# galacticglum/composer

Hardware: AMD Instinct MI355X
Metric: MIDI-event tokens/sec (train, seq=1024) (higher is better)
Workload: dtype bf16; 1 GPU; 6L/8H/d512 Transformer train step, seq=1024, B=128/GPU, dropout 0.10, Adam lr 1e-3, synthetic int32 event ids (vocab 390), random-init weights; global_batch=128, seq_len=1024, parallelism=dp1

## Files before the change

composer_amd/_lib.py:

```python
import ctypes as C
import os

_HERE = os.path.dirname(os.path.abspath(__file__))
LIB_PATH = os.environ.get("COMPOSER_HIP_LIB") or os.path.join(_HERE, "lib", "libcomposer_hip.so")

CMP_FP32, CMP_BF16 = 0, 1
DECODE_LITERAL, DECODE_KV = 0, 1
KIND_VALUE, KIND_ADAM_M, KIND_ADAM_V, KIND_GRAD = 0, 1, 2, 3


class HipLibraryError(RuntimeError):
    pass


class ModelCfg(C.Structure):
    _fields_ = [
        ("vocab_size", C.c_int32), ("embedding_size", C.c_int32), ("window_size", C.c_int32),
        ("layers", C.c_int32), ("heads", C.c_int32), ("ln_eps", C.c_float),
        ("scale_attention", C.c_int32), ("use_layer_norm", C.c_int32),
        ("attn_dropout", C.c_float), ("resid_dropout", C.c_float),
        ("dtype", C.c_int32), ("max_batch", C.c_int32), ("max_seq", C.c_int32), ("seed", C.c_uint64),
    ]


_P = C.c_void_p
_i, _f, _i64, _u64, _u32 = C.c_int, C.c_float, C.c_int64, C.c_uint64, C.c_uint32

SIGNATURES = {
    "cmp_last_error": (C.c_char_p, []),
    "cmp_version": (_i, []),
    "cmp_build_key": (C.c_char_p, []),
    "cmp_device_count": (_i, []),
    "cmp_ctx_create": (_i, [_i, C.POINTER(_P)]),
    "cmp_ctx_destroy": (_i, [_P]),
    "cmp_sync": (_i, [_P]),
    "cmp_ctx_stream": (_P, [_P]),
    "cmp_dp_unique_id": (_i, [_P]),
    "cmp_dp_init": (_i, [_P, _i, _i, _P]),
    "cmp_dp_allreduce_test": (_i, [_P, _P, _i]),
    "cmp_dp_init_exchange": (_i, [_P, _i, _i, _P, _P]),
    "cmp_dp_test_hog": (_i, [_P, _i, _i]),
    "cmp_dp_set_gemm_cus": (_i, [_P, _i]),
    "cmp_dp_set_mask_rank": (_i, [_P, _i]),
    "cmp_dp_stats": (_i, [_P, _i, C.POINTER(_i64), C.POINTER(C.c_double), C.POINTER(_i64), C.POINTER(_i)]),
    "cmp_dp_rccl_version": (_i, [C.POINTER(_i)]),
    "cmp_dp_allreduce_pattern": (_i, [_P, _i, C.POINTER(C.c_double), C.POINTER(_i64), C.POINTER(_i)]),
    "cmp_model_create": (_i, [_P, C.POINTER(ModelCfg), C.POINTER(_P)]),
    "cmp_model_destroy": (_i, [_P]),
    "cmp_param_count": (_i, [_P, C.POINTER(_i)]),
    "cmp_param_info": (_i, [_P, _i, C.POINTER(C.c_char_p), C.POINTER(_i), C.POINTER(_i64 * 4), C.POINTER(_i64)]),
    "cmp_param_get": (_i, [_P, C.c_char_p, _i, _P, _i64]),
    "cmp_param_set": (_i, [_P, C.c_char_p, _i, _P, _i64]),
    "cmp_adam_iter_get": (_i, [_P, C.POINTER(_i64)]),
    "cmp_adam_iter_set": (_i, [_P, _i64]),
    "cmp_train_step": (_i, [_P, _P, _P, _i, _i, _f, C.POINTER(_f), C.POINTER(_f)]),
    "cmp_train_step_dev": (_i, [_P, _P, _P, _i, _i, _f]),
    "cmp_train_metrics": (_i, [_P, C.POINTER(_f), C.POINTER(_f)]),
    "cmp_train_step_launches": (_i, [_P, _P, _P, _i, _i, C.POINTER(_i), C.POINTER(_i)]),
    "cmp_train_step_graph_probe": (_i, [_P, _P, _P, _i, _i, C.POINTER(_i), C.POINTER(_i), _i, C.POINTER(_f)]),
    "cmp_train_step_async": (_i, [_P, _P, _P, _i, _i, _f, C.POINTER(_i64)]),
    "cmp_train_metrics_wait": (_i, [_P, _i64, C.POINTER(_f), C.POINTER(_f)]),
    "cmp_train_options": (_i, [_P, _f, _i]),
    "cmp_train_options_get": (_i, [_P, C.POINTER(_f), C.POINTER(_i), C.POINTER(_i)]),
    "cmp_train_grad_stats": (_i, [_P, C.POINTER(_f), C.POINTER(_f)]),
    "cmp_train_metrics_wait_ex": (_i, [_P, _i64, C.POINTER(_f), C.POINTER(_f), C.POINTER(_f), C.POINTER(_f)]),
    "cmp_loss_and_grads": (_i, [_P, _P, _P, _i, _i, C.POINTER(_f), C.POINTER(_f)]),
    "cmp_eval_step": (_i, [_P, _P, _P, _i, _i, C.POINTER(C.c_double), C.POINTER(_i64), C.POINTER(_i64)]),
    "cmp_present_get": (_i, [_P, _i, _i, _i, _P]),
    "cmp_forward_generation": (_i, [_P, C.POINTER(_i64)]),
    "cmp_present_get_at": (_i, [_P, _i, _i, _i, _i64, _P]),
    "cmp_hidden_get_at": (_i, [_P, _i, _i, _i, _i64, _P]),
    "cmp_forward_logits": (_i, [_P, _P, _i, _i, _P]),
    "cmp_forward": (_i, [_P, _P, _i, _i, _i, _P, _i, _P]),
    "cmp_forward_ex": (_i, [_P, _P, _i, _i, _i, _P, _i, _P, _P, _P, _P, _P]),
    "cmp_decode_begin": (_i, [_P, _P, _i, _i, _f, _u64]),
    "cmp_decode_steps": (_i, [_P, _i, _P]),
    "cmp_decode_logits_get": (_i, [_P, _P]),
    "cmp_decode_begin_slide": (_i, [_P, _P, _i, _i, _f, _u64]),
    "cmp_decode_batch_begin_slide": (_i, [_P, _P, _P, _i, _i, _i, _f, _u64]),
    "cmp_decode_slide_stats": (_i, [_P, _i, _P, _P]),
    "cmp_k_sample": (_i, [_P, _P, _i, _f, _u64, _u32, _i, _P]),
    "cmp_decode_batch_begin": (_i, [_P, _P, _P, _i, _i, _i, _f, _u64]),
    "cmp_decode_batch_steps": (_i, [_P, _i, _P]),
    "cmp_decode_batch_logits_get": (_i, [_P, _P]),
    "cmp_k_sample_rows": (_i, [_P, _P, _i, _i, _i, _f, _u64, _u32, _P]),
    "cmp_k_sample_ex": (_i, [_P, _P, _i, _f, _i, _f, _u64, _u32, _i, _P]),
    "cmp_decode_begin_ex": (_i, [_P, _P, _i, _i, _i, _f, _i, _f, _u64]),
    "cmp_decode_batch_begin_ex": (_i, [_P, _P, _P, _i, _i, _i, _i, _P, _P, _P, _u64]),
    "cmp_k_sample_rows_ex": (_i, [_P, _P, _i, _i, _i, _P, _P, _P, _u64, _u32, _P]),
    "cmp_prof_begin": (_i, [_i]),
    "cmp_prof_end": (_i, [C.POINTER(C.c_double), C.POINTER(_i64), C.POINTER(C.c_double)]),
    "cmp_prof_pause": (_i, []),
    "cmp_prof_resume": (_i, []),
    "cmp_prof_end2": (_i, [C.POINTER(C.c_double), C.POINTER(_i64), C.POINTER(C.c_double), C.POINTER(C.c_double)]),
    "cmp_k_embed_fwd": (_i, [_P, _P, _P, _P, _P, _i, _i, _i, _i, _i, _f, _u64, _u32]),
    "cmp_k_embed_bwd": (_i, [_P, _P, _P, _P, _P, _i, _i, _i, _i, _i, _f, _u64, _u32]),
    "cmp_k_embed_bwd_v": (_i, [_P, _P, _P, _P, _P, _i, _i, _i, _i, _i, _f, _u64, _u32, _i]),
    "cmp_k_layernorm_fwd": (_i, [_P, _P, _P, _P, _P, _P, _P, _i, _i, _f, _i]),
    "cmp_k_layernorm_bwd": (_i, [_P, _P, _P, _P, _P, _P, _P, _P, _P, _P, _P, _i, _i, _i]),
    "cmp_k_layernorm_bwd_ws": (_i64, [_i, _i]),
    "cmp_k_layernorm_bwd_fused": (_i, [_P, _P, _P, _P, _P, _P, _P, _P, _P, _P, _P, _i, _i, _i, _P, _P, _f, _u64, _u32]),
    "cmp_k_gemm": (_i, [_P, _i, _i, _i, _i, _i, _i, _P, _i, _P, _i, _P, _i, _P, _i, _P, _i, _P, _i, _i, _i, _f, _u64, _u32, _i]),
    "cmp_k_embed_fwd_stats": (_i, [_P, _P, _P, _P, _P, _P, _i, _i, _i, _i, _f, _u64, _u32]),
    "cmp_k_ln_fold_prep": (_i, [_P, _P, _P, _P, _P, _P, _P, _P, _i, _i]),
    "cmp_gemm_ln_next": (_i, [_P, _i, _f, _P, _P, _P, _P]),
    "cmp_gemm_ln_scale_next": (_i, [_P, _i, _f]),
    "cmp_attn_bwd_ln_next": (_i, [_P]),
    "cmp_k_ln_stats_merge": (_i, [_P, _P, _i, _f, _P, _P, _i]),
    "cmp_k_layernorm_bwd_prescaled": (_i, [_P, _P, _P, _P, _P, _P, _P, _P, _P, _P, _P, _i, _i, _P, _P, _f, _u64, _u32]),
    "cmp_k_wgrad_ln_fix": (_i, [_P, _P, _i, _i, _P, _P, _P]),
    "cmp_k_layernorm_bwd_parts": (_i, [_P, _P, _P, _P, _P, _P, _f, _P, _P, _P, _P, _P, _P, _i, _i, _P, _P, _f, _u64, _u32]),
    "cmp_model_path_info": (_i, [_P, C.POINTER(_i), C.POINTER(_i64)]),
    "cmp_k_wgrad_group": (_i, [_P, _i, _P, _P, _P, _P, _P, _P, _P, _P, _i]),
    "cmp_gemm_set_workspace": (_i, [_P, _i64]),
    "cmp_gemm_colsum_next": (_i, [_P]),
    "cmp_gemm_set_stamps": (_i, [_P]),
    "cmp_k_colsum": (_i, [_P, _P, _i, _P, _i, _i, _i]),
    "cmp_k_attn_fwd": (_i, [_P, _P, _P, _P, _i, _i, _i, _i, _i, _i, _f, _u64, _u32]),
    "cmp_attn_bwd_bias_next": (_i, [_P]),
    "cmp_k_attn_bwd": (_i, [_P, _P, _P, _P, _P, _P, _P, _i, _i, _i, _i, _i, _i, _f, _u64, _u32]),
    "cmp_k_softmax_xent": (_i, [_P, _P, _i, _P, _P, _P, _P, _i, _i, _f, _i]),
    "cmp_k_adam": (_i, [_P, _P, _P, _P, _P, _P, _i64, _f, _f, _f, _f, _i64, _f]),
    "cmp_k_adam_dev": (_i, [_P, _P, _P, _P, _P, _P, _i64, _f, _f, _f, _f, _i64, _P]),
    "cmp_k_grad_clip_ws": (_i64, [_i64]),
    "cmp_k_grad_clip": (_i, [_P, _P, _i64, _f, _f, _P, _P]),
}

_ADDED_LATER = {"cmp_gemm_ln_scale_next", "cmp_attn_bwd_ln_next", "cmp_k_layernorm_bwd_prescaled", "cmp_k_wgrad_ln_fix", "cmp_k_ln_stats_merge", "cmp_dp_rccl_version", "cmp_dp_allreduce_pattern", "cmp_dp_init_exchange", "cmp_train_step_graph_probe", "cmp_train_step_launches", "cmp_k_embed_fwd_stats", "cmp_k_ln_fold_prep", "cmp_gemm_ln_next", "cmp_k_layernorm_bwd_parts", "cmp_model_path_info", "cmp_forward_ex", "cmp_hidden_get_at", "cmp_dp_stats", "cmp_prof_end2", "cmp_prof_pause", "cmp_prof_resume", "cmp_k_wgrad_group", "cmp_k_embed_bwd_v", "cmp_decode_batch_begin", "cmp_decode_batch_steps", "cmp_k_sample_rows", "cmp_decode_logits_get", "cmp_decode_batch_logits_get", "cmp_k_sample_ex", "cmp_k_sample_rows_ex", "cmp_decode_begin_ex", "cmp_decode_batch_begin_ex", "cmp_train_options",
                "cmp_train_options_get", "cmp_train_grad_stats", "cmp_train_metrics_wait_ex", "cmp_k_adam_dev", "cmp_k_grad_clip_ws", "cmp_k_grad_clip"}

_lib = None


def load():
    global _lib
    if _lib is not None:
        return _lib
    if not os.path.exists(LIB_PATH):
        raise HipLibraryError(
            "libcomposer_hip.so not found at %s -- build it with `python -m composer_amd.build` "
            "(hipcc, gfx950).  composer_amd has no CPU fallback." % LIB_PATH)
    lib = C.CDLL(LIB_PATH)
    check_single_runtime()
    for name, (res, args) in SIGNATURES.items():
        if name in _ADDED_LATER and os.environ.get("COMPOSER_HIP_LIB") and not hasattr(lib, name):
            continue
        fn = getattr(lib, name)
        fn.restype = res
        fn.argtypes = args
    _lib = lib
    return lib


_RUNTIME_STEMS = ("libamdhip64", "librccl", "libhsa-runtime64")


def mapped_runtime_libraries():
    found = {k: set() for k in _RUNTIME_STEMS}
    try:
        with open("/proc/self/maps") as f:
            for line in f:
                path = line.rstrip("\n").split(None, 5)[-1] if line.count("/") else ""
                base = os.path.basename(path)
                for stem in _RUNTIME_STEMS:
                    if base.startswith(stem + ".so"):
                        found[stem].add(os.path.realpath(path))
    except OSError:
        pass
    return {k: sorted(v) for k, v in found.items()}


def check_single_runtime():
    dup = {k: v for k, v in mapped_runtime_libraries().items() if len(v) > 1 and k != "libhsa-runtime64"}
    if dup:
        raise HipLibraryError(
            "two copies of the GPU runtime are mapped into this process: %s.  libcomposer_hip.so was loaded before torch was "
            "imported, so it is bound to /opt/rocm's runtime while torch brought its own.  Fix: `import torch` BEFORE the first "
            "composer_amd call that loads the library (composer_amd._lib.load(), Transformer(...)), or do not import torch in "
            "this process, or put torch's lib directory first in LD_LIBRARY_PATH so both resolve to the same files."
            % "; ".join("%s -> %s" % (k, " AND ".join(v)) for k, v in sorted(dup.items())))


def runtime_info():
    v = C.c_int(0)
    rc = load().cmp_dp_rccl_version(C.byref(v))
    libs = mapped_runtime_libraries()
    return {"rccl_version": v.value if rc == 0 else None, "rccl_path": (libs.get("librccl") or [None])[0],
            "hip_runtime_path": (libs.get("libamdhip64") or [None])[0]}


def last_error():
    return load().cmp_last_error().decode("utf-8", "replace")


def check(rc, what=""):
    if rc != 0:
        raise HipLibraryError("%s failed (status %d): %s" % (what or "libcomposer_hip call", rc, last_error()))


def require_gpu():
    check_single_runtime()
    n = load().cmp_device_count()
    if n <= 0:
        raise HipLibraryError("no HIP device visible: composer_amd needs an MI355X (gfx950); there is no CPU fallback")
    return n
```

composer_amd/build.py:

```python
import hashlib
import json
import os
import subprocess
import sys
from concurrent.futures import ThreadPoolExecutor

HERE = os.path.dirname(os.path.abspath(__file__))
CSRC = os.path.join(HERE, "csrc")
OBJ = os.path.join(CSRC, "_obj")
LIBDIR = os.path.join(HERE, "lib")
LIB = os.path.join(LIBDIR, "libcomposer_hip.so")
ROOT = os.path.dirname(HERE)
SOURCES = ["elementwise.hip", "gemm.hip", "attention.hip", "model.hip", "decode.hip", "decode_batch.hip"]
ARCH = "gfx950"
FLAGS = ["--offload-arch=" + ARCH, "-O3", "-fPIC", "-std=c++17", "-Wno-unused-value", "-Wno-inline-asm", "-I" + os.path.join(ROOT, "include")]
SOURCE_FLAGS = {"attention.hip": ["-fno-slp-vectorize"]}


def flags_for(src, flags=None):
    return list(FLAGS if flags is None else flags) + SOURCE_FLAGS.get(src, [])


def _hipcc():
    for c in (os.environ.get("HIPCC"), "/opt/rocm/bin/hipcc", "hipcc"):
        if c and (os.path.isabs(c) and os.path.exists(c) or not os.path.isabs(c)):
            return c
    return "hipcc"


def _hipcc_version():
    try:
        return subprocess.run([_hipcc(), "--version"], capture_output=True, text=True).stdout.strip().split("\n")[0]
    except Exception:
        return "unknown"


def _headers():
    out = []
    for d in (CSRC, os.path.join(ROOT, "include")):
        for f in sorted(os.listdir(d)):
            if f.endswith(".h"):
                out.append(os.path.join(d, f))
    return out


def source_key(src, flags):
    h = hashlib.sha256()
    h.update(("\0".join(flags) + "\0" + _hipcc_version()).encode())
    for path in [os.path.join(CSRC, src)] + _headers():
        h.update(os.path.basename(path).encode() + b"\0")
        h.update(open(path, "rb").read())
    return h.hexdigest()


def _compile(src, force, flags, tag=""):
    obj = os.path.join(OBJ, tag + src.replace(".hip", ".o"))
    keyfile = obj + ".key"
    key = source_key(src, flags)
    if not force and os.path.exists(obj) and os.path.exists(keyfile) and open(keyfile).read().strip() == key:
        return obj, False, key
    sp = os.path.join(CSRC, src)
    cmd = [_hipcc()] + flags + ["-c", sp, "-o", obj]
    r = subprocess.run(cmd, capture_output=True, text=True)
    if r.returncode != 0:
        raise RuntimeError("hipcc failed for %s:\n%s\n%s" % (src, " ".join(cmd), r.stderr[-4000:]))
    open(keyfile, "w").write(key)
    return obj, True, key


def _lib_key(keys):
    return hashlib.sha256("".join(keys).encode()).hexdigest()


def _file_sha256(path):
    h = hashlib.sha256()
    with open(path, "rb") as f:
        for blk in iter(lambda: f.read(1 << 20), b""):
            h.update(blk)
    return h.hexdigest()


def _key_object(lib_key, tag):
    src = os.path.join(OBJ, tag + "buildkey.cpp")
    obj = os.path.join(OBJ, tag + "buildkey.o")
    open(src, "w").write('extern "C" const char* cmp_build_key(void) { return "%s"; }\n' % lib_key)
    r = subprocess.run(["g++", "-O1", "-fPIC", "-c", src, "-o", obj], capture_output=True, text=True)
    if r.returncode != 0:
        raise RuntimeError("g++ failed for buildkey.cpp:\n" + r.stderr[-2000:])
    return obj


def build(force=False, verbose=True, asan=False):
    os.makedirs(OBJ, exist_ok=True)
    os.makedirs(LIBDIR, exist_ok=True)
    flags = FLAGS + (["-fsanitize=address", "-fno-gpu-sanitize", "-shared-libsan", "-g", "-fno-omit-frame-pointer"] if asan else [])
    tag = "asan_" if asan else ""
    lib = os.path.join(LIBDIR, "libcomposer_hip_asan.so") if asan else LIB
    info_path = os.path.join(LIBDIR, "BUILD_INFO_asan.json" if asan else "BUILD_INFO.json")
    with ThreadPoolExecutor(max_workers=min(5, os.cpu_count() or 1)) as ex:
        res = list(ex.map(lambda s: _compile(s, force, flags_for(s, flags), tag), SOURCES))
    objs = [o for o, _, _ in res]
    lib_key = _lib_key([k for _, _, k in res])
    old = {}
    try:
        old = json.load(open(info_path))
    except Exception:
        pass
    relink = any(c for _, c, _ in res) or not os.path.exists(lib) or old.get("library_key") != lib_key \
        or old.get("library_sha256") != _file_sha256(lib)
    if relink:
        objs = objs + [_key_object(lib_key, tag)]
        cmd = [_hipcc(), "--offload-arch=" + ARCH, "-shared", "-fPIC", "-o", lib] + objs + \
              ["-L/opt/rocm/lib", "-lrccl", "-Wl,-rpath,/opt/rocm/lib"] + (["-fsanitize=address", "-shared-libsan"] if asan else [])
        r = subprocess.run(cmd, capture_output=True, text=True)
        if r.returncode != 0:
            raise RuntimeError("link failed:\n%s\n%s" % (" ".join(cmd), r.stderr[-4000:]))
    info = {"library": os.path.basename(lib), "library_key": lib_key, "library_sha256": _file_sha256(lib), "hipcc": _hipcc_version(), "arch": ARCH,
            "sources": {s: {"key": k, "compiled_by_this_call": bool(c)} for s, (_, c, k) in zip(SOURCES, res)},
            "relinked_by_this_call": bool(relink)}
    json.dump(info, open(info_path, "w"), indent=1)
    if verbose:
        for s, (_, c, _) in zip(SOURCES, res):
            print("  %-18s %s" % (s, "compiled" if c else "cached object (source key unchanged)"))
        print(("built " if relink else "up to date: ") + lib)
    return lib


def verify():
    try:
        info = json.load(open(os.path.join(LIBDIR, "BUILD_INFO.json")))
    except Exception:
        return False
    if not os.path.exists(LIB):
        return False
    want = _lib_key([source_key(s, flags_for(s)) for s in SOURCES])
    if info.get("library_key") != want or info.get("library_sha256") != _file_sha256(LIB):
        return False
    import ctypes
    try:
        fn = ctypes.CDLL(LIB).cmp_build_key
    except (OSError, AttributeError):
        return False
    fn.restype = ctypes.c_char_p
    return fn().decode() == want


if __name__ == "__main__":
    build(force="--force" in sys.argv, asan="--asan" in sys.argv)
```

composer_amd/csrc/elementwise.hip:

```cpp
#include "model.h"

template <typename T>
__global__ void embed_fwd_kernel(const int32_t* __restrict__ ids, const float* __restrict__ wte,
                                 const float* __restrict__ wpe, T* __restrict__ out, int ntok, int T_,
                                 int E, int pos0, DropCfg drop, const int32_t* __restrict__ pos_ids,
                                 const int32_t* __restrict__ type_ids) {
    constexpr int VN = Vec16<T>::N;
    const int chunks = E / VN;
    int64_t gid = (int64_t)blockIdx.x * blockDim.x + threadIdx.x;
    int64_t total = (int64_t)ntok * chunks;
    for (; gid < total; gid += (int64_t)gridDim.x * blockDim.x) {
        int tok = (int)(gid / chunks);
        int e0 = (int)(gid % chunks) * VN;
        int id = ids[tok];
        int t = tok % T_;
        const float* a = wte + (int64_t)id * E + e0;
        const float* p = wpe + (int64_t)(pos_ids ? pos_ids[tok] : pos0 + t) * E + e0;
        const float* ty = type_ids ? wte + (int64_t)type_ids[tok] * E + e0 : nullptr;
        Vec16<T> r;
        const uint32_t rowh = drop_row_hash(drop, (uint32_t)tok);
#pragma unroll
        for (int i = 0; i < VN; i += 4) {
            f32x4 av = *reinterpret_cast<const f32x4*>(a + i);
            f32x4 pv = *reinterpret_cast<const f32x4*>(p + i);
// ... 632 lines not shown
        ssum = wave_sum(ssum);
        const float lse = gmx + logf(ssum);
        if (dz && active) {
            const float inv = 1.0f / ssum;
            Vec16<T> o0, o1;
            float g[8];
#pragma unroll
            for (int j = 0; j < 8; j++) g[j] = (c0 + j < V) ? (e[j] * inv - (c0 + j == yy ? 1.0f : 0.0f)) * inv_n : 0.f;
            T* dr = dz + (int64_t)row * ldz + c0;
            if constexpr (std::is_same<T, float>::value) {
#pragma unroll
                for (int j = 0; j < 4; j++) { o0.set(j, g[j]); o1.set(j, g[4 + j]); }
                st16(dr, o0);
                st16(dr + 4, o1);
            } else {
#pragma unroll
                for (int j = 0; j < 8; j++) o0.set(j, g[j]);
                st16(dr, o0);
            }
        }
        float zy = 0.f;
#pragma unroll
        for (int j = 0; j < 8; j++)
            if (j == (yy & 7)) zy = v[j];
        zy = __shfl(zy, yy >> 3);
        if (lane == 0) {
            row_loss[row] = lse - zy;
            row_correct[row] = (garg == yy) ? 1 : 0;
        }
    }
}

template <typename T>
__global__ void softmax_xent_wide_kernel(const float* __restrict__ z, int ldz, const int32_t* __restrict__ y,
                                         T* __restrict__ dz, float* __restrict__ row_loss,
                                         int32_t* __restrict__ row_correct, int rows, int V, float inv_n) {
    const int lane = threadIdx.x & 63;
    const int wpb = blockDim.x >> 6;
    for (int row = blockIdx.x * wpb + (threadIdx.x >> 6); row < rows; row += gridDim.x * wpb) {
        const float* zr = z + (int64_t)row * ldz;
        float mx = -INFINITY;
        int arg = 0x7fffffff;
        for (int c = lane; c < V; c += 64) {
            const float v = zr[c];
            if (v > mx) {
                mx = v;
                arg = c;
            }
        }
#pragma unroll
        for (int o = 32; o > 0; o >>= 1) {
            float om = __shfl_xor(mx, o);
            int oa = __shfl_xor(arg, o);
            if (om > mx || (om == mx && oa < arg)) {
                mx = om;
                arg = oa;
            }
        }
        float s = 0.f;
        for (int c = lane; c < V; c += 64) s += expf(zr[c] - mx);
        s = wave_sum(s);
        const float lse = mx + logf(s);
        const int yy = y[row];
        if (dz) {
            T* dr = dz + (int64_t)row * ldz;
            for (int c = lane; c < ldz; c += 64) {
                float g = 0.f;
                if (c < V) g = (expf(zr[c] - lse) - (c == yy ? 1.0f : 0.0f)) * inv_n;
                dr[c] = from_f32<T>(g);
            }
        }
        if (lane == 0) {
            row_loss[row] = lse - zr[yy];
            row_correct[row] = (arg == yy) ? 1 : 0;
        }
    }
}

__global__ __launch_bounds__(1024) void metrics_reduce_kernel(const float* __restrict__ row_loss, const int32_t* __restrict__ row_correct,
                                                               int rows, Metrics* __restrict__ out) {
    __shared__ double sl[1024];
    __shared__ long long sc[1024];
    double a0 = 0.0, a1 = 0.0, a2 = 0.0, a3 = 0.0;
    int c = 0;
    const int rows4 = rows >> 2;
    typedef int i32x4 __attribute__((ext_vector_type(4)));
    for (int i = threadIdx.x; i < rows4; i += 1024) {
        const f32x4 l = reinterpret_cast<const f32x4*>(row_loss)[i];
        const i32x4 k = reinterpret_cast<const i32x4*>(row_correct)[i];
        a0 += (double)l[0];
        a1 += (double)l[1];
        a2 += (double)l[2];
        a3 += (double)l[3];
        c += k[0] + k[1] + k[2] + k[3];
    }
    for (int i = (rows4 << 2) + threadIdx.x; i < rows; i += 1024) {
        a0 += (double)row_loss[i];
        c += row_correct[i];
    }
    sl[threadIdx.x] = (a0 + a1) + (a2 + a3);
    sc[threadIdx.x] = c;
    __syncthreads();
    for (int s = 512; s > 0; s >>= 1) {
        if (threadIdx.x < s) {
            sl[threadIdx.x] += sl[threadIdx.x + s];
            sc[threadIdx.x] += sc[threadIdx.x + s];
        }
        __syncthreads();
    }
    if (threadIdx.x == 0) {
        out->loss_sum = sl[0];
        out->correct = sc[0];
        out->loss_mean = (float)(sl[0] / (double)rows);
        out->acc = (float)((double)sc[0] / (double)rows);
    }
}

#define ADAM_LOOP()                                                                     \
    int64_t i = (int64_t)blockIdx.x * blockDim.x + threadIdx.x;                         \
    for (; i < n4; i += (int64_t)gridDim.x * blockDim.x) {                              \
        f32x4 pv = reinterpret_cast<f32x4*>(p)[i];                                      \
        f32x4 gv = reinterpret_cast<const f32x4*>(g)[i];                                \
        f32x4 mv = reinterpret_cast<f32x4*>(m)[i];                                      \
        f32x4 vv = reinterpret_cast<f32x4*>(v)[i];                                      \
        _Pragma("unroll")                                                               \
        for (int j = 0; j < 4; j++) {                                                   \
            float gg = gv[j] * gscale;                                                  \
            mv[j] = beta1 * mv[j] + (1.0f - beta1) * gg;                                \
            vv[j] = beta2 * vv[j] + (1.0f - beta2) * gg * gg;                           \
            pv[j] = pv[j] - alpha * mv[j] / (sqrtf(vv[j]) + eps);                       \
        }                                                                               \
        reinterpret_cast<f32x4*>(p)[i] = pv;                                            \
        reinterpret_cast<f32x4*>(m)[i] = mv;                                            \
        reinterpret_cast<f32x4*>(v)[i] = vv;                                            \
        if (shadow) {                                                                   \
            bf16x4 s;                                                                   \
            _Pragma("unroll")                                                           \
            for (int j = 0; j < 4; j++) s[j] = (bf16_t)pv[j];                           \
            reinterpret_cast<bf16x4*>(shadow)[i] = s;                                   \
        }                                                                               \
    }
__global__ void adam_kernel(float* __restrict__ p, const float* __restrict__ g, float* __restrict__ m,
                            float* __restrict__ v, bf16_t* __restrict__ shadow, int64_t n4, int64_t n,
                            float alpha, float beta1, float beta2, float eps, float gscale) {
    ADAM_LOOP()
}
__global__ void adam_dev_kernel(float* __restrict__ p, const float* __restrict__ g, float* __restrict__ m,
                                float* __restrict__ v, bf16_t* __restrict__ shadow, int64_t n4, int64_t n,
                                float alpha, float beta1, float beta2, float eps, const float* __restrict__ factor_dev) {
    const float gscale = *factor_dev;
    ADAM_LOOP()
}
#undef ADAM_LOOP

#define CLIP_CHUNK 8192
struct GradClipOut { double norm; float scale; float factor; };
__global__ __launch_bounds__(256) void grad_sumsq_kernel(const float* __restrict__ g, int64_t n4, double* __restrict__ slots) {
    __shared__ double sw[4];
    const int64_t base = (int64_t)blockIdx.x * (CLIP_CHUNK / 4);
    const int64_t lim = min(n4, base + CLIP_CHUNK / 4);
    double a0 = 0.0, a1 = 0.0, a2 = 0.0, a3 = 0.0;
#pragma unroll
    for (int r = 0; r < CLIP_CHUNK / 4 / 256; r++) {
        const int64_t i = base + r * 256 + threadIdx.x;
        if (i < lim) {
            const f32x4 x = reinterpret_cast<const f32x4*>(g)[i];
            const double d0 = (double)x[0], d1 = (double)x[1], d2 = (double)x[2], d3 = (double)x[3];
            a0 = fma(d0, d0, a0);
            a1 = fma(d1, d1, a1);
            a2 = fma(d2, d2, a2);
            a3 = fma(d3, d3, a3);
        }
    }
    double a = (a0 + a1) + (a2 + a3);
#pragma unroll
    for (int o = 32; o > 0; o >>= 1) a += __shfl_xor(a, o);
    if ((threadIdx.x & 63) == 0) sw[threadIdx.x >> 6] = a;
    __syncthreads();
    if (threadIdx.x == 0) slots[blockIdx.x] = (sw[0] + sw[1]) + (sw[2] + sw[3]);
}
__global__ __launch_bounds__(256) void grad_clip_finish_kernel(const double* __restrict__ slots, int nslots, float gscale, float clip_norm,
                                                               GradClipOut* __restrict__ out) {
    __shared__ double sl[256];
    double a = 0.0;
    for (int i = threadIdx.x; i < nslots; i += 256) a += slots[i];
    sl[threadIdx.x] = a;
    __syncthreads();
    for (int s = 128; s > 0; s >>= 1) {
        if ((int)threadIdx.x < s) sl[threadIdx.x] += sl[threadIdx.x + s];
        __syncthreads();
    }
    if (threadIdx.x == 0) {
        const double norm = (double)gscale * sqrt(sl[0]);
        const float scale = norm <= (double)clip_norm ? 1.0f : (float)((double)clip_norm / norm);
        out->norm = norm;
        out->scale = scale;
        out->factor = gscale * scale;
    }
}

__global__ void cast_f32_to_bf16_kernel(const float* __restrict__ in, bf16_t* __restrict__ out, int64_t n4) {
    int64_t i = (int64_t)blockIdx.x * blockDim.x + threadIdx.x;
    for (; i < n4; i += (int64_t)gridDim.x * blockDim.x) {
        f32x4 a = reinterpret_cast<const f32x4*>(in)[i];
        bf16x4 s;
#pragma unroll
        for (int j = 0; j < 4; j++) s[j] = (bf16_t)a[j];
        reinterpret_cast<bf16x4*>(out)[i] = s;
    }
}

template <typename T>
__global__ __launch_bounds__(256) void colsum_kernel(const T* __restrict__ X, int ldx, float* __restrict__ out, int rows, int cols,
                                                     float* __restrict__ part) {
    constexpr int VN = Vec16<T>::N;
    __shared__ float sm[4][64 * VN];
    const int lane = threadIdx.x & 63, wave = threadIdx.x >> 6;
    const int c0 = (blockIdx.x * 64 + lane) * VN;
    const int rows_per = cdiv(rows, (int)gridDim.y);
    const int r0 = blockIdx.y * rows_per;
    const int r1 = min(rows, r0 + rows_per);
    float acc[VN];
#pragma unroll
    for (int j = 0; j < VN; j++) acc[j] = 0.f;
    if (c0 < cols) {
        int r = r0 + wave;
        for (; r + 12 < r1; r += 16) {
            Vec16<T> v0 = ld16(X + (int64_t)r * ldx + c0), v1 = ld16(X + (int64_t)(r + 4) * ldx + c0);
            Vec16<T> v2 = ld16(X + (int64_t)(r + 8) * ldx + c0), v3 = ld16(X + (int64_t)(r + 12) * ldx + c0);
#pragma unroll
            for (int j = 0; j < VN; j++) acc[j] += (v0.get(j) + v1.get(j)) + (v2.get(j) + v3.get(j));
        }
        for (; r < r1; r += 4) {
            Vec16<T> v0 = ld16(X + (int64_t)r * ldx + c0);
#pragma unroll
            for (int j = 0; j < VN; j++) acc[j] += v0.get(j);
        }
    }
#pragma unroll
    for (int j = 0; j < VN; j++) sm[wave][lane * VN + j] = acc[j];
    __syncthreads();
    for (int i = threadIdx.x; i < 64 * VN; i += 256) {
        int c = blockIdx.x * 64 * VN + i;
        const float v = sm[0][i] + sm[1][i] + sm[2][i] + sm[3][i];
        if (c < cols) {
            if (part) part[(size_t)blockIdx.y * cols + c] = v;
            else atomicAdd(out + c, v);
        }
    }
}
__global__ void colsum_fold_kernel(const float* __restrict__ part, float* __restrict__ out, int splits, int cols) {
    const int c = blockIdx.x * blockDim.x + threadIdx.x;
    if (c >= cols) return;
    float a = 0.f;
    for (int sI = 0; sI < splits; sI++) a += part[(size_t)sI * cols + c];
    out[c] += a;
}

extern "C" int cmp_k_embed_fwd(void* stream, const int32_t* ids, const float* wte, const float* wpe, void* out,
                               int B, int T, int E, int pos0, int dtype, float p_drop, uint64_t seed,
                               uint32_t rng_stream) {
    return embed_fwd_run(stream, ids, wte, wpe, out, B, T, E, pos0, dtype, p_drop, seed, rng_stream, nullptr, nullptr);
}

int embed_fwd_run(void* stream, const int32_t* ids, const float* wte, const float* wpe, void* out, int B, int T, int E, int pos0,
                  int dtype, float p_drop, uint64_t seed, uint32_t rng_stream, const int32_t* pos_ids, const int32_t* type_ids) {
    CMP_REQUIRE(E % 8 == 0, "embed_fwd: E=%d must be a multiple of 8", E);
    hipStream_t s = (hipStream_t)stream;
    DropCfg d = make_drop(p_drop, seed, rng_stream);
    int ntok = B * T;
    if (ntok == 0) return CMP_OK;
    if (dtype == CMP_BF16) {
        int64_t total = (int64_t)ntok * (E / 8);
        int grid = (int)std::min<int64_t>(cdiv64(total, 256), 4096);
        embed_fwd_kernel<bf16_t><<<grid, 256, 0, s>>>(ids, wte, wpe, (bf16_t*)out, ntok, T, E, pos0, d, pos_ids, type_ids);
    } else {
        int64_t total = (int64_t)ntok * (E / 4);
        int grid = (int)std::min<int64_t>(cdiv64(total, 256), 4096);
        embed_fwd_kernel<float><<<grid, 256, 0, s>>>(ids, wte, wpe, (float*)out, ntok, T, E, pos0, d, pos_ids, type_ids);
    }
    KERNEL_CHECK();
    return CMP_OK;
}

int embed_fwd_stats_run(void* stream, const int32_t* ids, const float* wte, const float* wpe, void* out, float* part, int B, int T,
                        int E, int pos0, float p_drop, uint64_t seed, uint32_t rng_stream) {
    CMP_REQUIRE(E % 256 == 0 && E <= 2048, "embed_fwd_stats: E=%d must be a multiple of 256, at most 2048", E);
    hipStream_t s = (hipStream_t)stream;
    DropCfg d = make_drop(p_drop, seed, rng_stream);
    const int ntok = B * T;
    if (ntok == 0) return CMP_OK;
    const int grid = std::min(cdiv(ntok, 4), 8192), maxi = cdiv(E / 8, 64);
#define EMB_ST(MI) embed_fwd_stats_kernel<MI><<<grid, 256, 0, s>>>(ids, wte, wpe, (bf16_t*)out, part, ntok, T, E, pos0, d)
    if (maxi == 1) EMB_ST(1); else if (maxi == 2) EMB_ST(2); else EMB_ST(4);
#undef EMB_ST
    KERNEL_CHECK();
    return CMP_OK;
}
extern "C" int cmp_k_embed_fwd_stats(void* stream, const int32_t* ids, const float* wte, const float* wpe, void* out, float* part,
                                     int B, int T, int E, int pos0, float p_drop, uint64_t seed, uint32_t rng_stream) {
    return embed_fwd_stats_run(stream, ids, wte, wpe, out, part, B, T, E, pos0, p_drop, seed, rng_stream);
}

__global__ __launch_bounds__(256) void ln_fold_prep_kernel(const float* __restrict__ P, bf16_t* __restrict__ ST, float* __restrict__ fold,
                                                           const FoldDesc* __restrict__ desc) {
    __shared__ bf16_t tile[32][34];
// ... 277 lines not shown
__global__ __launch_bounds__(1024) void wgrad_ln_fix_kernel(LnFixDesc d0, LnFixDesc d1) {
    __shared__ float part[32][33];
    const LnFixDesc d = ((int)blockIdx.x >= d1.blk0 && d1.G) ? d1 : d0;
    const int tx = threadIdx.x & 31, ty = threadIdx.x >> 5;
    const int c = ((int)blockIdx.x - d.blk0) * 32 + tx;
    const bool ok = c < d.cols;
    float s0 = 0.f, s1 = 0.f, s2 = 0.f, s3 = 0.f;
    if (ok) {
        int k = ty;
        for (; k + 96 < d.rows; k += 128) {
            s0 += d.G[(int64_t)k * d.cols + c];
            s1 += d.G[(int64_t)(k + 32) * d.cols + c];
            s2 += d.G[(int64_t)(k + 64) * d.cols + c];
            s3 += d.G[(int64_t)(k + 96) * d.cols + c];
        }
        for (; k < d.rows; k += 32) s0 += d.G[(int64_t)k * d.cols + c];
    }
    part[ty][tx] = (s0 + s1) + (s2 + s3);
    __syncthreads();
    float tot = 0.f;
#pragma unroll
    for (int t = 0; t < 32; t++) tot += part[t][tx];
    if (!ok) return;
    const float mean = tot / (float)d.rows, bc = d.colsum[c];
    for (int k = ty; k < d.rows; k += 32) {
        const int64_t at = (int64_t)k * d.cols + c;
        d.G[at] = fmaf(d.gamma[k], d.G[at] - mean, d.beta[k] * bc);
    }
}
int wgrad_ln_fix_run(void* stream, float* G0, int rows0, int cols0, const float* gamma0, const float* beta0, const float* colsum0,
                     float* G1, int rows1, int cols1, const float* gamma1, const float* beta1, const float* colsum1) {
    CMP_REQUIRE(G0 && gamma0 && beta0 && colsum0 && rows0 > 0 && cols0 > 0, "wgrad_ln_fix: bad arguments");
    LnFixDesc d0{G0, gamma0, beta0, colsum0, rows0, cols0, 0, 0};
    LnFixDesc d1{G1, gamma1, beta1, colsum1, rows1, cols1, cdiv(cols0, 32), 0};
    const int grid = cdiv(cols0, 32) + (G1 ? cdiv(cols1, 32) : 0);
    wgrad_ln_fix_kernel<<<grid, 1024, 0, (hipStream_t)stream>>>(d0, d1);
    KERNEL_CHECK();
    return CMP_OK;
}
int layernorm_bwd_run(void* stream, const void* dy, const void* x, const float* gamma, const float* mean, const float* rstd,
                      const void* resid, void* dx, float* dgamma, float* dbeta, void* ws, int rows, int E, int dtype, void* dmask,
                      float* colsum, float p_drop, uint64_t seed, uint32_t rng_stream, bool deterministic, const LnBwdFused* fz,
                      bool keep_dmask, bool prescaled) {
    int rc = ln_check(E, dtype);
    if (rc) return rc;
    if (rows == 0) return CMP_OK;
    hipStream_t s = (hipStream_t)stream;
    int grid = ln_bwd_grid(rows);
    size_t smem = (size_t)4 * 3 * E * sizeof(float);
    const int vn = dtype == CMP_BF16 ? 8 : 4;
    const int maxi = cdiv(E / vn, 64);
    DropCfg dcfg = make_drop(p_drop, seed, rng_stream);
    if (fz) CMP_REQUIRE(dtype == CMP_BF16 && fz->part && fz->beta && E % 256 == 0 && fz->np == E / 256,
                        "layernorm_bwd: the statistics-from-partials form needs bf16 rows of a multiple of 256 columns (E=%d, np=%d)", E, fz->np);
    if (p_drop <= 0.f && !fz && !keep_dmask) dmask = nullptr;
    PROF_START(8, s);
    const int want_cs = colsum != nullptr;
    const bool direct = !deterministic && grid <= 256;
    float* dg_ = direct ? dgamma : nullptr;
#define LN_BWD(TT, MI) do { \
        if (smem > 65536) HIP_CHECK(hipFuncSetAttribute((const void*)layernorm_bwd_kernel<TT, MI>, hipFuncAttributeMaxDynamicSharedMemorySize, (int)smem)); \
        layernorm_bwd_kernel<TT, MI><<<grid, 256, smem, s>>>((const TT*)dy, (const TT*)x, gamma, mean, rstd, (const TT*)resid, (TT*)dx, (float*)ws, rows, E, (TT*)dmask, want_cs, dcfg, dg_, dbeta, colsum); \
    } while (0)
#define LN_BWDF(MI) do { \
        if (smem > 65536) HIP_CHECK(hipFuncSetAttribute((const void*)layernorm_bwd_kernel<bf16_t, MI, true>, hipFuncAttributeMaxDynamicSharedMemorySize, (int)smem)); \
        layernorm_bwd_kernel<bf16_t, MI, true><<<grid, 256, smem, s>>>((const bf16_t*)dy, (const bf16_t*)x, gamma, mean, rstd, (const bf16_t*)resid, (bf16_t*)dx, (float*)ws, rows, E, (bf16_t*)dmask, want_cs, dcfg, dg_, dbeta, colsum, *fz); \
    } while (0)
#define LN_BWDP(MI) do { \
        if (smem > 65536) HIP_CHECK(hipFuncSetAttribute((const void*)layernorm_bwd_kernel<bf16_t, MI, false, true>, hipFuncAttributeMaxDynamicSharedMemorySize, (int)smem)); \
        layernorm_bwd_kernel<bf16_t, MI, false, true><<<grid, 256, smem, s>>>((const bf16_t*)dy, (const bf16_t*)x, gamma, mean, rstd, (const bf16_t*)resid, (bf16_t*)dx, (float*)ws, rows, E, (bf16_t*)dmask, want_cs, dcfg, dg_, dbeta, colsum); \
    } while (0)
    if (prescaled && !fz) {
        CMP_REQUIRE(dtype == CMP_BF16 && maxi <= 4, "layernorm_bwd: the prescaled form exists for bf16 rows of at most 2048 columns");
        if (maxi == 1) LN_BWDP(1); else if (maxi == 2) LN_BWDP(2); else LN_BWDP(4);
    } else
    if (fz) { if (maxi == 1) LN_BWDF(1); else if (maxi == 2) LN_BWDF(2); else if (maxi <= 4) LN_BWDF(4); else LN_BWDF(8); }
    else if (dtype == CMP_BF16) { if (maxi == 1) LN_BWD(bf16_t, 1); else if (maxi == 2) LN_BWD(bf16_t, 2); else if (maxi <= 4) LN_BWD(bf16_t, 4); else LN_BWD(bf16_t, 8); }
    else { if (maxi == 1) LN_BWD(float, 1); else if (maxi == 2) LN_BWD(float, 2); else if (maxi <= 4) LN_BWD(float, 4); else LN_BWD(float, 8); }
#undef LN_BWD
#undef LN_BWDF
#undef LN_BWDP
    KERNEL_CHECK();
    if (!direct)
        ln_param_reduce_kernel<<<dim3(cdiv(3 * E, 256), deterministic ? 1 : std::min(grid, 32)), 256, 0, s>>>((const float*)ws, dgamma, dbeta, colsum, grid, E);
    {
        const double lb = (double)rows * ((3.0 + (resid ? 1.0 : 0.0) + (dmask ? 1.0 : 0.0) + (fz && fz->yout ? 1.0 : 0.0)) * E * dtype_size(dtype) + 8.0);
        PROF_STOP(8, s, lb, lb);
    }
    KERNEL_CHECK();
    return CMP_OK;
}

extern "C" int cmp_k_softmax_xent(void* stream, const float* logits, int ldz, const int32_t* y, void* dlogits,
                                  float* row_loss, int32_t* row_correct, int rows, int V, float inv_n, int dtype) {
    CMP_REQUIRE(V > 0 && V <= ldz, "softmax_xent: V=%d ldz=%d", V, ldz);
    if (rows == 0) return CMP_OK;
    hipStream_t s = (hipStream_t)stream;
    int grid = std::min(cdiv(rows, 4), 8192);
    if (ldz > 64 * XENT_MAXI) {
        if (dtype == CMP_BF16)
            softmax_xent_wide_kernel<bf16_t><<<grid, 256, 0, s>>>(logits, ldz, y, (bf16_t*)dlogits, row_loss, row_correct, rows, V, inv_n);
        else
            softmax_xent_wide_kernel<float><<<grid, 256, 0, s>>>(logits, ldz, y, (float*)dlogits, row_loss, row_correct, rows, V, inv_n);
    } else if (ldz % 8 == 0 && ((uintptr_t)logits & 15) == 0 && ((uintptr_t)dlogits & 15) == 0) {
        if (dtype == CMP_BF16)
            softmax_xent8_kernel<bf16_t><<<grid, 256, 0, s>>>(logits, ldz, y, (bf16_t*)dlogits, row_loss, row_correct, rows, V, inv_n);
        else
            softmax_xent8_kernel<float><<<grid, 256, 0, s>>>(logits, ldz, y, (float*)dlogits, row_loss, row_correct, rows, V, inv_n);
    } else if (dtype == CMP_BF16)
        softmax_xent_kernel<bf16_t><<<grid, 256, 0, s>>>(logits, ldz, y, (bf16_t*)dlogits, row_loss, row_correct, rows, V, inv_n);
    else
        softmax_xent_kernel<float><<<grid, 256, 0, s>>>(logits, ldz, y, (float*)dlogits, row_loss, row_correct, rows, V, inv_n);
    KERNEL_CHECK();
    return CMP_OK;
}

int launch_metrics_reduce(hipStream_t s, const float* row_loss, const int32_t* row_correct, int rows, void* metrics) {
    metrics_reduce_kernel<<<1, 1024, 0, s>>>(row_loss, row_correct, rows, (Metrics*)metrics);
    KERNEL_CHECK();
    return CMP_OK;
}

extern "C" int cmp_k_adam(void* stream, float* p, const float* g, float* m, float* v, void* shadow_bf16, int64_t n,
                          float lr, float beta1, float beta2, float eps, int64_t step, float grad_scale) {
    CMP_REQUIRE(n % 4 == 0, "adam: n=%lld must be a multiple of 4", (long long)n);
    if (n == 0) return CMP_OK;
    hipStream_t s = (hipStream_t)stream;
    double alpha = (double)lr * sqrt(1.0 - pow((double)beta2, (double)step)) / (1.0 - pow((double)beta1, (double)step));
    int64_t n4 = n / 4;
    int grid = (int)std::min<int64_t>(cdiv64(n4, 256), 8192);
    PROF_START(7, s);
    adam_kernel<<<grid, 256, 0, s>>>(p, g, m, v, (bf16_t*)shadow_bf16, n4, n, (float)alpha, beta1, beta2, eps, grad_scale);
    PROF_STOP(7, s, (double)n * (28.0 + (shadow_bf16 ? 2.0 : 0.0)), (double)n * (28.0 + (shadow_bf16 ? 2.0 : 0.0)));
    KERNEL_CHECK();
    return CMP_OK;
}

extern "C" int cmp_k_adam_dev(void* stream, float* p, const float* g, float* m, float* v, void* shadow_bf16, int64_t n,
                              float lr, float beta1, float beta2, float eps, int64_t step, const float* factor_dev) {
    CMP_REQUIRE(n % 4 == 0, "adam_dev: n=%lld must be a multiple of 4", (long long)n);
    CMP_REQUIRE(factor_dev, "adam_dev: null factor");
    if (n == 0) return CMP_OK;
    hipStream_t s = (hipStream_t)stream;
    double alpha = (double)lr * sqrt(1.0 - pow((double)beta2, (double)step)) / (1.0 - pow((double)beta1, (double)step));
    int64_t n4 = n / 4;
    int grid = (int)std::min<int64_t>(cdiv64(n4, 256), 8192);
    PROF_START(7, s);
    adam_dev_kernel<<<grid, 256, 0, s>>>(p, g, m, v, (bf16_t*)shadow_bf16, n4, n, (float)alpha, beta1, beta2, eps, factor_dev);
    PROF_STOP(7, s, (double)n * (28.0 + (shadow_bf16 ? 2.0 : 0.0)), (double)n * (28.0 + (shadow_bf16 ? 2.0 : 0.0)));
    KERNEL_CHECK();
    return CMP_OK;
}

int64_t grad_sumsq_slots(int64_t n) { return cdiv64(n, CLIP_CHUNK); }
int grad_sumsq_run(void* stream, const float* g, int64_t n, double* slots) {
    CMP_REQUIRE(n % 4 == 0 && ((uintptr_t)g & 15) == 0, "grad_sumsq: n=%lld must be a multiple of 4 and the range 16-byte aligned", (long long)n);
    CMP_REQUIRE(grad_sumsq_slots(n) < (1ll << 31), "grad_sumsq: n=%lld is too large", (long long)n);
    if (n == 0) return CMP_OK;
    grad_sumsq_kernel<<<(int)grad_sumsq_slots(n), 256, 0, (hipStream_t)stream>>>(g, n / 4, slots);
    KERNEL_CHECK();
    return CMP_OK;
}
int grad_clip_finish_run(void* stream, const double* slots, int nslots, float gscale, float clip_norm, void* out) {
    grad_clip_finish_kernel<<<1, 256, 0, (hipStream_t)stream>>>(slots, nslots, gscale, clip_norm, (GradClipOut*)out);
    KERNEL_CHECK();
    return CMP_OK;
}
extern "C" int64_t cmp_k_grad_clip_ws(int64_t n) { return std::max<int64_t>(1, grad_sumsq_slots(n)) * 8; }
extern "C" int cmp_k_grad_clip(void* stream, const float* g, int64_t n, float gscale, float clip_norm, void* ws, void* out) {
    CMP_REQUIRE(g && ws && out && n > 0, "grad_clip: null argument or empty range");
    CMP_REQUIRE(clip_norm > 0.f, "grad_clip: clip_norm %g must be positive (+inf: measure only)", (double)clip_norm);
    CMP_REQUIRE(((uintptr_t)ws & 7) == 0 && ((uintptr_t)out & 7) == 0, "grad_clip: ws and out must be 8-byte aligned");
    { const int rc = grad_sumsq_run(stream, g, n, (double*)ws); if (rc != CMP_OK) return rc; }
    return grad_clip_finish_run(stream, (const double*)ws, (int)grad_sumsq_slots(n), gscale, clip_norm, out);
}

int launch_cast_bf16(hipStream_t s, const float* in, void* out, int64_t n) {
    if (n == 0) return CMP_OK;
    int64_t n4 = n / 4;
    int grid = (int)std::min<int64_t>(cdiv64(n4, 256), 8192);
    cast_f32_to_bf16_kernel<<<grid, 256, 0, s>>>(in, (bf16_t*)out, n4);
    KERNEL_CHECK();
    return CMP_OK;
}

extern "C" int cmp_k_colsum(void* stream, const void* X, int ldx, float* out, int rows, int cols, int dtype) {
    return colsum_run(stream, X, ldx, out, rows, cols, dtype, nullptr, 0);
}

int colsum_run(void* stream, const void* X, int ldx, float* out, int rows, int cols, int dtype, float* det_ws, size_t det_ws_bytes) {
    if (rows == 0 || cols == 0) return CMP_OK;
    hipStream_t s = (hipStream_t)stream;
    const int vn = dtype == CMP_BF16 ? 8 : 4;
    CMP_REQUIRE(cols % vn == 0 && ldx % vn == 0, "colsum: cols=%d and ldx=%d must be multiples of %d", cols, ldx, vn);
    const int gx = cdiv(cols, 64 * vn);
    int splits = std::max(1, std::min(std::min(rows / 64, 128), std::max(1, 1024 / gx)));
    dim3 grid(gx, splits);
    if (det_ws) CMP_REQUIRE((size_t)splits * cols * 4 <= det_ws_bytes, "colsum: deterministic workspace too small");
    if (dtype == CMP_BF16)
        colsum_kernel<bf16_t><<<grid, 256, 0, s>>>((const bf16_t*)X, ldx, out, rows, cols, det_ws);
    else
        colsum_kernel<float><<<grid, 256, 0, s>>>((const float*)X, ldx, out, rows, cols, det_ws);
    if (det_ws) colsum_fold_kernel<<<cdiv(cols, 256), 256, 0, s>>>(det_ws, out, splits, cols);
    KERNEL_CHECK();
    return CMP_OK;
}
```

composer_amd/csrc/model.h:

```cpp
#pragma once
#include "common.h"
#include <rccl/rccl.h>
#include <vector>
#include <string>
#include <map>

struct DecodeState;
struct DecodeBatchState;

struct GradClipStats { double norm; float scale; float factor; };

struct Metrics {
    double loss_sum;
    long long correct;
    float loss_mean;
    float acc;
    int bad_ids;
    int pad;
};

#define NCCL_CHECK(expr)                                                                         \
    do {                                                                                         \
        ncclResult_t _r = (expr);                                                                \
        if (_r != ncclSuccess) {                                                                 \
            cmp_set_error("%s:%d: %s failed: %s", __FILE__, __LINE__, #expr, ncclGetErrorString(_r)); \
            return CMP_ERR_RCCL;                                                                 \
        }                                                                                        \
    } while (0)

#define CHECK_RC(expr)            \
    do {                          \
        int _rc = (expr);         \
        if (_rc != CMP_OK) return _rc; \
    } while (0)

struct cmp_ctx {
    int device = 0;
    hipStream_t stream = nullptr;
    hipStream_t comm_stream = nullptr;
    ncclComm_t comm = nullptr;
    int (*xfn)(void*, void*, int64_t, void*) = nullptr;
    void* xuser = nullptr;
    bool dp_on() const { return comm != nullptr || xfn != nullptr; }
    int rank = 0, nranks = 1;
    uint32_t seed_mix = 0;
    int mask_rank = 0;
    int gemm_max_wgs = 0;
    hipStream_t copy_stream = nullptr;
    SchedWs gemm_sched;
};
void sched_ws_free(SchedWs* w);

struct ParamInfo {
    std::string name;
    int rank;
    int64_t shape[4];
    int64_t numel;
    int64_t offset;
    int pad = 0;
    int64_t store = 0;
};

struct LayerOff {
    int64_t ln1_g, ln1_b, attn_w, attn_b, proj_w, proj_b, ln2_g, ln2_b, fc_w, fc_b, pr_w, pr_b;
    int64_t begin, end;
};

struct WDesc {
    int64_t off;
    int rows, cols;
};

struct FoldDesc {
    int64_t w_off, b_off, g_off, be_off;
    int64_t out_off;
    int rows, cols;
};

struct LayerAct {
    void *u, *qkv, *att, *r, *n, *fc, *g;
    float *ln1_mean, *ln1_rstd, *ln2_mean, *ln2_rstd, *lse;
    float *ln1_part = nullptr, *ln2_part = nullptr;
};

struct cmp_model {
    cmp_ctx* ctx = nullptr;
    cmp_model_cfg cfg;
    int V, E, W, L, H, D, ldz;
    int Dl = 0, Ea = 0;
    int dtype;
    size_t es;
    std::vector<ParamInfo> params;
    std::map<std::string, int> index;
    int64_t total = 0;
    int64_t off_wte = 0, off_wpe = 0, off_lnf_g = 0, off_lnf_b = 0;
    std::vector<LayerOff> lo;
    float *P = nullptr, *G = nullptr, *Am = nullptr, *Av = nullptr;
    bf16_t* S = nullptr;
    bf16_t* ST = nullptr;
    void* wdesc = nullptr;
    void* wdesc_plain = nullptr;
    void* fdesc = nullptr;
    void* ln_sites = nullptr;
    float* lnfold = nullptr;
    int64_t fold_stride = 0;
    int st_state = 0;
    int64_t st_version = -1;
    bool fused_last = false;
    void* dmask3 = nullptr;
    bf16_t* wte_lnf = nullptr;
    float* lnf_fold = nullptr;
    int lnf_npad = 0;
    float* lnf_part = nullptr;
    bool hf_valid = false;
    int64_t iterations = 0;
    int64_t param_version = 0;
    int capB = 0, capT = 0;
    std::vector<void*> allocs;
    std::vector<void*> xs;
    const int32_t* fwd_pos_ids = nullptr;
    const int32_t* fwd_type_ids = nullptr;
    const float* fwd_amask = nullptr;
    float* const* fwd_probs_out = nullptr;
    float* fwd_probs_dev = nullptr;
    void* io_buf[3] = {nullptr, nullptr, nullptr};
    size_t io_buf_bytes[3] = {0, 0, 0};
    std::vector<LayerAct> act;
    void *hf = nullptr, *dlogits = nullptr;
    float* logits_pack = nullptr;
    float *logits = nullptr, *lnf_mean = nullptr, *lnf_rstd = nullptr, *row_loss = nullptr, *delta = nullptr;
    int32_t *row_correct = nullptr, *x_dev = nullptr, *y_dev = nullptr;
    void *dx = nullptr, *dr = nullptr, *tmpE = nullptr, *dmask = nullptr, *dfc = nullptr, *dqkv = nullptr;
    int* embed_ws = nullptr;
    int64_t embed_ws_words = 0;
    void* dmask2 = nullptr;
    std::vector<WgradGroup> wgrad_groups;
    WgradWs wgrad_ws;
    void* ln_ws = nullptr;
    void* slab = nullptr;
    int64_t slab_bytes = 0;
    Metrics* metrics = nullptr;
    Metrics* metrics_host = nullptr;
    float* dp_metrics = nullptr;
    static constexpr int STAGES = 3;
    int32_t* stage_host[STAGES] = {nullptr, nullptr, nullptr};
    int32_t* stage_dev[STAGES] = {nullptr, nullptr, nullptr};
    Metrics* stage_metrics = nullptr;
    hipEvent_t stage_uploaded[STAGES] = {nullptr, nullptr, nullptr};
    hipEvent_t stage_done[STAGES] = {nullptr, nullptr, nullptr};
    int64_t stage_ticket[STAGES] = {-1, -1, -1};
    int64_t next_ticket = 0;
    int64_t stage_cap = 0;
    int lastB = 0, lastT = 0, last_past = 0;
    int64_t fwd_gen = 0;
    std::vector<hipEvent_t> bucket_ev;
    hipEvent_t comm_done = nullptr, metrics_ev = nullptr;
    static constexpr int DP_RING = 32;
    hipEvent_t dp_wait_a[DP_RING] = {}, dp_wait_b[DP_RING] = {};
    bool dp_wait_used[DP_RING] = {};
    int64_t dp_steps = 0;
    int64_t dp_folded = 0;
    double dp_exposed_ms = 0.0;
    int64_t dp_bytes_step = 0;
    int dp_msgs_step = 0;
    int dp_buckets_updated = 0;
    bool poisoned = false;
    float clip_norm = 0.f;
    int accum_steps = 1;
    int accum_pending = 0;
    int accumB = 0, accumT = 0;
    double* clip_slots = nullptr;
    int64_t clip_slots_cap = 0;
    int64_t clip_slots_used = 0;
    GradClipStats* clip_out = nullptr;
    GradClipStats* clip_host = nullptr;
    bool last_has_norm = false;
    bool stage_has_norm[3] = {false, false, false};
    std::vector<char> reload_seen;
    int ln_fused_mode = -1;
    DecodeState* dec = nullptr;
    DecodeBatchState* decb = nullptr;
    int gemm_role = -1;

    uint64_t drop_seed() const { return (uint64_t)((uint32_t)cfg.seed ^ ctx->seed_mix); }
    const void* w(int64_t off) const { return dtype == CMP_BF16 ? (const void*)(S + off) : (const void*)(P + off); }
};


template <typename Tp> static int dev_alloc(cmp_model* m, Tp** p, size_t bytes) {
    void* q = nullptr;
    HIP_CHECK(hipMalloc(&q, bytes ? bytes : 16));
    m->allocs.push_back(q);
    *p = (Tp*)q;
    return CMP_OK;
}

int embed_fwd_run(void* stream, const int32_t* ids, const float* wte, const float* wpe, void* out, int B, int T, int E, int pos0,
                  int dtype, float p_drop, uint64_t seed, uint32_t rng_stream, const int32_t* pos_ids, const int32_t* type_ids);
int embed_bwd_run(void* stream, const int32_t* ids, const void* dh, float* dwte, float* dwpe, int B, int T, int E, int pos0,
                  int dtype, float p_drop, uint64_t seed, uint32_t rng_stream, int V, float* det_ws, size_t det_ws_bytes,
                  int sort_V = 0, int* sort_ws = nullptr, int64_t sort_ws_words = 0);
int64_t embed_bwd_sort_ws_words(int64_t ntok, int V);
struct LnBwdFused {
    const float* part = nullptr;
    int np = 0;
    float eps = 0.f;
    const float* beta = nullptr;
    void* yout = nullptr;
    int prescaled = 0;
};
int wgrad_ln_fix_run(void* stream, float* G0, int rows0, int cols0, const float* gamma0, const float* beta0, const float* colsum0,
                     float* G1, int rows1, int cols1, const float* gamma1, const float* beta1, const float* colsum1);
int layernorm_bwd_run(void* stream, const void* dy, const void* x, const float* gamma, const float* mean, const float* rstd,
                      const void* resid, void* dx, float* dgamma, float* dbeta, void* ws, int rows, int E, int dtype, void* dmask,
                      float* colsum, float p_drop, uint64_t seed, uint32_t rng_stream, bool deterministic, const LnBwdFused* fz = nullptr,
                      bool keep_dmask = false, bool prescaled = false);
int ln_stats_merge_run(void* stream, const void* sites_dev, int nsites, int np, float eps, int rows);
int embed_fwd_stats_run(void* stream, const int32_t* ids, const float* wte, const float* wpe, void* out, float* part, int B, int T,
                        int E, int pos0, float p_drop, uint64_t seed, uint32_t rng_stream);
int ln_fold_prep_run(void* stream, const float* P, void* ST, float* fold, const void* desc_dev, int ndesc, int max_cols);
int lnf_fold_prep_run(void* stream, const float* wte, const float* gamma, const float* beta, void* out, float* cs, float* bias, int V, int E,
                      int npad);
int colsum_run(void* stream, const void* X, int ldx, float* out, int rows, int cols, int dtype, float* det_ws, size_t det_ws_bytes);
int launch_metrics_reduce(hipStream_t s, const float* row_loss, const int32_t* row_correct, int rows, void* metrics);
int launch_cast_bf16(hipStream_t s, const float* in, void* out, int64_t n);
int64_t grad_sumsq_slots(int64_t n);
int grad_sumsq_run(void* stream, const float* g, int64_t n, double* slots);
int grad_clip_finish_run(void* stream, const double* slots, int nslots, float gscale, float clip_norm, void* out);
int ensure_workspace(cmp_model* m, int B, int T);
int model_forward(cmp_model* m, const int32_t* x_dev, int B, int T, bool training, int64_t step, int past_len = 0);
void decode_state_free(DecodeState* d);
void decode_batch_state_free(DecodeBatchState* d);
int decode_batch_slide_stats(DecodeBatchState* d, int64_t* row_slides, int64_t* forward_calls);
```

composer_amd/csrc/model.hip:

```cpp
#include "model.h"
#include <stdarg.h>
#include <dlfcn.h>

static thread_local char g_err[1024] = "";
void cmp_set_error(const char* fmt, ...) {
    va_list ap;
    va_start(ap, fmt);
    vsnprintf(g_err, sizeof(g_err), fmt, ap);
    va_end(ap);
}
extern "C" const char* cmp_last_error(void) { return g_err; }
extern "C" int cmp_version(void) { return 1; }
extern "C" int cmp_device_count(void) {
    int n = 0;
    if (hipGetDeviceCount(&n) != hipSuccess) return 0;
    return n;
}

thread_local int g_prof_cls = -1;
static thread_local std::vector<hipEvent_t> g_prof_ev;
static thread_local size_t g_prof_used = 0;
static thread_local double g_prof_work = 0.0, g_prof_bytes = 0.0;
void prof_start(int, hipStream_t s) {
    if (g_prof_used + 2 > g_prof_ev.size()) {
// ... 151 lines not shown
        const int rc = c->xfn(c->xuser, p, (int64_t)n, (void*)c->comm_stream);
        if (rc != 0) {
            cmp_set_error("data-parallel exchange function failed with %d on %zu floats", rc, n);
            return CMP_ERR_INVALID;
        }
        return CMP_OK;
    }
    NCCL_CHECK(ncclAllReduce(p, p, n, ncclFloat, ncclSum, c->comm, c->comm_stream));
    return CMP_OK;
}
extern "C" int cmp_dp_set_mask_rank(cmp_ctx* c, int rank) {
    CMP_REQUIRE(c && rank >= 0, "dp_set_mask_rank: bad arguments");
    c->seed_mix = mix32((uint32_t)rank);
    c->mask_rank = rank;
    return CMP_OK;
}
extern "C" int cmp_dp_set_gemm_cus(cmp_ctx* c, int cus) {
    CMP_REQUIRE(c && cus >= 0 && cus <= 256, "dp_set_gemm_cus: 0 (all) .. 256");
    c->gemm_max_wgs = cus;
    return CMP_OK;
}
__global__ __launch_bounds__(1024) void cu_hog_kernel(unsigned long long ticks, int* sink) {
    __shared__ int big[16384];
    big[threadIdx.x] = (int)threadIdx.x;
    __syncthreads();
    const unsigned long long t0 = __builtin_amdgcn_s_memrealtime();
    while (__builtin_amdgcn_s_memrealtime() - t0 < ticks) __builtin_amdgcn_s_sleep(32);
    if (sink && big[(threadIdx.x * 7) & 16383] == -1) *sink = 1;
}
extern "C" int cmp_dp_test_hog(cmp_ctx* c, int wgs, int usec) {
    CMP_REQUIRE(c && wgs > 0 && wgs <= 256 && usec > 0 && usec <= 1000000, "dp_test_hog: bad arguments");
    HIP_CHECK(hipSetDevice(c->device));
    cu_hog_kernel<<<wgs, 1024, 0, c->comm_stream>>>((unsigned long long)usec * 100ull, nullptr);
    KERNEL_CHECK();
    return CMP_OK;
}
extern "C" int cmp_dp_allreduce_test(cmp_ctx* c, float* host_inout, int n) {
    CMP_REQUIRE(c && c->dp_on(), "dp_allreduce_test: communicator not initialised");
    float* d = nullptr;
    HIP_CHECK(hipMalloc(&d, (size_t)n * 4));
    HIP_CHECK(hipMemcpyAsync(d, host_inout, (size_t)n * 4, hipMemcpyHostToDevice, c->comm_stream));
    if (const int rc = dp_allreduce(c, d, (size_t)n)) {
        (void)hipStreamSynchronize(c->comm_stream);
        (void)hipFree(d);
        return rc;
    }
    HIP_CHECK(hipMemcpyAsync(host_inout, d, (size_t)n * 4, hipMemcpyDeviceToHost, c->comm_stream));
    HIP_CHECK(hipStreamSynchronize(c->comm_stream));
    HIP_CHECK(hipFree(d));
    return CMP_OK;
}

static int64_t add_param(cmp_model* m, const std::string& name, int rank, int64_t d0, int64_t d1, int pad = 0) {
    ParamInfo p;
    p.name = name;
    p.rank = rank;
    p.shape[0] = d0;
    p.shape[1] = d1;
    p.shape[2] = p.shape[3] = 1;
    p.numel = d0 * (rank > 1 ? d1 : 1);
    p.pad = (m->Dl == m->D) ? 0 : pad;
    p.store = p.numel;
    if (p.pad == 1) p.store = d0 * 3 * m->Ea;
    if (p.pad == 2) p.store = (int64_t)m->Ea * d1;
    p.offset = m->total;
    m->total += (p.store + 7) / 8 * 8;
    m->index[name] = (int)m->params.size();
    m->params.push_back(p);
    return p.offset;
}


static int model_create_fill(cmp_model* m, cmp_ctx* ctx, const cmp_model_cfg* cfg, int V, int E, int W, int L, int H, int D, int Dl);
extern "C" int cmp_model_destroy(cmp_model* m);

extern "C" int cmp_model_create(cmp_ctx* ctx, const cmp_model_cfg* cfg, cmp_model** out) {
    CMP_REQUIRE(ctx && cfg && out, "model_create: null argument");
    const int V = cfg->vocab_size, E = cfg->embedding_size, W = cfg->window_size, L = cfg->layers, H = cfg->heads;
    CMP_REQUIRE(V > 0 && E > 0 && W > 0 && L > 0 && H > 0, "model_create: sizes must be positive");
    CMP_REQUIRE(E % H == 0, "model_create: embedding_size %d not divisible by heads %d (transformer.py:255)", E, H);
    CMP_REQUIRE(E % 8 == 0, "model_create: embedding_size %d must be a multiple of 8", E);
    CMP_REQUIRE(E <= 2048, "model_create: embedding_size %d unsupported (at most 2048: LayerNorm rows, per-token decode rows of 4E)", E);
    const int Dl = E / H;
    CMP_REQUIRE(Dl <= 128, "model_create: head size %d unsupported (at most 128)", Dl);
    const int D = Dl <= 16 ? 16 : (Dl <= 32 ? 32 : (Dl <= 64 ? 64 : 128));
    CMP_REQUIRE(cfg->dtype == CMP_FP32 || cfg->dtype == CMP_BF16, "model_create: bad dtype %d", cfg->dtype);
    CMP_REQUIRE(L < 64, "model_create: at most 63 layers");
    HIP_CHECK(hipSetDevice(ctx->device));
    cmp_model* m = new cmp_model();
    m->ctx = ctx;
    {
        const char* e = getenv("COMPOSER_LN_FUSED");
        m->ln_fused_mode = e ? atoi(e) : -1;
    }
    const int rc = model_create_fill(m, ctx, cfg, V, E, W, L, H, D, Dl);
    if (rc != CMP_OK) { cmp_model_destroy(m); return rc; }
    *out = m;
    return CMP_OK;
}

static int model_create_fill(cmp_model* m, cmp_ctx* ctx, const cmp_model_cfg* cfg, int V, int E, int W, int L, int H, int D, int Dl) {
    m->cfg = *cfg;
    m->V = V; m->E = E; m->W = W; m->L = L; m->H = H; m->D = D; m->Dl = Dl; m->Ea = H * D;
    m->ldz = (V + 63) / 64 * 64;
    m->dtype = cfg->dtype;
    m->es = dtype_size(cfg->dtype);
    m->off_wte = add_param(m, "wte/weight", 2, V, E);
    m->off_wpe = add_param(m, "wpe/embeddings", 2, W, E);
    m->lo.resize(L);
    for (int i = 0; i < L; i++) {
        std::string p = "decoder_blocks/" + std::to_string(i) + "/";
        LayerOff& o = m->lo[i];
        o.begin = m->total;
        o.ln1_g = add_param(m, p + "ln_1/gamma", 1, E, 1);
        o.ln1_b = add_param(m, p + "ln_1/beta", 1, E, 1);
        o.attn_w = add_param(m, p + "attn/c_attn/weight", 2, E, 3 * E, 1);
        o.attn_b = add_param(m, p + "attn/c_attn/bias", 2, 1, 3 * E, 1);
        o.proj_w = add_param(m, p + "attn/c_proj/weight", 2, E, E, 2);
        o.proj_b = add_param(m, p + "attn/c_proj/bias", 2, 1, E);
        o.ln2_g = add_param(m, p + "ln_2/gamma", 1, E, 1);
        o.ln2_b = add_param(m, p + "ln_2/beta", 1, E, 1);
        o.fc_w = add_param(m, p + "mlp/c_fc/weight", 2, E, 4 * E);
        o.fc_b = add_param(m, p + "mlp/c_fc/bias", 2, 1, 4 * E);
        o.pr_w = add_param(m, p + "mlp/c_proj/weight", 2, 4 * E, E);
        o.pr_b = add_param(m, p + "mlp/c_proj/bias", 2, 1, E);
        o.end = m->total;
    }
    m->off_lnf_g = add_param(m, "ln_f/gamma", 1, E, 1);
    m->off_lnf_b = add_param(m, "ln_f/beta", 1, E, 1);
    size_t bytes = (size_t)m->total * 4;
    CHECK_RC(dev_alloc(m, &m->P, bytes));
    CHECK_RC(dev_alloc(m, &m->G, bytes));
    CHECK_RC(dev_alloc(m, &m->Am, bytes));
    CHECK_RC(dev_alloc(m, &m->Av, bytes));
    HIP_CHECK(hipMemsetAsync(m->P, 0, bytes, ctx->stream));
    HIP_CHECK(hipMemsetAsync(m->G, 0, bytes, ctx->stream));
    HIP_CHECK(hipMemsetAsync(m->Am, 0, bytes, ctx->stream));
    HIP_CHECK(hipMemsetAsync(m->Av, 0, bytes, ctx->stream));
    if (m->dtype == CMP_BF16) {
        CHECK_RC(dev_alloc(m, &m->S, (size_t)m->total * 2));
        HIP_CHECK(hipMemsetAsync(m->S, 0, (size_t)m->total * 2, ctx->stream));
        CHECK_RC(dev_alloc(m, &m->ST, (size_t)m->total * 2));
        HIP_CHECK(hipMemsetAsync(m->ST, 0, (size_t)m->total * 2, ctx->stream));
        std::vector<WDesc> wd;
        for (int i = 0; i < m->L; i++) {
            const LayerOff& o = m->lo[i];
            wd.push_back({o.attn_w, m->E, 3 * m->Ea});
            wd.push_back({o.proj_w, m->Ea, m->E});
            wd.push_back({o.fc_w, m->E, 4 * m->E});
            wd.push_back({o.pr_w, 4 * m->E, m->E});
        }
        CHECK_RC(dev_alloc(m, &m->wdesc, wd.size() * sizeof(WDesc)));
        HIP_CHECK(hipMemcpyAsync(m->wdesc, wd.data(), wd.size() * sizeof(WDesc), hipMemcpyHostToDevice, ctx->stream));
        std::vector<WDesc> wp;
        std::vector<FoldDesc> fd;
        m->fold_stride = 2 * (int64_t)(3 * m->Ea + 4 * m->E);
        for (int i = 0; i < m->L; i++) {
            const LayerOff& o = m->lo[i];
            wp.push_back({o.proj_w, m->Ea, m->E});
            wp.push_back({o.pr_w, 4 * m->E, m->E});
            fd.push_back({o.attn_w, o.attn_b, o.ln1_g, o.ln1_b, i * m->fold_stride, m->E, 3 * m->Ea});
            fd.push_back({o.fc_w, o.fc_b, o.ln2_g, o.ln2_b, i * m->fold_stride + 6 * m->Ea, m->E, 4 * m->E});
        }
        CHECK_RC(dev_alloc(m, &m->wdesc_plain, wp.size() * sizeof(WDesc)));
        CHECK_RC(dev_alloc(m, &m->fdesc, fd.size() * sizeof(FoldDesc)));
        CHECK_RC(dev_alloc(m, &m->lnfold, (size_t)m->L * m->fold_stride * 4));
        m->lnf_npad = cdiv(m->V, 256) * 256;
        CHECK_RC(dev_alloc(m, &m->wte_lnf, (size_t)m->V * m->E * 2));
        CHECK_RC(dev_alloc(m, &m->lnf_fold, (size_t)2 * m->lnf_npad * 4));
        HIP_CHECK(hipMemcpyAsync(m->wdesc_plain, wp.data(), wp.size() * sizeof(WDesc), hipMemcpyHostToDevice, ctx->stream));
        HIP_CHECK(hipMemcpyAsync(m->fdesc, fd.data(), fd.size() * sizeof(FoldDesc), hipMemcpyHostToDevice, ctx->stream));
        HIP_CHECK(hipStreamSynchronize(ctx->stream));
    }
    CHECK_RC(dev_alloc(m, &m->metrics, sizeof(Metrics)));
    CHECK_RC(dev_alloc(m, &m->dp_metrics, 16));
    HIP_CHECK(hipHostMalloc((void**)&m->metrics_host, sizeof(Metrics), hipHostMallocDefault));
    memset(m->metrics_host, 0, sizeof(Metrics));
    m->bucket_ev.resize(L + 2);
    for (auto& e : m->bucket_ev) HIP_CHECK(hipEventCreateWithFlags(&e, hipEventDisableTiming));
    HIP_CHECK(hipEventCreateWithFlags(&m->comm_done, hipEventDisableTiming));
    HIP_CHECK(hipEventCreateWithFlags(&m->metrics_ev, hipEventDisableTiming));
    HIP_CHECK(hipStreamSynchronize(ctx->stream));
    return CMP_OK;
}

extern "C" int cmp_model_destroy(cmp_model* m) {
    if (!m) return CMP_OK;
    hipSetDevice(m->ctx->device);
    hipStreamSynchronize(m->ctx->stream);
    hipStreamSynchronize(m->ctx->comm_stream);
    if (m->ctx->copy_stream) hipStreamSynchronize(m->ctx->copy_stream);
    if (m->dec) decode_state_free(m->dec);
    if (m->decb) decode_batch_state_free(m->decb);
    for (void* p : m->allocs) if (p) hipFree(p);
    for (auto& wg : m->wgrad_groups) wgrad_group_free(&wg);
    wgrad_ws_free(&m->wgrad_ws);
    if (m->metrics_host) hipHostFree(m->metrics_host);
    if (m->clip_host) hipHostFree(m->clip_host);
    if (m->stage_metrics) hipHostFree(m->stage_metrics);
    for (int i = 0; i < cmp_model::STAGES; i++) {
        if (m->stage_host[i]) hipHostFree(m->stage_host[i]);
        if (m->stage_uploaded[i]) hipEventDestroy(m->stage_uploaded[i]);
        if (m->stage_done[i]) hipEventDestroy(m->stage_done[i]);
    }
    for (auto& e : m->bucket_ev) hipEventDestroy(e);
    if (m->comm_done) hipEventDestroy(m->comm_done);
    if (m->metrics_ev) hipEventDestroy(m->metrics_ev);
    for (int i = 0; i < cmp_model::DP_RING; i++) {
        if (m->dp_wait_a[i]) hipEventDestroy(m->dp_wait_a[i]);
        if (m->dp_wait_b[i]) hipEventDestroy(m->dp_wait_b[i]);
    }
    delete m;
    (void)hipGetLastError();
    return CMP_OK;
}

extern "C" int cmp_param_count(cmp_model* m, int* n) {
    CMP_REQUIRE(m && n, "param_count: null");
    *n = (int)m->params.size();
    return CMP_OK;
}
extern "C" int cmp_param_info(cmp_model* m, int i, const char** name, int* rank, int64_t shape[4], int64_t* numel) {
    CMP_REQUIRE(m && i >= 0 && i < (int)m->params.size(), "param_info: index %d out of range", i);
    const ParamInfo& p = m->params[i];
    if (name) *name = p.name.c_str();
    if (rank) *rank = p.rank;
    if (shape) for (int k = 0; k < 4; k++) shape[k] = p.shape[k];
    if (numel) *numel = p.numel;
    return CMP_OK;
}
static void pad_copy(const cmp_model* m, const ParamInfo& p, float* st, float* logical, bool to_store) {
    const int H = m->H, D = m->D, Dl = m->Dl, E = m->E, Ea = m->Ea;
    if (p.pad == 1) {
        const int64_t rows = p.numel / (3 * E);
        for (int64_t r = 0; r < rows; r++)
            for (int part = 0; part < 3; part++)
                for (int h = 0; h < H; h++)
                    for (int d = 0; d < Dl; d++) {
                        float& a = st[r * 3 * Ea + (int64_t)part * Ea + h * D + d];
                        float& b = logical[r * 3 * E + (int64_t)part * E + h * Dl + d];
                        if (to_store) a = b; else b = a;
                    }
    } else {
        const int64_t cols = p.shape[1];
        for (int h = 0; h < H; h++)
            for (int d = 0; d < Dl; d++)
                for (int64_t c = 0; c < cols; c++) {
                    float& a = st[((int64_t)h * D + d) * cols + c];
                    float& b = logical[((int64_t)h * Dl + d) * cols + c];
                    if (to_store) a = b; else b = a;
                }
    }
}
static float* kind_buf(cmp_model* m, int kind) {
    switch (kind) {
        case 0: return m->P;
        case 1: return m->Am;
        case 2: return m->Av;
        case 3: return m->G;
    }
    return nullptr;
}
extern "C" int cmp_param_get(cmp_model* m, const char* name, int kind, float* host, int64_t numel) {
    CMP_REQUIRE(m && name && host, "param_get: null");
    auto it = m->index.find(name);
    CMP_REQUIRE(it != m->index.end(), "param_get: unknown parameter '%s'", name);
    const ParamInfo& p = m->params[it->second];
    CMP_REQUIRE(numel == p.numel, "param_get: '%s' has %lld elements, caller passed %lld", name, (long long)p.numel, (long long)numel);
    float* b = kind_buf(m, kind);
    CMP_REQUIRE(b, "param_get: bad kind %d", kind);
    HIP_CHECK(hipStreamSynchronize(m->ctx->stream));
    HIP_CHECK(hipStreamSynchronize(m->ctx->comm_stream));
    if (p.pad) {
        std::vector<float> st((size_t)p.store);
        HIP_CHECK(hipMemcpyAsync(st.data(), b + p.offset, (size_t)p.store * 4, hipMemcpyDeviceToHost, m->ctx->stream));
        HIP_CHECK(hipStreamSynchronize(m->ctx->stream));
        pad_copy(m, p, st.data(), host, false);
        return CMP_OK;
    }
    HIP_CHECK(hipMemcpyAsync(host, b + p.offset, (size_t)numel * 4, hipMemcpyDeviceToHost, m->ctx->stream));
    HIP_CHECK(hipStreamSynchronize(m->ctx->stream));
    return CMP_OK;
}
extern "C" int cmp_param_set(cmp_model* m, const char* name, int kind, const float* host, int64_t numel) {
    CMP_REQUIRE(m && name && host, "param_set: null");
    auto it = m->index.find(name);
    CMP_REQUIRE(it != m->index.end(), "param_set: unknown parameter '%s'", name);
    const ParamInfo& p = m->params[it->second];
    CMP_REQUIRE(numel == p.numel, "param_set: '%s' has %lld elements, caller passed %lld", name, (long long)p.numel, (long long)numel);
    float* b = kind_buf(m, kind);
    CMP_REQUIRE(b, "param_set: bad kind %d", kind);
    HIP_CHECK(hipStreamSynchronize(m->ctx->stream));
    if (p.pad) {
        std::vector<float> st((size_t)p.store, 0.f);
        pad_copy(m, p, st.data(), const_cast<float*>(host), true);
        HIP_CHECK(hipMemcpyAsync(b + p.offset, st.data(), (size_t)p.store * 4, hipMemcpyHostToDevice, m->ctx->stream));
        HIP_CHECK(hipStreamSynchronize(m->ctx->stream));
    } else {
        HIP_CHECK(hipMemcpyAsync(b + p.offset, host, (size_t)numel * 4, hipMemcpyHostToDevice, m->ctx->stream));
        HIP_CHECK(hipStreamSynchronize(m->ctx->stream));
    }
    if (kind == 0) {
        m->param_version += 1;
        if (m->poisoned) {
            if (m->reload_seen.size() != m->params.size()) m->reload_seen.assign(m->params.size(), 0);
            m->reload_seen[it->second] = 1;
            bool all = true;
            for (char c : m->reload_seen) all = all && c;
            if (all) { m->poisoned = false; m->reload_seen.clear(); }
        }
    }
    if (kind == 0 && m->S) {
        int64_t n8 = (p.store + 7) / 8 * 8;
        CHECK_RC(launch_cast_bf16(m->ctx->stream, m->P + p.offset, m->S + p.offset, n8));
        HIP_CHECK(hipStreamSynchronize(m->ctx->stream));
    }
    return CMP_OK;
}
extern "C" int cmp_adam_iter_get(cmp_model* m, int64_t* it) {
    CMP_REQUIRE(m && it, "adam_iter_get: null");
    *it = m->iterations;
    return CMP_OK;
}
extern "C" int cmp_adam_iter_set(cmp_model* m, int64_t it) {
    CMP_REQUIRE(m && it >= 0, "adam_iter_set: bad value");
    m->iterations = it;
    return CMP_OK;
}

static int ensure_workspace_fill(cmp_model* m, int B, int T);
int ensure_workspace(cmp_model* m, int B, int T) {
    const size_t mark = m->allocs.size();
    const int rc = ensure_workspace_fill(m, B, T);
    if (rc != CMP_OK && m->allocs.size() > mark) {
        for (size_t i = mark; i < m->allocs.size(); i++) (void)hipFree(m->allocs[i]);
        m->allocs.resize(mark);
        m->xs.clear(); m->act.clear();
        m->capB = 0; m->capT = 0;
        (void)hipGetLastError();
    }
    return rc;
}
static int ensure_workspace_fill(cmp_model* m, int B, int T) {
    CMP_REQUIRE(B > 0 && T > 0, "batch and sequence must be positive (B=%d T=%d)", B, T);
    CMP_REQUIRE(T <= m->W, "sequence length %d exceeds window_size %d (wpe rows, transformer.py:675-679)", T, m->W);
    if (m->capB * m->capT >= B * T && m->capB > 0) return CMP_OK;
    CMP_REQUIRE(m->capB == 0, "workspace was sized for %d tokens; create the model with max_batch/max_seq covering B=%d T=%d",
                m->capB * m->capT, B, T);
    int64_t M = (int64_t)B * T;
    int64_t Mcfg = (int64_t)std::max(1, m->cfg.max_batch) * std::max(1, std::min(m->cfg.max_seq, m->W));
    if (Mcfg > M) { M = Mcfg; }
    m->capB = (int)M; m->capT = 1;
    const int E = m->E, L = m->L;
    const size_t es = m->es;
    m->xs.resize(L + 1);
    for (int i = 0; i <= L; i++) CHECK_RC(dev_alloc(m, &m->xs[i], (size_t)M * E * es));
    m->act.resize(L);
    const bool ln = m->cfg.use_layer_norm != 0;
    for (int i = 0; i < L; i++) {
        LayerAct& a = m->act[i];
        if (ln) CHECK_RC(dev_alloc(m, &a.u, (size_t)M * E * es)); else a.u = m->xs[i];
        CHECK_RC(dev_alloc(m, &a.qkv, (size_t)M * 3 * m->Ea * es));
        CHECK_RC(dev_alloc(m, &a.att, (size_t)M * m->Ea * es));
        CHECK_RC(dev_alloc(m, &a.r, (size_t)M * E * es));
        if (ln) CHECK_RC(dev_alloc(m, &a.n, (size_t)M * E * es)); else a.n = a.r;
        CHECK_RC(dev_alloc(m, &a.fc, (size_t)M * 4 * E * es));
        CHECK_RC(dev_alloc(m, &a.g, (size_t)M * 4 * E * es));
        CHECK_RC(dev_alloc(m, &a.ln1_mean, (size_t)M * 4));
        CHECK_RC(dev_alloc(m, &a.ln1_rstd, (size_t)M * 4));
        CHECK_RC(dev_alloc(m, &a.ln2_mean, (size_t)M * 4));
        CHECK_RC(dev_alloc(m, &a.ln2_rstd, (size_t)M * 4));
        CHECK_RC(dev_alloc(m, &a.lse, (size_t)M * m->H * 4));
        if (ln && m->ST && E % 256 == 0) {
            CHECK_RC(dev_alloc(m, &a.ln1_part, (size_t)M * (E / 256) * 8));
            CHECK_RC(dev_alloc(m, &a.ln2_part, (size_t)M * (E / 256) * 8));
        }
    }
    if (ln && m->ST && E % 256 == 0) CHECK_RC(dev_alloc(m, &m->lnf_part, (size_t)M * (E / 256) * 8));
    if (ln && m->ST && E % 256 == 0) {
        std::vector<const void*> st;
        for (int i = 0; i < L; i++) {
            const LayerAct& a = m->act[i];
            st.insert(st.end(), {a.ln1_part, a.ln1_mean, a.ln1_rstd, a.ln2_part, a.ln2_mean, a.ln2_rstd});
        }
        CHECK_RC(dev_alloc(m, &m->ln_sites, st.size() * sizeof(void*)));
        HIP_CHECK(hipMemcpyAsync(m->ln_sites, st.data(), st.size() * sizeof(void*), hipMemcpyHostToDevice, m->ctx->stream));
        HIP_CHECK(hipStreamSynchronize(m->ctx->stream));
    }
    CHECK_RC(dev_alloc(m, &m->hf, (size_t)M * E * es));
    CHECK_RC(dev_alloc(m, &m->logits, (size_t)M * m->ldz * 4));
    CHECK_RC(dev_alloc(m, &m->dlogits, (size_t)M * m->ldz * es));
    CHECK_RC(dev_alloc(m, &m->lnf_mean, (size_t)M * 4));
    CHECK_RC(dev_alloc(m, &m->lnf_rstd, (size_t)M * 4));
    CHECK_RC(dev_alloc(m, &m->row_loss, (size_t)M * 4));
    CHECK_RC(dev_alloc(m, &m->row_correct, (size_t)M * 4));
    CHECK_RC(dev_alloc(m, &m->delta, (size_t)M * m->H * 4));
    CHECK_RC(dev_alloc(m, &m->x_dev, (size_t)M * 4));
    CHECK_RC(dev_alloc(m, &m->y_dev, (size_t)M * 4));
    CHECK_RC(dev_alloc(m, &m->dx, (size_t)M * E * es));
    CHECK_RC(dev_alloc(m, &m->dr, (size_t)M * E * es));
    CHECK_RC(dev_alloc(m, &m->tmpE, (size_t)M * m->Ea * es));
    CHECK_RC(dev_alloc(m, &m->dmask, (size_t)M * E * es));
    CHECK_RC(dev_alloc(m, &m->dmask2, (size_t)M * E * es));
    CHECK_RC(dev_alloc(m, &m->dmask3, (size_t)M * E * es));
    CHECK_RC(dev_alloc(m, &m->dfc, (size_t)M * 4 * E * es));
    CHECK_RC(dev_alloc(m, &m->dqkv, (size_t)M * 3 * m->Ea * es));
    {
        const char* det = getenv("COMPOSER_DETERMINISTIC");
        if (det && det[0] == '1') {
            m->slab_bytes = (int64_t)16 * E * std::max(4 * E, 3 * m->Ea) * 4 + (int64_t)64 * m->V * E * 4;
            CHECK_RC(dev_alloc(m, &m->slab, (size_t)m->slab_bytes));
        }
    }
    CHECK_RC(dev_alloc(m, &m->ln_ws, (size_t)cmp_k_layernorm_bwd_ws((int)std::min<int64_t>(M, 1 << 30), E)));
    m->embed_ws_words = embed_bwd_sort_ws_words(M, m->V);
    if (m->embed_ws_words > 0) CHECK_RC(dev_alloc(m, &m->embed_ws, (size_t)m->embed_ws_words * 4));
    return CMP_OK;
}

template <typename T>
__global__ void drop_apply_kernel(const T* __restrict__ in, T* __restrict__ out, int64_t n, int E, DropCfg d) {
    int64_t i = (int64_t)blockIdx.x * blockDim.x + threadIdx.x;
    for (; i < n; i += (int64_t)gridDim.x * blockDim.x)
        out[i] = from_f32<T>(apply_drop(d, (uint32_t)(i / E), (uint32_t)(i % E), to_f32<T>(in[i])));
}
static int drop_apply(cmp_model* m, const void* in, void* out, int64_t n, float p, uint32_t stream_id) {
    DropCfg d = make_drop(p, m->drop_seed(), stream_id);
    int grid = (int)std::min<int64_t>(cdiv64(n, 256), 8192);
    if (m->dtype == CMP_BF16)
        drop_apply_kernel<bf16_t><<<grid, 256, 0, m->ctx->stream>>>((const bf16_t*)in, (bf16_t*)out, n, m->cfg.embedding_size, d);
    else
        drop_apply_kernel<float><<<grid, 256, 0, m->ctx->stream>>>((const float*)in, (float*)out, n, m->cfg.embedding_size, d);
    KERNEL_CHECK();
    return CMP_OK;
}

__global__ __launch_bounds__(256) void transpose_weights_kernel(const bf16_t* __restrict__ S, bf16_t* __restrict__ ST,
                                                                const WDesc* __restrict__ desc) {
    __shared__ bf16_t tile[32][34];
    const WDesc d = desc[blockIdx.y];
    const int tiles_c = (d.cols + 31) >> 5, ntiles = ((d.rows + 31) >> 5) * tiles_c;
    if ((int)blockIdx.x >= ntiles) return;
    const int tr = (blockIdx.x / tiles_c) << 5, tc = (blockIdx.x % tiles_c) << 5;
    const int tx = threadIdx.x & 31, ty = threadIdx.x >> 5;
    const bf16_t* src = S + d.off;
    bf16_t* dst = ST + d.off;
#pragma unroll
    for (int j = 0; j < 4; j++) {
        const int r = tr + ty + 8 * j, c = tc + tx;
        tile[ty + 8 * j][tx] = (r < d.rows && c < d.cols) ? src[(int64_t)r * d.cols + c] : (bf16_t)0.f;
    }
    __syncthreads();
#pragma unroll
    for (int j = 0; j < 4; j++) {
        const int c = tc + ty + 8 * j, r = tr + tx;
        if (c < d.cols && r < d.rows) dst[(int64_t)c * d.rows + r] = tile[tx][ty + 8 * j];
    }
}
static int refresh_transposed_weights(cmp_model* m, bool fold) {
    if (!m->ST) return CMP_OK;
    const int want = fold ? 2 : 1;
    if (m->st_state == want && m->st_version == m->param_version) return CMP_OK;
    m->st_state = 0;
    const int maxtiles = std::max(cdiv(4 * m->E, 32) * cdiv(m->E, 32), cdiv(3 * m->Ea, 32) * cdiv(m->E, 32));
    if (fold) {
        transpose_weights_kernel<<<dim3(maxtiles, 2 * m->L), 256, 0, m->ctx->stream>>>(m->S, m->ST, (const WDesc*)m->wdesc_plain);
        KERNEL_CHECK();
        CHECK_RC(ln_fold_prep_run(m->ctx->stream, m->P, m->ST, m->lnfold, m->fdesc, 2 * m->L, 4 * m->E));
        CHECK_RC(lnf_fold_prep_run(m->ctx->stream, m->P + m->off_wte, m->P + m->off_lnf_g, m->P + m->off_lnf_b, m->wte_lnf, m->lnf_fold,
                                   m->lnf_fold + m->lnf_npad, m->V, m->E, m->lnf_npad));
    } else {
        transpose_weights_kernel<<<dim3(maxtiles, 4 * m->L), 256, 0, m->ctx->stream>>>(m->S, m->ST, (const WDesc*)m->wdesc);
        KERNEL_CHECK();
    }
    m->st_state = want;
    m->st_version = m->param_version;
    return CMP_OK;
}

static bool ln_fused_ok(const cmp_model* m, int M, int past_len, bool training) {
    if (m->ln_fused_mode == 0) return false;
    if (training && m->ln_fused_mode != 2 && m->ln_fused_mode != 3) return false;
    if (!m->cfg.use_layer_norm || m->dtype != CMP_BF16 || m->slab || past_len) return false;
    if (m->Ea != m->E || m->E % 256 || m->E < 512 || m->E > 768 || !m->act[0].ln1_part) return false;
    if (M % 256 || (int64_t)(M / 256) * (m->E / 256) < 192) return false;
    if (m->fwd_pos_ids || m->fwd_type_ids || m->fwd_amask || m->fwd_probs_out) return false;
    return true;
}

static int colsum_det(cmp_model* m, const void* X, int ldx, float* out, int rows, int cols) {
    return colsum_run(m->ctx->stream, X, ldx, out, rows, cols, m->dtype, (float*)m->slab, (size_t)m->slab_bytes);
}
static int colsum_any(cmp_model* m, const void* X, int ldx, float* out, int rows, int cols) {
    if (m->slab) return colsum_det(m, X, ldx, out, rows, cols);
    return cmp_k_colsum(m->ctx->stream, X, ldx, out, rows, cols, m->dtype);
}
static int ln_bwd(cmp_model* m, const void* dy, const void* x, const float* gamma, const float* mean, const float* rstd,
                  const void* resid, void* dx, float* dgamma, float* dbeta, int rows, void* dmask, float* colsum, float p_drop,
                  uint32_t rng_stream, const LnBwdFused* fz = nullptr, bool prescaled = false) {
    return layernorm_bwd_run(m->ctx->stream, dy, x, gamma, mean, rstd, resid, dx, dgamma, dbeta, m->ln_ws, rows, m->E, m->dtype,
                             dmask, colsum, p_drop, m->drop_seed(), rng_stream, m->slab != nullptr, fz, m->fused_last, prescaled);
}

#define GEMM_REV (1 << 20)
static int gemm(cmp_model* m, int ta, int tb, int M, int N, int K, const void* A, int lda, const void* B, int ldb, void* C,
                int ldc, const float* bias, int act, void* aux, int ldaux, const void* resid, int ldr, int out_fp32,
                int splitk, float p_drop, uint32_t rng_stream, int flags = 0, float* colsum = nullptr, const LnEpi* ln = nullptr) {
    const bool det = m->slab != nullptr;
    GemmExtra ex;
    if (ln) ex.ln = *ln;
    ex.rev = (flags & GEMM_REV) != 0;
    flags &= ~GEMM_REV;
    ex.colsum = det ? nullptr : colsum;
    if (splitk > 1 && det) { ex.slab_ws = (float*)m->slab; ex.slab_bytes = (size_t)m->slab_bytes; }
    ex.role = m->gemm_role >= 0 ? m->gemm_role : (ta ? 2 : 1);
    ex.max_wgs = m->ctx->dp_on() ? m->ctx->gemm_max_wgs : 0;
    ex.dp = m->ctx->dp_on();
    ex.sched = &m->ctx->gemm_sched;
    CHECK_RC(gemm_run(m->ctx->stream, m->dtype, ta, tb, M, N, K, A, lda, B, ldb, C, ldc, bias, act, aux, ldaux, resid, ldr,
                      out_fp32, splitk, p_drop, m->drop_seed(), rng_stream, flags, ex));
    if (det && colsum) CHECK_RC(colsum_det(m, C, ldc, colsum, M, N));
    return CMP_OK;
}

__global__ void rows_copy_kernel(const uint4* __restrict__ src, uint4* __restrict__ dst, int B, int Tn, int w, int sT, int s0,
                                 int src_ld, int dT, int d0, int dst_ld) {
    const int64_t n = (int64_t)B * Tn * w;
    for (int64_t i = (int64_t)blockIdx.x * blockDim.x + threadIdx.x; i < n; i += (int64_t)gridDim.x * blockDim.x) {
        const int c = (int)(i % w);
        const int t = (int)((i / w) % Tn);
        const int b = (int)(i / ((int64_t)w * Tn));
        dst[((int64_t)b * dT + d0 + t) * dst_ld + c] = src[((int64_t)b * sT + s0 + t) * src_ld + c];
    }
}
static int rows_copy(cmp_model* m, const void* src, void* dst, int B, int Tn, int width, int sT, int s0, int src_w, int dT, int d0,
                     int dst_w) {
    const int es = (int)m->es, w = width * es / 16;
    const int64_t n = (int64_t)B * Tn * w;
    rows_copy_kernel<<<(int)std::min<int64_t>(cdiv64(n, 256), 4096), 256, 0, m->ctx->stream>>>(
        (const uint4*)src, (uint4*)dst, B, Tn, w, sT, s0, src_w * es / 16, dT, d0, dst_w * es / 16);
    KERNEL_CHECK();
    return CMP_OK;
}

static float attn_scale(const cmp_model* m) { return m->cfg.scale_attention ? 1.0f / sqrtf((float)m->Dl) : 1.0f; }

int model_forward(cmp_model* m, const int32_t* x_dev, int B, int T, bool training, int64_t step, int past_len) {
    Range range_("composer.forward");
    hipStream_t s = m->ctx->stream;
    struct RoleGuard {
        cmp_model* m;
        RoleGuard(cmp_model* mm) : m(mm) { m->gemm_role = 0; }
        ~RoleGuard() { m->gemm_role = -1; }
    } role_guard(m);
    const int E = m->E, Ea = m->Ea, M = B * T, dt = m->dtype;
    const float pr = training ? m->cfg.resid_dropout : 0.f;
    const float pa = training ? m->cfg.attn_dropout : 0.f;
    const bool ln = m->cfg.use_layer_norm != 0;
    const int Tp = past_len, Tt = past_len + T;
    m->lastB = B; m->lastT = Tt; m->last_past = Tp;
    m->fwd_gen += 1;
    const bool fused = ln_fused_ok(m, M, Tp, training);
    m->fused_last = fused;
    if (fused)
        CHECK_RC(embed_fwd_stats_run(s, x_dev, m->P + m->off_wte, m->P + m->off_wpe, m->xs[0], m->act[0].ln1_part, B, T, E, 0, pr,
                                     m->drop_seed(), drop_stream(step, 0, 0)));
    else
        CHECK_RC(embed_fwd_run(s, x_dev, m->P + m->off_wte, m->P + m->off_wpe, m->xs[0], B, T, E, Tp, dt, pr, m->drop_seed(),
                               drop_stream(step, 0, 0), m->fwd_pos_ids, m->fwd_type_ids));
    CHECK_RC(refresh_transposed_weights(m, fused));
    const bool wt = m->ST != nullptr;
    auto W = [&](int64_t off) { return wt ? (const void*)(m->ST + off) : m->w(off); };
    static const int alt_mode = [] { const char* e = getenv("COMPOSER_GEMM_ALT"); return e ? atoi(e) : 1; }();
    const int RV[4] = {alt_mode == 2 ? GEMM_REV : 0, alt_mode == 1 ? GEMM_REV : 0, alt_mode == 2 ? GEMM_REV : 0, alt_mode == 1 ? GEMM_REV : 0};
    PROF_START(9, s);
    for (int i = 0; fused && i < m->L; i++) {
        const LayerOff& o = m->lo[i];
        LayerAct& a = m->act[i];
        const float* fold = m->lnfold + i * m->fold_stride;
        LnEpi l;
        l.in_part = a.ln1_part; l.np = E / 256; l.eps = m->cfg.ln_eps; l.cs = fold;
        CHECK_RC(gemm(m, 0, 1, M, 3 * E, E, m->xs[i], E, W(o.attn_w), E, a.qkv, 3 * E, fold + 3 * E, 0, nullptr, 0, nullptr, 0, 0, 1, 0.f,
                      0, RV[0], nullptr, &l));
        CHECK_RC(attn_fwd_run(s, a.qkv, a.att, a.lse, B, Tt, m->H, m->D, attn_scale(m), dt, pa, m->drop_seed(), drop_stream(step, i, 1),
                              nullptr));
        l = LnEpi();
        l.in_part = a.ln1_part; l.np = E / 256; l.eps = m->cfg.ln_eps; l.gamma = m->P + o.ln1_g; l.beta = m->P + o.ln1_b;
        l.out_part = a.ln2_part;
        CHECK_RC(gemm(m, 0, 1, M, E, E, a.att, E, W(o.proj_w), E, a.r, E, m->P + o.proj_b, 0, nullptr, 0, m->xs[i], E, 0, 1, pr,
                      drop_stream(step, i, 2), RV[1], nullptr, &l));
        l = LnEpi();
        l.in_part = a.ln2_part; l.np = E / 256; l.eps = m->cfg.ln_eps; l.cs = fold + 6 * E;
        CHECK_RC(gemm(m, 0, 1, M, 4 * E, E, a.r, E, W(o.fc_w), E, a.g, 4 * E, fold + 10 * E, 1, training ? a.fc : nullptr, 4 * E, nullptr,
                      0, 0, 1, 0.f, 0, RV[2], nullptr, &l));
        l = LnEpi();
        l.out_part = i + 1 < m->L ? m->act[i + 1].ln1_part : (training ? nullptr : m->lnf_part);
        CHECK_RC(gemm(m, 0, 1, M, E, 4 * E, a.g, 4 * E, W(o.pr_w), 4 * E, m->xs[i + 1], E, m->P + o.pr_b, 0, nullptr, 0, a.r, E, 0, 1, pr,
                      drop_stream(step, i, 3), RV[3], nullptr, l.out_part ? &l : nullptr));
    }
    for (int i = 0; !fused && i < m->L; i++) {
        const LayerOff& o = m->lo[i];
        LayerAct& a = m->act[i];
        if (ln)
            CHECK_RC(cmp_k_layernorm_fwd(s, m->xs[i], m->P + o.ln1_g, m->P + o.ln1_b, a.u, a.ln1_mean, a.ln1_rstd, M, E,
                                         m->cfg.ln_eps, dt));
        CHECK_RC(gemm(m, 0, wt, M, 3 * Ea, E, a.u, E, W(o.attn_w), wt ? E : 3 * Ea, Tp ? m->dqkv : a.qkv, 3 * Ea, m->P + o.attn_b, 0,
                      nullptr, 0, nullptr, 0, 0, 1, 0.f, 0));
        if (Tp) CHECK_RC(rows_copy(m, m->dqkv, a.qkv, B, T, 3 * Ea, T, 0, 3 * Ea, Tt, Tp, 3 * Ea));
        CHECK_RC(attn_fwd_run(s, a.qkv, a.att, a.lse, B, Tt, m->H, m->D, attn_scale(m), dt, pa, m->drop_seed(),
                              drop_stream(step, i, 1), m->fwd_amask));
        if (m->fwd_probs_out) {
            CHECK_RC(attn_probs_run(s, a.qkv, a.lse, m->fwd_amask, m->fwd_probs_dev, B, Tp, Tt, m->H, m->D, attn_scale(m), dt, pa,
                                    m->drop_seed(), drop_stream(step, i, 1)));
            HIP_CHECK(hipMemcpyAsync(m->fwd_probs_out[i], m->fwd_probs_dev, (size_t)B * m->H * T * Tt * 4, hipMemcpyDeviceToHost, s));
            HIP_CHECK(hipStreamSynchronize(s));
        }
        const void* att = a.att;
        if (Tp) { CHECK_RC(rows_copy(m, a.att, m->tmpE, B, T, Ea, Tt, Tp, Ea, T, 0, Ea)); att = m->tmpE; }
        CHECK_RC(gemm(m, 0, wt, M, E, Ea, att, Ea, W(o.proj_w), wt ? Ea : E, a.r, E, m->P + o.proj_b, 0, nullptr, 0, a.u, E, 0, 1, pr,
                      drop_stream(step, i, 2)));
        if (ln)
            CHECK_RC(cmp_k_layernorm_fwd(s, a.r, m->P + o.ln2_g, m->P + o.ln2_b, a.n, a.ln2_mean, a.ln2_rstd, M, E,
                                         m->cfg.ln_eps, dt));
        CHECK_RC(gemm(m, 0, wt, M, 4 * E, E, a.n, E, W(o.fc_w), wt ? E : 4 * E, a.g, 4 * E, m->P + o.fc_b, 1, training ? a.fc : nullptr,
                      4 * E, nullptr, 0, 0, 1, 0.f, 0));
        CHECK_RC(gemm(m, 0, wt, M, E, 4 * E, a.g, 4 * E, W(o.pr_w), wt ? 4 * E : E, m->xs[i + 1], E, m->P + o.pr_b, 0, nullptr, 0, a.r, E,
                      0, 1, pr, drop_stream(step, i, 3)));
    }
    PROF_STOP(9, s, (double)M * m->L * (24.0 * E * E + 2.0 * E * Tt), 0.0);
    static const bool lnf_fold_on = [] { const char* e = getenv("COMPOSER_LNF_FOLD"); return !(e && e[0] == '0'); }();
    if (fused && !training && lnf_fold_on) {
        LnEpi l;
        l.in_part = m->lnf_part; l.np = E / 256; l.eps = m->cfg.ln_eps; l.cs = m->lnf_fold;
        m->hf_valid = false;
        CHECK_RC(gemm(m, 0, 1, M, m->V, E, m->xs[m->L], E, m->wte_lnf, E, m->logits, m->ldz, m->lnf_fold + m->lnf_npad, 0, nullptr, 0, nullptr,
                      0, 1, 1, 0.f, 0, CMP_GEMM_TILE256, nullptr, &l));
        return CMP_OK;
    }
    CHECK_RC(cmp_k_layernorm_fwd(s, m->xs[m->L], m->P + m->off_lnf_g, m->P + m->off_lnf_b, m->hf, m->lnf_mean, m->lnf_rstd, M,
                                 E, m->cfg.ln_eps, dt));
    m->hf_valid = true;
    CHECK_RC(gemm(m, 0, 1, M, m->V, E, m->hf, E, m->w(m->off_wte), E, m->logits, m->ldz, nullptr, 0, nullptr, 0, nullptr, 0, 1,
                  1, 0.f, 0));
    return CMP_OK;
}

static int loss(cmp_model* m, const int32_t* y_dev, int M, bool want_grad) {
    Range range_("composer.loss");
    hipStream_t s = m->ctx->stream;
    CHECK_RC(cmp_k_softmax_xent(s, m->logits, m->ldz, y_dev, want_grad ? m->dlogits : nullptr, m->row_loss, m->row_correct, M,
                                m->V, 1.0f / (float)M, m->dtype));
    CHECK_RC(launch_metrics_reduce(s, m->row_loss, m->row_correct, M, m->metrics));
    return CMP_OK;
}

static int wgrad_splits(int K, int M, int N) {
    const int tiles256 = cdiv(M, 256) * cdiv(N, 256);
    int s;
    if (tiles256 >= 8) s = std::max(1, 256 / tiles256);
    else s = std::max(1, 768 / std::max(1, cdiv(M, 128) * cdiv(N, 128)));
    return std::min(s, std::max(1, K / 256));
}

static int adam_range(cmp_model* m, hipStream_t s, int64_t begin, int64_t end, float lr, int64_t step, float gscale) {
    return cmp_k_adam(s, m->P + begin, m->G + begin, m->Am + begin, m->Av + begin, m->S ? (void*)(m->S + begin) : nullptr, end - begin, lr,
                      0.9f, 0.999f, 1e-7f, step, gscale);
}

static int bucket_ready(cmp_model* m, int ev, int64_t begin, int64_t end, float lr, bool update) {
    cmp_ctx* c = m->ctx;
    if (!c->dp_on()) return CMP_OK;
    HIP_CHECK(hipEventRecord(m->bucket_ev[ev], c->stream));
    HIP_CHECK(hipStreamWaitEvent(c->comm_stream, m->bucket_ev[ev], 0));
    CHECK_RC(dp_allreduce(c, m->G + begin, (size_t)(end - begin)));
    m->dp_bytes_step += (end - begin) * 4;
    m->dp_msgs_step += 1;
    if (update && m->clip_norm > 0.f) {
        const int64_t ns = grad_sumsq_slots(end - begin);
        CMP_REQUIRE(m->clip_slots && m->clip_slots_used + ns <= m->clip_slots_cap, "train step: gradient-norm workspace too small");
        CHECK_RC(grad_sumsq_run(c->comm_stream, m->G + begin, end - begin, m->clip_slots + m->clip_slots_used));
        m->clip_slots_used += ns;
    } else if (update) {
        CHECK_RC(adam_range(m, c->comm_stream, begin, end, lr, m->iterations + 1, 1.0f / (float)(c->nranks * m->accum_steps)));
        m->dp_buckets_updated += 1;
    }
    return CMP_OK;
}

static int backward(cmp_model* m, const int32_t* x_dev, int B, int T, int64_t step, bool allreduce, float lr = 0.f, bool update = false,
                    bool zero = true) {
    Range range_("composer.backward");
    hipStream_t s = m->ctx->stream;
    const int E = m->E, Ea = m->Ea, M = B * T, dt = m->dtype, V = m->V;
    const float pr = m->cfg.resid_dropout, pa = m->cfg.attn_dropout;
    const bool ln = m->cfg.use_layer_norm != 0;
    if (zero) HIP_CHECK(hipMemsetAsync(m->G, 0, (size_t)m->total * 4, s));
    {
        const int t256 = cdiv(V, 256) * cdiv(E, 256);
        const bool p4 = dt == CMP_BF16 && t256 <= 64 && M >= 65536 && M % 32 == 0;
        const int tsplit = p4 ? std::max(2, std::min(256 / t256, M / 1024)) : std::max(2, wgrad_splits(M, V, E));
        const int tflags = p4 ? CMP_GEMM_P4 : 0;
        CHECK_RC(gemm(m, 1, 0, V, E, M, m->dlogits, m->ldz, m->hf, E, m->G + m->off_wte, E, nullptr, 0, nullptr, 0, nullptr, 0, 1,
                      tsplit, 0.f, 0, tflags));
    }
    CHECK_RC(gemm(m, 0, 0, M, E, V, m->dlogits, m->ldz, m->w(m->off_wte), E, m->tmpE, E, nullptr, 0, nullptr, 0, nullptr, 0, 0,
                  1, 0.f, 0, CMP_GEMM_KPAD_ZERO));
    CHECK_RC(ln_bwd(m, m->tmpE, m->xs[m->L], m->P + m->off_lnf_g, m->lnf_mean, m->lnf_rstd, nullptr, m->dx,
                    m->G + m->off_lnf_g, m->G + m->off_lnf_b, M, m->dmask, m->G + m->lo[m->L - 1].pr_b, pr,
                    drop_stream(step, m->L - 1, 3)));
    bool dmo_ready = true;
    const bool fused = m->fused_last;
    const bool raw = fused && m->ln_fused_mode == 3;
    if (raw) CHECK_RC(ln_stats_merge_run(s, m->ln_sites, 2 * m->L, E / 256, m->cfg.ln_eps, M));
    void* const dmk[2] = {m->dmask, m->dmask3};
    int cur = 0;
    if (allreduce) CHECK_RC(bucket_ready(m, m->L, m->off_lnf_g, m->total, lr, update));
    const bool grouped = ln && dt == CMP_BF16;
    CMP_REQUIRE(!fused || grouped, "backward: the fused block path needs the grouped weight-gradient order");
    if (grouped && (int)m->wgrad_groups.size() != m->L) m->wgrad_groups.resize(m->L);
    for (int i = m->L - 1; i >= 0; i--) {
        const LayerOff& o = m->lo[i];
        LayerAct& a = m->act[i];
        bool group_now = grouped;
        const void* dmo = m->dx;
        if (fused) {
            dmo = dmk[cur];
        } else if (pr > 0.f) {
            if (!dmo_ready) CHECK_RC(drop_apply(m, m->dx, m->dmask, (int64_t)M * E, pr, drop_stream(step, i, 3)));
            dmo = m->dmask;
        }
        LnBwdFused fz;
        fz.np = E / 256; fz.eps = m->cfg.ln_eps;
        auto wgrad = [&](int Mw, int Nw, const void* A, int lda, const void* Bm, int ldb, float* Cw) {
            return gemm(m, 1, 0, Mw, Nw, M, A, lda, Bm, ldb, Cw, Nw, nullptr, 0, nullptr, 0, nullptr, 0, 1, std::max(2, wgrad_splits(M, Mw, Nw)), 0.f, 0);
        };
        if (!group_now) CHECK_RC(wgrad(4 * E, E, a.g, 4 * E, dmo, E, m->G + o.pr_w));
        if (!dmo_ready) CHECK_RC(colsum_any(m, dmo, E, m->G + o.pr_b, M, E));
        LnEpi ls;
        ls.np = E / 256; ls.eps = m->cfg.ln_eps; ls.scale = 1;
        ls.in_part = a.ln2_part;
        CHECK_RC(gemm(m, 0, 1, M, 4 * E, E, dmo, E, m->w(o.pr_w), E, m->dfc, 4 * E, nullptr, 2, a.fc, 4 * E, nullptr, 0, 0, 1,
                      0.f, 0, 0, m->G + o.fc_b, raw ? &ls : nullptr));
        if (!group_now) CHECK_RC(wgrad(E, 4 * E, a.n, E, m->dfc, 4 * E, m->G + o.fc_w));
        void* const dao_mask = group_now ? m->dmask2 : m->dmask;
        if (ln) {
            CHECK_RC(gemm(m, 0, 1, M, E, 4 * E, m->dfc, 4 * E, m->w(o.fc_w), 4 * E, m->tmpE, E, nullptr, 0, nullptr, 0, nullptr,
                          0, 0, 1, 0.f, 0));
            fz.part = a.ln2_part; fz.beta = m->P + o.ln2_b; fz.yout = a.n;
            CHECK_RC(ln_bwd(m, m->tmpE, a.r, m->P + o.ln2_g, a.ln2_mean, a.ln2_rstd, m->dx, m->dr, m->G + o.ln2_g, m->G + o.ln2_b, M,
                            dao_mask, m->G + o.proj_b, pr, drop_stream(step, i, 2), (fused && !raw) ? &fz : nullptr, raw));
        } else {
            CHECK_RC(gemm(m, 0, 1, M, E, 4 * E, m->dfc, 4 * E, m->w(o.fc_w), 4 * E, m->dr, E, nullptr, 0, nullptr, 0, m->dx, E,
                          0, 1, 0.f, 0));
        }
        const void* dao = m->dr;
        if (fused) {
            dao = dao_mask;
        } else if (pr > 0.f) {
            if (!ln) CHECK_RC(drop_apply(m, m->dr, m->dmask, (int64_t)M * E, pr, drop_stream(step, i, 2)));
            dao = dao_mask;
        }
        if (!group_now) CHECK_RC(wgrad(Ea, E, a.att, Ea, dao, E, m->G + o.proj_w));
        if (!ln) CHECK_RC(colsum_any(m, dao, E, m->G + o.proj_b, M, E));
        CHECK_RC(gemm(m, 0, 1, M, Ea, E, dao, E, m->w(o.proj_w), E, m->tmpE, Ea, nullptr, 0, nullptr, 0, nullptr, 0, 0, 1, 0.f,
                      0));
        const bool det = m->slab != nullptr;
        AttnLnRows alr;
        if (raw) alr.rstd = a.ln1_rstd;
        CHECK_RC(attn_bwd_run(s, a.qkv, a.att, m->tmpE, a.lse, m->delta, m->dqkv, B, T, m->H, m->D, attn_scale(m),
                              dt, pa, m->drop_seed(), drop_stream(step, i, 1), det ? nullptr : m->G + o.attn_b, alr));
        if (det) CHECK_RC(colsum_det(m, m->dqkv, 3 * Ea, m->G + o.attn_b, M, 3 * Ea));
        auto group_launch = [&]() -> int {
            const WgradProblem wp[4] = {
                {a.g, 4 * E, dmo, E, m->G + o.pr_w, E, 4 * E, E},
                {raw ? a.r : a.n, E, m->dfc, 4 * E, m->G + o.fc_w, 4 * E, E, 4 * E},
                {a.att, Ea, dao, E, m->G + o.proj_w, E, Ea, E},
                {raw ? m->xs[i] : a.u, E, m->dqkv, 3 * Ea, m->G + o.attn_w, 3 * Ea, E, 3 * Ea}};
            GemmExtra ex;
            ex.role = 2;
            ex.max_wgs = m->ctx->dp_on() ? m->ctx->gemm_max_wgs : 0;
            ex.dp = m->ctx->dp_on();
            ex.sched = &m->ctx->gemm_sched;
            if (m->slab) ex.wws = &m->wgrad_ws;
            bool handled = false;
            CHECK_RC(wgrad_group_run(s, &m->wgrad_groups[i], wp, 4, M, ex, &handled));
            if (!handled) {
                CHECK_RC(wgrad(4 * E, E, a.g, 4 * E, dmo, E, m->G + o.pr_w));
                CHECK_RC(wgrad(E, 4 * E, wp[1].A, E, m->dfc, 4 * E, m->G + o.fc_w));
                CHECK_RC(wgrad(Ea, E, a.att, Ea, dao, E, m->G + o.proj_w));
                CHECK_RC(wgrad(E, 3 * Ea, wp[3].A, E, m->dqkv, 3 * Ea, m->G + o.attn_w));
            }
            if (raw) {
                CHECK_RC(wgrad_ln_fix_run(s, m->G + o.fc_w, E, 4 * E, m->P + o.ln2_g, m->P + o.ln2_b, m->G + o.fc_b,
                                          m->G + o.attn_w, E, 3 * E, m->P + o.ln1_g, m->P + o.ln1_b, m->G + o.attn_b));
            }
            return CMP_OK;
        };
        if (group_now && (!fused || raw)) {
            CHECK_RC(group_launch());
        } else if (!group_now) {
            CHECK_RC(wgrad(E, 3 * Ea, a.u, E, m->dqkv, 3 * Ea, m->G + o.attn_w));
        }
        if (ln) {
            ls.in_part = a.ln1_part;
            CHECK_RC(gemm(m, 0, 1, M, E, 3 * Ea, m->dqkv, 3 * Ea, m->w(o.attn_w), 3 * Ea, m->tmpE, E, nullptr, 0, nullptr, 0, m->dr,
                          E, 0, 1, 0.f, 0, 0, nullptr, raw ? &ls : nullptr));
            fz.part = a.ln1_part; fz.beta = m->P + o.ln1_b; fz.yout = a.u;
            void* const next_mask = fused ? dmk[cur ^ 1] : m->dmask;
            CHECK_RC(ln_bwd(m, m->tmpE, m->xs[i], m->P + o.ln1_g, a.ln1_mean, a.ln1_rstd, nullptr, m->dx, m->G + o.ln1_g,
                            m->G + o.ln1_b, M, i > 0 ? next_mask : nullptr, i > 0 ? m->G + m->lo[i - 1].pr_b : nullptr, pr,
                            drop_stream(step, i > 0 ? i - 1 : 0, 3), (fused && !raw) ? &fz : nullptr, raw));
            if (fused) {
                if (!raw) CHECK_RC(group_launch());
                cur ^= 1;
            }
            dmo_ready = true;
        } else {
            dmo_ready = false;
            CHECK_RC(gemm(m, 0, 1, M, E, 3 * Ea, m->dqkv, 3 * Ea, m->w(o.attn_w), 3 * Ea, m->dx, E, nullptr, 0, nullptr, 0, m->dr, E,
                          0, 1, 0.f, 0));
        }
        if (allreduce) CHECK_RC(bucket_ready(m, i, o.begin, o.end, lr, update));
    }
    CHECK_RC(embed_bwd_run(s, x_dev, m->dx, m->G + m->off_wte, m->G + m->off_wpe, B, T, E, 0, dt, pr, m->drop_seed(),
                           drop_stream(step, 0, 0), m->slab ? V : 0, (float*)m->slab, (size_t)m->slab_bytes, V, m->embed_ws,
                           m->embed_ws_words));
    if (allreduce) CHECK_RC(bucket_ready(m, m->L + 1, 0, m->lo[0].begin, lr, update));
    return CMP_OK;
}

__global__ void dp_metrics_pack_kernel(const Metrics* __restrict__ mt, float* __restrict__ dp) {
    if (threadIdx.x == 0) { dp[0] = mt->loss_mean; dp[1] = mt->acc; dp[2] = 1.0f; dp[3] = 0.f; }
}
__global__ void dp_metrics_unpack_kernel(Metrics* __restrict__ mt, const float* __restrict__ dp) {
    if (threadIdx.x == 0 && dp[2] > 0.f) { mt->loss_mean = dp[0] / dp[2]; mt->acc = dp[1] / dp[2]; }
}
static int dp_metrics_begin(cmp_model* m) {
    cmp_ctx* c = m->ctx;
    if (!c->dp_on()) return CMP_OK;
    dp_metrics_pack_kernel<<<1, 64, 0, c->stream>>>(m->metrics, m->dp_metrics);
    KERNEL_CHECK();
    HIP_CHECK(hipEventRecord(m->metrics_ev, c->stream));
    HIP_CHECK(hipStreamWaitEvent(c->comm_stream, m->metrics_ev, 0));
    CHECK_RC(dp_allreduce(c, m->dp_metrics, 3));
    m->dp_bytes_step = 12;
    m->dp_msgs_step = 1;
    return CMP_OK;
}

static int dp_fold(cmp_model* m, int slot, bool all) {
    for (int i = 0; i < cmp_model::DP_RING; i++) {
        if (!(all || i == slot) || !m->dp_wait_used[i]) continue;
        HIP_CHECK(hipEventSynchronize(m->dp_wait_b[i]));
        float ms = 0.f;
        HIP_CHECK(hipEventElapsedTime(&ms, m->dp_wait_a[i], m->dp_wait_b[i]));
        m->dp_exposed_ms += ms;
        m->dp_folded += 1;
        m->dp_wait_used[i] = false;
    }
    return CMP_OK;
}

static int dp_metrics_end(cmp_model* m) {
    cmp_ctx* c = m->ctx;
    if (!c->dp_on()) return CMP_OK;
    HIP_CHECK(hipEventRecord(m->comm_done, c->comm_stream));
    HIP_CHECK(hipStreamWaitEvent(c->stream, m->comm_done, 0));
    dp_metrics_unpack_kernel<<<1, 64, 0, c->stream>>>(m->metrics, m->dp_metrics);
    KERNEL_CHECK();
    return CMP_OK;
}

static int adam_clipped(cmp_model* m, hipStream_t s, int nslots, float lr, int64_t step, float gscale) {
    CHECK_RC(grad_clip_finish_run(s, m->clip_slots, nslots, gscale, m->clip_norm, m->clip_out));
    return cmp_k_adam_dev(s, m->P, m->G, m->Am, m->Av, m->S ? (void*)m->S : nullptr, m->total, lr, 0.9f, 0.999f, 1e-7f, step,
                          &m->clip_out->factor);
}

static int adam(cmp_model* m, float lr) {
    Range range_("composer.adam");
    cmp_ctx* c = m->ctx;
    const bool clip = m->clip_norm > 0.f;
    const float gscale = 1.0f / (float)(c->nranks * m->accum_steps);
    if (clip && c->dp_on()) {
        CHECK_RC(adam_clipped(m, c->comm_stream, (int)m->clip_slots_used, lr, m->iterations + 1, gscale));
        m->dp_buckets_updated = m->L + 2;
    }
    m->iterations += 1;
    m->param_version += 1;
    if (c->dp_on()) {
        const int slot = (int)(m->dp_steps % cmp_model::DP_RING);
        CHECK_RC(dp_fold(m, slot, false));
        if (!m->dp_wait_a[slot]) {
            HIP_CHECK(hipEventCreate(&m->dp_wait_a[slot]));
            HIP_CHECK(hipEventCreate(&m->dp_wait_b[slot]));
        }
        HIP_CHECK(hipEventRecord(m->comm_done, c->comm_stream));
        HIP_CHECK(hipEventRecord(m->dp_wait_a[slot], c->stream));
        HIP_CHECK(hipStreamWaitEvent(c->stream, m->comm_done, 0));
        HIP_CHECK(hipEventRecord(m->dp_wait_b[slot], c->stream));
        m->dp_wait_used[slot] = true;
        m->dp_steps += 1;
        dp_metrics_unpack_kernel<<<1, 64, 0, c->stream>>>(m->metrics, m->dp_metrics);
        KERNEL_CHECK();
        return CMP_OK;
    }
    if (clip) {
        CHECK_RC(grad_sumsq_run(c->stream, m->G, m->total, m->clip_slots));
        return adam_clipped(m, c->stream, (int)grad_sumsq_slots(m->total), lr, m->iterations, gscale);
    }
    return adam_range(m, c->stream, 0, m->total, lr, m->iterations, gscale);
}

extern "C" int cmp_dp_stats(cmp_model* m, int reset, int64_t* steps, double* exposed_ms, int64_t* bytes_per_step, int* msgs_per_step) {
    CMP_REQUIRE(m, "dp_stats: null model");
    HIP_CHECK(hipSetDevice(m->ctx->device));
    CHECK_RC(dp_fold(m, -1, true));
    if (steps) *steps = m->dp_folded;
    if (exposed_ms) *exposed_ms = m->dp_exposed_ms;
    if (bytes_per_step) *bytes_per_step = m->ctx->dp_on() ? m->dp_bytes_step : 0;
    if (msgs_per_step) *msgs_per_step = m->ctx->dp_on() ? m->dp_msgs_step : 0;
    if (reset) { m->dp_steps = 0; m->dp_folded = 0; m->dp_exposed_ms = 0.0; }
    return CMP_OK;
}

extern "C" int cmp_dp_rccl_version(int* version) {
    CMP_REQUIRE(version, "dp_rccl_version: null");
    NCCL_CHECK(ncclGetVersion(version));
    return CMP_OK;
}

extern "C" int cmp_dp_allreduce_pattern(cmp_model* m, int reps, double* ms, int64_t* bytes_per_rep, int* msgs_per_rep) {
    CMP_REQUIRE(m && reps > 0 && ms, "dp_allreduce_pattern: bad arguments");
    cmp_ctx* c = m->ctx;
    CMP_REQUIRE(c->dp_on(), "dp_allreduce_pattern: communicator not initialised");
    HIP_CHECK(hipSetDevice(c->device));
    HIP_CHECK(hipStreamSynchronize(c->stream));
    HIP_CHECK(hipMemsetAsync(m->G, 0, (size_t)m->total * 4, c->comm_stream));
    HIP_CHECK(hipMemsetAsync(m->dp_metrics, 0, 16, c->comm_stream));
    hipEvent_t a = nullptr, b = nullptr;
    HIP_CHECK(hipEventCreate(&a));
    HIP_CHECK(hipEventCreate(&b));
    int64_t bytes = 0;
    int msgs = 0, rc = CMP_OK;
    auto one = [&](float* p, int64_t n) { if (rc == CMP_OK) { rc = dp_allreduce(c, p, (size_t)n); bytes += n * 4; msgs += 1; } };
    for (int r = -1; r < reps && rc == CMP_OK; r++) {
        if (r == 0) { HIP_CHECK(hipEventRecord(a, c->comm_stream)); bytes = 0; msgs = 0; }
        one(m->dp_metrics, 3);
        one(m->G + m->off_lnf_g, m->total - m->off_lnf_g);
        for (int i = m->L - 1; i >= 0; i--) one(m->G + m->lo[i].begin, m->lo[i].end - m->lo[i].begin);
        one(m->G, m->lo[0].begin);
    }
    if (rc == CMP_OK) {
        HIP_CHECK(hipEventRecord(b, c->comm_stream));
        HIP_CHECK(hipEventSynchronize(b));
        float t = 0.f;
        HIP_CHECK(hipEventElapsedTime(&t, a, b));
        *ms = t;
    } else {
        (void)hipStreamSynchronize(c->comm_stream);
    }
    (void)hipEventDestroy(a);
    (void)hipEventDestroy(b);
    if (bytes_per_rep) *bytes_per_rep = bytes / reps;
    if (msgs_per_rep) *msgs_per_rep = msgs / reps;
    return rc;
}

extern "C" int cmp_model_path_info(cmp_model* m, int* fused, int64_t* wgrad_table_builds) {
    CMP_REQUIRE(m, "model_path_info: null model");
    if (fused) *fused = m->fused_last ? 1 : 0;
    if (wgrad_table_builds) {
        int64_t n = 0;
        for (const WgradGroup& g : m->wgrad_groups) n += g.rebuilds;
        *wgrad_table_builds = n;
    }
    return CMP_OK;
}

static int fetch_metrics(cmp_model* m) {
    HIP_CHECK(hipMemcpyAsync(m->metrics_host, m->metrics, sizeof(Metrics), hipMemcpyDeviceToHost, m->ctx->stream));
    return CMP_OK;
}

__global__ void sanitize_ids_kernel(const int32_t* __restrict__ x, const int32_t* __restrict__ y, int32_t* __restrict__ xo,
                                    int32_t* __restrict__ yo, int n, int V, int* __restrict__ bad) {
    int nbad = 0;
    for (int i = blockIdx.x * blockDim.x + threadIdx.x; i < n; i += gridDim.x * blockDim.x) {
        const int a = x[i], b = y[i];
        nbad += (a < 0 || a >= V) + (b < 0 || b >= V);
        xo[i] = min(max(a, 0), V - 1);
        yo[i] = min(max(b, 0), V - 1);
    }
    if (nbad) atomicAdd(bad, nbad);
}

static int accum_shape_check(cmp_model* m, int B, int T) {
    CMP_REQUIRE(m->accum_pending == 0 || (B == m->accumB && T == m->accumT),
                "train step: micro-step %d of %d has shape [%d,%d], the group's first had [%d,%d]", m->accum_pending + 1, m->accum_steps, B,
                T, m->accumB, m->accumT);
    return CMP_OK;
}

static int fetch_clip(cmp_model* m, int slot) {
    if (!m->last_has_norm) return CMP_OK;
    HIP_CHECK(hipMemcpyAsync(&m->clip_host[slot], m->clip_out, sizeof(GradClipStats), hipMemcpyDeviceToHost, m->ctx->stream));
    return CMP_OK;
}

extern "C" int cmp_train_options(cmp_model* m, float clip_norm, int accum_steps) {
    CMP_REQUIRE(m, "train_options: null model");
    CMP_REQUIRE(clip_norm >= 0.f, "train_options: clip_norm %g is not 0 (off), positive or +inf (measure only)", (double)clip_norm);
    CMP_REQUIRE(accum_steps >= 1, "train_options: accum_steps %d must be at least 1", accum_steps);
    CMP_REQUIRE(accum_steps == 1 || m->ln_fused_mode != 3, "train_options: COMPOSER_LN_FUSED=3 transforms the weight gradients in place and "
                "cannot accumulate (accum_steps %d)", accum_steps);
    HIP_CHECK(hipSetDevice(m->ctx->device));
    if (clip_norm > 0.f && !m->clip_slots) {
        const int64_t cap = grad_sumsq_slots(m->total) + m->L + 2;
        CHECK_RC(dev_alloc(m, &m->clip_out, sizeof(GradClipStats)));
        HIP_CHECK(hipHostMalloc((void**)&m->clip_host, sizeof(GradClipStats) * (1 + cmp_model::STAGES), hipHostMallocDefault));
        memset(m->clip_host, 0, sizeof(GradClipStats) * (1 + cmp_model::STAGES));
        CHECK_RC(dev_alloc(m, &m->clip_slots, (size_t)cap * 8));
        m->clip_slots_cap = cap;
    }
    m->clip_norm = clip_norm;
    m->accum_steps = accum_steps;
    m->accum_pending = 0;
    return CMP_OK;
}
extern "C" int cmp_train_options_get(cmp_model* m, float* clip_norm, int* accum_steps, int* pending_micro_steps) {
    CMP_REQUIRE(m, "train_options_get: null model");
    if (clip_norm) *clip_norm = m->clip_norm;
    if (accum_steps) *accum_steps = m->accum_steps;
    if (pending_micro_steps) *pending_micro_steps = m->accum_pending;
    return CMP_OK;
}
extern "C" int cmp_train_grad_stats(cmp_model* m, float* norm, float* scale) {
    CMP_REQUIRE(m, "train_grad_stats: null model");
    HIP_CHECK(hipSetDevice(m->ctx->device));
    HIP_CHECK(hipStreamSynchronize(m->ctx->stream));
    if (norm) *norm = m->last_has_norm ? (float)m->clip_host[0].norm : NAN;
    if (scale) *scale = m->last_has_norm ? m->clip_host[0].scale : 1.0f;
    return CMP_OK;
}

static int train_step_enqueue(cmp_model* m, const int32_t* x_dev, const int32_t* y_dev, int B, int T, float lr) {
    CMP_REQUIRE(lr >= 0.f && lr == lr, "train step: learning rate %g is not a non-negative number", (double)lr);
    CMP_REQUIRE(!m->poisoned, "train step: an earlier data-parallel step failed after some gradient buckets had been all-reduced and "
                "applied (parameters are partially stepped and may differ between replicas): reload a checkpoint on every rank");
    CHECK_RC(accum_shape_check(m, B, T));
    const int64_t step = m->iterations;
    const int k = m->accum_steps, j = m->accum_pending;
    const bool final_ = j == k - 1;
    const uint32_t seed_mix = m->ctx->seed_mix;
    if (k > 1) m->ctx->seed_mix = mix32((uint32_t)(m->ctx->mask_rank * k + j));
    m->last_has_norm = false;
    m->dp_buckets_updated = 0;
    m->clip_slots_used = 0;
    int rc = model_forward(m, x_dev, B, T, true, step);
    if (rc == CMP_OK) rc = loss(m, y_dev, B * T, true);
    if (rc == CMP_OK) rc = dp_metrics_begin(m);
    if (rc == CMP_OK) rc = backward(m, x_dev, B, T, step, final_, lr, final_, j == 0);
    m->ctx->seed_mix = seed_mix;
    if (rc == CMP_OK) rc = final_ ? adam(m, lr) : dp_metrics_end(m);
    if (rc == CMP_OK) {
        m->accum_pending = final_ ? 0 : j + 1;
        m->accumB = B; m->accumT = T;
        m->last_has_norm = final_ && m->clip_norm > 0.f;
    } else {
        m->accum_pending = 0;
    }
    if (rc != CMP_OK && m->ctx->dp_on()) {
        cmp_ctx* c = m->ctx;
        if (hipEventRecord(m->comm_done, c->comm_stream) == hipSuccess) (void)hipStreamWaitEvent(c->stream, m->comm_done, 0);
        else (void)hipStreamSynchronize(c->comm_stream);
        (void)hipGetLastError();
        if (m->dp_buckets_updated > 0) {
            m->poisoned = true;
            m->param_version += 1;
            m->st_state = 0;
            m->reload_seen.assign(m->params.size(), 0);
        }
    }
    return rc;
}

extern "C" int cmp_train_step_dev(cmp_model* m, const void* x_dev, const void* y_dev, int B, int T, float lr) {
    CMP_REQUIRE(m && x_dev && y_dev, "train_step_dev: null argument");
    CHECK_RC(accum_shape_check(m, B, T));
    HIP_CHECK(hipSetDevice(m->ctx->device));
    CHECK_RC(ensure_workspace(m, B, T));
    hipStream_t s = m->ctx->stream;
    HIP_CHECK(hipMemsetAsync(&m->metrics->bad_ids, 0, sizeof(int), s));
    sanitize_ids_kernel<<<std::min(cdiv(B * T, 256), 1024), 256, 0, s>>>((const int32_t*)x_dev, (const int32_t*)y_dev, m->x_dev,
                                                                         m->y_dev, B * T, m->V, &m->metrics->bad_ids);
    KERNEL_CHECK();
    CHECK_RC(train_step_enqueue(m, m->x_dev, m->y_dev, B, T, lr));
    CHECK_RC(fetch_metrics(m));
    CHECK_RC(fetch_clip(m, 0));
    return CMP_OK;
}

extern "C" int cmp_train_step_graph_probe(cmp_model* m, const void* x_dev, const void* y_dev, int B, int T, int* kernels, int* others,
                                         int replay_reps, float* replay_ms);
extern "C" int cmp_train_step_launches(cmp_model* m, const void* x_dev, const void* y_dev, int B, int T, int* kernels, int* others) {
    return cmp_train_step_graph_probe(m, x_dev, y_dev, B, T, kernels, others, 0, nullptr);
}
extern "C" int cmp_train_step_graph_probe(cmp_model* m, const void* x_dev, const void* y_dev, int B, int T, int* kernels, int* others,
                                         int replay_reps, float* replay_ms) {
    CMP_REQUIRE(m && x_dev && y_dev && kernels, "train_step_launches: null argument");
    CMP_REQUIRE(!m->ctx->dp_on(), "train_step_launches: not available with a communicator");
    HIP_CHECK(hipSetDevice(m->ctx->device));
    CHECK_RC(ensure_workspace(m, B, T));
    hipStream_t s = m->ctx->stream;
    HIP_CHECK(hipStreamSynchronize(s));
    const int64_t it = m->iterations, pv = m->param_version, gen = m->fwd_gen, stv = m->st_version;
    const int sts = m->st_state, lB = m->lastB, lT = m->lastT, lP = m->last_past;
    const bool fl = m->fused_last, hv = m->hf_valid, hn = m->last_has_norm;
    const int ap = m->accum_pending, aB = m->accumB, aT = m->accumT;
    m->accum_pending = m->accum_steps - 1;
    m->accumB = B; m->accumT = T;
    HIP_CHECK(hipStreamBeginCapture(s, hipStreamCaptureModeThreadLocal));
    const int rc = train_step_enqueue(m, (const int32_t*)x_dev, (const int32_t*)y_dev, B, T, 0.f);
    hipGraph_t g = nullptr;
    const hipError_t e = hipStreamEndCapture(s, &g);
    m->iterations = it; m->param_version = pv; m->fwd_gen = gen; m->st_version = stv; m->st_state = sts;
    m->lastB = lB; m->lastT = lT; m->last_past = lP; m->fused_last = fl; m->hf_valid = hv;
    m->accum_pending = ap; m->accumB = aB; m->accumT = aT; m->last_has_norm = hn;
    if (rc != CMP_OK) { if (g) (void)hipGraphDestroy(g); return rc; }
    HIP_CHECK(e);
    size_t n = 0;
    HIP_CHECK(hipGraphGetNodes(g, nullptr, &n));
    std::vector<hipGraphNode_t> nodes(n);
    if (n) HIP_CHECK(hipGraphGetNodes(g, nodes.data(), &n));
    int nk = 0, no = 0;
    for (size_t i = 0; i < n; i++) {
        hipGraphNodeType ty;
        if (hipGraphNodeGetType(nodes[i], &ty) == hipSuccess && ty == hipGraphNodeTypeKernel) nk++; else no++;
    }
    if (replay_reps > 0 && replay_ms) {
        hipGraphExec_t ge = nullptr;
        hipError_t e2 = hipGraphInstantiate(&ge, g, nullptr, nullptr, 0);
        if (e2 == hipSuccess) {
            hipEvent_t a, b;
            (void)hipEventCreate(&a); (void)hipEventCreate(&b);
            for (int i = 0; i < 3 && e2 == hipSuccess; i++) e2 = hipGraphLaunch(ge, s);
            (void)hipEventRecord(a, s);
            for (int i = 0; i < replay_reps && e2 == hipSuccess; i++) e2 = hipGraphLaunch(ge, s);
            (void)hipEventRecord(b, s);
            if (e2 == hipSuccess) e2 = hipEventSynchronize(b);
            float ms = 0.f;
            if (e2 == hipSuccess) (void)hipEventElapsedTime(&ms, a, b);
            *replay_ms = ms / (float)replay_reps;
            (void)hipEventDestroy(a); (void)hipEventDestroy(b);
            (void)hipGraphExecDestroy(ge);
        }
        if (e2 != hipSuccess) { (void)hipGraphDestroy(g); HIP_CHECK(e2); }
    }
    (void)hipGraphDestroy(g);
    *kernels = nk;
    if (others) *others = no;
    return CMP_OK;
}

extern "C" int cmp_train_metrics(cmp_model* m, float* loss_out, float* acc_out) {
    CMP_REQUIRE(m, "train_metrics: null model");
    HIP_CHECK(hipStreamSynchronize(m->ctx->stream));
    if (loss_out) *loss_out = m->metrics_host->loss_mean;
    if (acc_out) *acc_out = m->metrics_host->acc;
    CMP_REQUIRE(m->metrics_host->bad_ids == 0, "train step: %d token ids outside [0, %d) were passed by device pointer (clamped)",
                m->metrics_host->bad_ids, m->V);
    return CMP_OK;
}

static int check_host_ids(cmp_model* m, const int32_t* ids, int64_t n, const char* what) {
    uint32_t mx = 0;
    for (int64_t i = 0; i < n; i++) mx = std::max(mx, (uint32_t)ids[i]);
    if (mx < (uint32_t)m->V) return CMP_OK;
    for (int64_t i = 0; i < n; i++)
        CMP_REQUIRE(ids[i] >= 0 && ids[i] < m->V, "%s: token id %d at flat index %lld is outside [0, %d)", what, ids[i], (long long)i, m->V);
    return CMP_OK;
}

static int upload_xy(cmp_model* m, const int32_t* x, const int32_t* y, int B, int T, int past_len = 0) {
    CHECK_RC(ensure_workspace(m, B, T + past_len));
    CHECK_RC(check_host_ids(m, x, (int64_t)B * T, "input ids"));
    if (y) CHECK_RC(check_host_ids(m, y, (int64_t)B * T, "target ids"));
    HIP_CHECK(hipMemsetAsync(&m->metrics->bad_ids, 0, sizeof(int), m->ctx->stream));
    HIP_CHECK(hipMemcpyAsync(m->x_dev, x, (size_t)B * T * 4, hipMemcpyHostToDevice, m->ctx->stream));
    if (y) HIP_CHECK(hipMemcpyAsync(m->y_dev, y, (size_t)B * T * 4, hipMemcpyHostToDevice, m->ctx->stream));
    return CMP_OK;
}

static int ensure_stages(cmp_model* m, int64_t tokens) {
    if (m->stage_cap >= tokens) return CMP_OK;
    CMP_REQUIRE(m->stage_cap == 0, "train_step_async: staging was sized for %lld tokens", (long long)m->stage_cap);
    const int64_t cap = std::max<int64_t>(tokens, (int64_t)m->capB * m->capT);
    if (!m->stage_metrics) {
        HIP_CHECK(hipHostMalloc((void**)&m->stage_metrics, sizeof(Metrics) * cmp_model::STAGES, hipHostMallocDefault));
        memset(m->stage_metrics, 0, sizeof(Metrics) * cmp_model::STAGES);
    }
    for (int i = 0; i < cmp_model::STAGES; i++) {
        if (!m->stage_host[i]) HIP_CHECK(hipHostMalloc((void**)&m->stage_host[i], (size_t)cap * 8, hipHostMallocDefault));
        if (!m->stage_dev[i]) CHECK_RC(dev_alloc(m, &m->stage_dev[i], (size_t)cap * 8));
        if (!m->stage_uploaded[i]) HIP_CHECK(hipEventCreateWithFlags(&m->stage_uploaded[i], hipEventDisableTiming));
        if (!m->stage_done[i]) HIP_CHECK(hipEventCreateWithFlags(&m->stage_done[i], hipEventDisableTiming));
    }
    m->stage_cap = cap;
    return CMP_OK;
}

extern "C" int cmp_train_step_async(cmp_model* m, const int32_t* x, const int32_t* y, int B, int T, float lr, int64_t* ticket) {
    CMP_REQUIRE(m && x && y && ticket, "train_step_async: null argument");
    CHECK_RC(accum_shape_check(m, B, T));
    HIP_CHECK(hipSetDevice(m->ctx->device));
    CHECK_RC(ensure_workspace(m, B, T));
    const int64_t n = (int64_t)B * T;
    CHECK_RC(ensure_stages(m, n));
    CHECK_RC(check_host_ids(m, x, n, "input ids"));
    CHECK_RC(check_host_ids(m, y, n, "target ids"));
    const int64_t tk = m->next_ticket;
    const int slot = (int)(tk % cmp_model::STAGES);
    if (m->stage_ticket[slot] >= 0) HIP_CHECK(hipEventSynchronize(m->stage_done[slot]));
    memcpy(m->stage_host[slot], x, (size_t)n * 4);
    memcpy(m->stage_host[slot] + n, y, (size_t)n * 4);
    cmp_ctx* c = m->ctx;
    HIP_CHECK(hipMemcpyAsync(m->stage_dev[slot], m->stage_host[slot], (size_t)n * 8, hipMemcpyHostToDevice, c->copy_stream));
    HIP_CHECK(hipEventRecord(m->stage_uploaded[slot], c->copy_stream));
    HIP_CHECK(hipStreamWaitEvent(c->stream, m->stage_uploaded[slot], 0));
    HIP_CHECK(hipMemsetAsync(&m->metrics->bad_ids, 0, sizeof(int), c->stream));
    CHECK_RC(train_step_enqueue(m, m->stage_dev[slot], m->stage_dev[slot] + n, B, T, lr));
    HIP_CHECK(hipMemcpyAsync(&m->stage_metrics[slot], m->metrics, sizeof(Metrics), hipMemcpyDeviceToHost, c->stream));
    HIP_CHECK(hipMemcpyAsync(m->metrics_host, m->metrics, sizeof(Metrics), hipMemcpyDeviceToHost, c->stream));
    CHECK_RC(fetch_clip(m, 0));
    CHECK_RC(fetch_clip(m, 1 + slot));
    m->stage_has_norm[slot] = m->last_has_norm;
    HIP_CHECK(hipEventRecord(m->stage_done[slot], c->stream));
    m->stage_ticket[slot] = tk;
    m->next_ticket = tk + 1;
    *ticket = tk;
    return CMP_OK;
}

extern "C" int cmp_train_metrics_wait_ex(cmp_model* m, int64_t ticket, float* loss_out, float* acc_out, float* norm, float* scale) {
    CHECK_RC(cmp_train_metrics_wait(m, ticket, loss_out, acc_out));
    const int slot = (int)(ticket % cmp_model::STAGES);
    const bool has = m->stage_has_norm[slot];
    if (norm) *norm = has ? (float)m->clip_host[1 + slot].norm : NAN;
    if (scale) *scale = has ? m->clip_host[1 + slot].scale : 1.0f;
    return CMP_OK;
}
extern "C" int cmp_train_metrics_wait(cmp_model* m, int64_t ticket, float* loss_out, float* acc_out) {
    CMP_REQUIRE(m, "train_metrics_wait: null model");
    const int slot = (int)(ticket % cmp_model::STAGES);
    CMP_REQUIRE(ticket >= 0 && m->stage_cap > 0 && m->stage_ticket[slot] == ticket,
                "train_metrics_wait: ticket %lld is not in flight (at most %d steps are)", (long long)ticket, cmp_model::STAGES);
    HIP_CHECK(hipSetDevice(m->ctx->device));
    HIP_CHECK(hipEventSynchronize(m->stage_done[slot]));
    if (loss_out) *loss_out = m->stage_metrics[slot].loss_mean;
    if (acc_out) *acc_out = m->stage_metrics[slot].acc;
    return CMP_OK;
}

extern "C" int cmp_train_step(cmp_model* m, const int32_t* x, const int32_t* y, int B, int T, float lr, float* loss_out,
                              float* acc_out) {
    CMP_REQUIRE(m && x && y, "train_step: null argument");
    CHECK_RC(accum_shape_check(m, B, T));
    HIP_CHECK(hipSetDevice(m->ctx->device));
    CHECK_RC(upload_xy(m, x, y, B, T));
    CHECK_RC(train_step_enqueue(m, m->x_dev, m->y_dev, B, T, lr));
    CHECK_RC(fetch_metrics(m));
    CHECK_RC(fetch_clip(m, 0));
    if (loss_out || acc_out) CHECK_RC(cmp_train_metrics(m, loss_out, acc_out));
    return CMP_OK;
}

extern "C" int cmp_loss_and_grads(cmp_model* m, const int32_t* x, const int32_t* y, int B, int T, float* loss_out,
                                  float* acc_out) {
    CMP_REQUIRE(m && x && y, "loss_and_grads: null argument");
    HIP_CHECK(hipSetDevice(m->ctx->device));
    CHECK_RC(upload_xy(m, x, y, B, T));
    const int64_t step = m->iterations;
    m->accum_pending = 0;
    CHECK_RC(model_forward(m, m->x_dev, B, T, true, step));
    CHECK_RC(loss(m, m->y_dev, B * T, true));
    CHECK_RC(backward(m, m->x_dev, B, T, step, false));
    CHECK_RC(fetch_metrics(m));
    CHECK_RC(cmp_train_metrics(m, loss_out, acc_out));
    return CMP_OK;
}

extern "C" int cmp_eval_step(cmp_model* m, const int32_t* x, const int32_t* y, int B, int T, double* loss_sum,
                             int64_t* correct, int64_t* count) {
    CMP_REQUIRE(m && x && y, "eval_step: null argument");
    HIP_CHECK(hipSetDevice(m->ctx->device));
    CHECK_RC(upload_xy(m, x, y, B, T));
    CHECK_RC(model_forward(m, m->x_dev, B, T, false, 0));
    CHECK_RC(loss(m, m->y_dev, B * T, false));
    CHECK_RC(fetch_metrics(m));
    HIP_CHECK(hipStreamSynchronize(m->ctx->stream));
    if (loss_sum) *loss_sum = m->metrics_host->loss_sum;
    if (correct) *correct = m->metrics_host->correct;
    if (count) *count = (int64_t)B * T;
    return CMP_OK;
}

template <typename T_>
__global__ void present_gather_kernel(const T_* __restrict__ qkv, float* __restrict__ out, int B, int T, int H, int D, int Dk) {
    const int E = H * Dk;
    const int64_t n = (int64_t)2 * B * H * T * D;
    for (int64_t i = (int64_t)blockIdx.x * blockDim.x + threadIdx.x; i < n; i += (int64_t)gridDim.x * blockDim.x) {
        const int d = (int)(i % D);
        const int t = (int)((i / D) % T);
        const int h = (int)((i / ((int64_t)D * T)) % H);
        const int b = (int)((i / ((int64_t)D * T * H)) % B);
        const int kv = (int)(i / ((int64_t)D * T * H * B));
        out[i] = to_f32<T_>(qkv[((int64_t)b * T + t) * 3 * E + (1 + kv) * E + h * Dk + d]);
    }
}
static int io_scratch(cmp_model* m, int slot, size_t bytes, void** out) {
    if (m->io_buf_bytes[slot] < bytes) {
        if (m->io_buf[slot]) {
            HIP_CHECK(hipStreamSynchronize(m->ctx->stream));
            for (auto& p : m->allocs) if (p == m->io_buf[slot]) { p = nullptr; break; }
            (void)hipFree(m->io_buf[slot]);
            m->io_buf[slot] = nullptr; m->io_buf_bytes[slot] = 0;
        }
        void* q = nullptr;
        const size_t want = std::max(bytes, (size_t)1 << 16);
        HIP_CHECK(hipMalloc(&q, want));
        m->allocs.push_back(q);
        m->io_buf[slot] = q; m->io_buf_bytes[slot] = want;
    }
    *out = m->io_buf[slot];
    return CMP_OK;
}
extern "C" int cmp_forward_generation(cmp_model* m, int64_t* gen) {
    CMP_REQUIRE(m && gen, "forward_generation: null argument");
    *gen = m->fwd_gen;
    return CMP_OK;
}
extern "C" int cmp_present_get(cmp_model* m, int layer, int B, int T, float* host_out);
extern "C" int cmp_present_get_at(cmp_model* m, int layer, int B, int T, int64_t generation, float* host_out) {
    CMP_REQUIRE(m, "present_get_at: null argument");
    CMP_REQUIRE(generation == m->fwd_gen, "present_get_at: these presents belong to forward pass %lld, the activations held are those of "
                "pass %lld (a later forward / train step / decode prefill overwrote them; read presents before the next pass)",
                (long long)generation, (long long)m->fwd_gen);
    return cmp_present_get(m, layer, B, T, host_out);
}
extern "C" int cmp_present_get(cmp_model* m, int layer, int B, int T, float* host_out) {
    CMP_REQUIRE(m && host_out, "present_get: null argument");
    CMP_REQUIRE(layer >= 0 && layer < m->L, "present_get: layer %d outside [0, %d)", layer, m->L);
    CMP_REQUIRE(B > 0 && T > 0 && !m->act.empty() && B == m->lastB && T == m->lastT,
                "present_get: the forward pass held is [%d,%d] (batch, past + new positions), not [%d,%d]", m->lastB, m->lastT, B, T);
    HIP_CHECK(hipSetDevice(m->ctx->device));
    const int64_t n = (int64_t)2 * B * m->H * T * m->Dl;
    float* tmp = nullptr;
    CHECK_RC(io_scratch(m, 0, (size_t)n * 4, (void**)&tmp));
    const int grid = (int)std::min<int64_t>(cdiv64(n, 256), 4096);
    if (m->dtype == CMP_BF16) present_gather_kernel<bf16_t><<<grid, 256, 0, m->ctx->stream>>>((const bf16_t*)m->act[layer].qkv, tmp, B, T, m->H, m->Dl, m->D);
    else present_gather_kernel<float><<<grid, 256, 0, m->ctx->stream>>>((const float*)m->act[layer].qkv, tmp, B, T, m->H, m->Dl, m->D);
    KERNEL_CHECK();
    HIP_CHECK(hipMemcpyAsync(host_out, tmp, (size_t)n * 4, hipMemcpyDeviceToHost, m->ctx->stream));
    HIP_CHECK(hipStreamSynchronize(m->ctx->stream));
    return CMP_OK;
}

template <typename T_>
__global__ void hidden_unpack_kernel(const T_* __restrict__ in, float* __restrict__ out, int64_t n) {
    for (int64_t i = (int64_t)blockIdx.x * blockDim.x + threadIdx.x; i < n; i += (int64_t)gridDim.x * blockDim.x) out[i] = to_f32<T_>(in[i]);
}
extern "C" int cmp_hidden_get_at(cmp_model* m, int index, int B, int T, int64_t generation, float* host_out) {
    CMP_REQUIRE(m && host_out, "hidden_get_at: null argument");
    CMP_REQUIRE(index >= 0 && index <= m->L, "hidden_get_at: index %d outside [0, %d]", index, m->L);
    CMP_REQUIRE(generation == m->fwd_gen, "hidden_get_at: these hidden states belong to forward pass %lld, the activations held are "
                "those of pass %lld (a later forward / train step / decode prefill overwrote them)",
                (long long)generation, (long long)m->fwd_gen);
    CMP_REQUIRE(B > 0 && T > 0 && !m->act.empty() && B == m->lastB && T == m->lastT - m->last_past,
                "hidden_get_at: the forward pass held is [%d,%d] (batch, new positions), not [%d,%d]", m->lastB,
                m->lastT - m->last_past, B, T);
    HIP_CHECK(hipSetDevice(m->ctx->device));
    const int64_t n = (int64_t)B * T * m->E;
    if (index == m->L && !m->hf_valid) {
        CHECK_RC(cmp_k_layernorm_fwd(m->ctx->stream, m->xs[m->L], m->P + m->off_lnf_g, m->P + m->off_lnf_b, m->hf, m->lnf_mean, m->lnf_rstd,
                                     B * T, m->E, m->cfg.ln_eps, m->dtype));
        m->hf_valid = true;
    }
    const void* src = index < m->L ? m->xs[index] : m->hf;
    float* tmp = nullptr;
    CHECK_RC(io_scratch(m, 0, (size_t)n * 4, (void**)&tmp));
    const int grid = (int)std::min<int64_t>(cdiv64(n, 256), 4096);
    if (m->dtype == CMP_BF16) hidden_unpack_kernel<bf16_t><<<grid, 256, 0, m->ctx->stream>>>((const bf16_t*)src, tmp, n);
    else hidden_unpack_kernel<float><<<grid, 256, 0, m->ctx->stream>>>((const float*)src, tmp, n);
    KERNEL_CHECK();
    HIP_CHECK(hipMemcpyAsync(host_out, tmp, (size_t)n * 4, hipMemcpyDeviceToHost, m->ctx->stream));
    HIP_CHECK(hipStreamSynchronize(m->ctx->stream));
    return CMP_OK;
}

template <typename T_>
__global__ void past_scatter_kernel(const float* __restrict__ in, T_* __restrict__ qkv, int B, int Tp, int Tt, int H, int D, int Dl) {
    const int E = H * D;
    const int64_t n = (int64_t)2 * B * H * Tp * D, nq = (int64_t)B * Tp * E;
    for (int64_t i = (int64_t)blockIdx.x * blockDim.x + threadIdx.x; i < n + nq; i += (int64_t)gridDim.x * blockDim.x) {
        if (i < n) {
            const int d = (int)(i % D);
            const int t = (int)((i / D) % Tp);
            const int h = (int)((i / ((int64_t)D * Tp)) % H);
            const int b = (int)((i / ((int64_t)D * Tp * H)) % B);
            const int kv = (int)(i / ((int64_t)D * Tp * H * B));
            const float v = d < Dl ? in[((((int64_t)kv * B + b) * H + h) * Tp + t) * Dl + d] : 0.f;
            qkv[((int64_t)b * Tt + t) * 3 * E + (1 + kv) * E + h * D + d] = from_f32<T_>(v);
        } else {
            const int64_t j = i - n;
            const int e = (int)(j % E);
            const int t = (int)((j / E) % Tp);
            const int b = (int)(j / ((int64_t)E * Tp));
            qkv[((int64_t)b * Tt + t) * 3 * E + e] = from_f32<T_>(0.f);
        }
    }
}

__global__ void logits_pack_kernel(const float* __restrict__ z, float* __restrict__ out, int64_t n, int V, int ldz) {
    for (int64_t i = (int64_t)blockIdx.x * blockDim.x + threadIdx.x; i < n; i += (int64_t)gridDim.x * blockDim.x)
        out[i] = z[(i / V) * ldz + (i % V)];
}

extern "C" int cmp_forward(cmp_model* m, const int32_t* x, int B, int T, int past_len, const float* const* past, int training,
                           float* logits_out) {
    return cmp_forward_ex(m, x, B, T, past_len, past, training, nullptr, nullptr, nullptr, nullptr, logits_out);
}

__global__ void attention_mask_term_kernel(const int32_t* __restrict__ mask, float* __restrict__ out, int64_t n) {
    for (int64_t i = (int64_t)blockIdx.x * blockDim.x + threadIdx.x; i < n; i += (int64_t)gridDim.x * blockDim.x)
        out[i] = (1.0f - (float)mask[i]) * -10000.0f;
}

extern "C" int cmp_forward_ex(cmp_model* m, const int32_t* x, int B, int T, int past_len, const float* const* past, int training,
                              const int32_t* position_ids, const int32_t* token_type_ids, const int32_t* attention_mask,
                              float* const* attention_weights_out, float* logits_out) {
    CMP_REQUIRE(m && x && logits_out, "forward: null argument");
    CMP_REQUIRE(past_len >= 0 && (past_len == 0 || past != nullptr), "forward: past_len %d without past tensors", past_len);
    CMP_REQUIRE(T > 0 && T + past_len <= m->W, "forward: positions %d..%d exceed window_size %d (wpe rows, transformer.py:675-679,786)",
                past_len, past_len + T - 1, m->W);
    HIP_CHECK(hipSetDevice(m->ctx->device));
    CHECK_RC(upload_xy(m, x, nullptr, B, T, past_len));
    hipStream_t s = m->ctx->stream;
    struct IdBuf {
        cmp_model* m;
        int32_t* dev = nullptr;
// ... 73 lines not shown
```

include/composer_hip.h:

```cpp
#ifndef COMPOSER_HIP_H
#define COMPOSER_HIP_H

#include <stdint.h>

#ifdef __cplusplus
extern "C" {
#endif

typedef struct cmp_ctx cmp_ctx;
typedef struct cmp_model cmp_model;

enum cmp_status {
    CMP_OK = 0,
    CMP_ERR_INVALID = -1,
    CMP_ERR_HIP = -2,
    CMP_ERR_RCCL = -3,
    CMP_ERR_STATE = -4
};

enum cmp_dtype {
    CMP_FP32 = 0,
    CMP_BF16 = 1
};

enum cmp_decode_mode {
    CMP_DECODE_LITERAL = 0,
    CMP_DECODE_KV = 1
};

typedef struct cmp_model_cfg {
    int32_t vocab_size;
    int32_t embedding_size;
    int32_t window_size;
    int32_t layers;
    int32_t heads;
    float   ln_eps;
    int32_t scale_attention;
    int32_t use_layer_norm;
    float   attn_dropout;
    float   resid_dropout;
    int32_t dtype;
    int32_t max_batch;
    int32_t max_seq;
    uint64_t seed;
} cmp_model_cfg;

const char* cmp_last_error(void);
int cmp_version(void);
const char* cmp_build_key(void);
int cmp_device_count(void);

int cmp_ctx_create(int device, cmp_ctx** out);
int cmp_ctx_destroy(cmp_ctx* ctx);
int cmp_sync(cmp_ctx* ctx);
void* cmp_ctx_stream(cmp_ctx* ctx);

int cmp_dp_unique_id(void* id128);
int cmp_dp_init(cmp_ctx* ctx, int rank, int nranks, const void* id128);
int cmp_dp_allreduce_test(cmp_ctx* ctx, float* host_inout, int n);
typedef int (*cmp_exchange_fn)(void* user, void* dev_f32, int64_t count, void* hip_stream);
int cmp_dp_init_exchange(cmp_ctx* ctx, int rank, int nranks, cmp_exchange_fn fn, void* user);
int cmp_dp_test_hog(cmp_ctx* ctx, int wgs, int usec);
int cmp_dp_set_gemm_cus(cmp_ctx* ctx, int cus);
int cmp_dp_set_mask_rank(cmp_ctx* ctx, int rank);
int cmp_dp_stats(cmp_model* m, int reset, int64_t* steps, double* exposed_ms, int64_t* bytes_per_step, int* msgs_per_step);
int cmp_dp_rccl_version(int* version);
int cmp_dp_allreduce_pattern(cmp_model* m, int reps, double* ms, int64_t* bytes_per_rep, int* msgs_per_rep);

int cmp_model_create(cmp_ctx* ctx, const cmp_model_cfg* cfg, cmp_model** out);
int cmp_model_destroy(cmp_model* m);

int cmp_param_count(cmp_model* m, int* n);
int cmp_param_info(cmp_model* m, int i, const char** name, int* rank, int64_t shape[4], int64_t* numel);
int cmp_param_get(cmp_model* m, const char* name, int kind, float* host, int64_t numel);
int cmp_param_set(cmp_model* m, const char* name, int kind, const float* host, int64_t numel);
int cmp_adam_iter_get(cmp_model* m, int64_t* iterations);
int cmp_adam_iter_set(cmp_model* m, int64_t iterations);

int cmp_train_step(cmp_model* m, const int32_t* x, const int32_t* y, int B, int T, float lr,
                   float* loss, float* acc);
int cmp_train_step_dev(cmp_model* m, const void* x_dev, const void* y_dev, int B, int T, float lr);
int cmp_train_metrics(cmp_model* m, float* loss, float* acc);
int cmp_train_step_launches(cmp_model* m, const void* x_dev, const void* y_dev, int B, int T, int* kernels, int* others);
int cmp_train_step_graph_probe(cmp_model* m, const void* x_dev, const void* y_dev, int B, int T, int* kernels, int* others,
                               int replay_reps, float* replay_ms);
int cmp_train_step_async(cmp_model* m, const int32_t* x, const int32_t* y, int B, int T, float lr, int64_t* ticket);
int cmp_train_metrics_wait(cmp_model* m, int64_t ticket, float* loss, float* acc);
int cmp_train_options(cmp_model* m, float clip_norm, int accum_steps);
int cmp_train_options_get(cmp_model* m, float* clip_norm, int* accum_steps, int* pending_micro_steps);
int cmp_train_grad_stats(cmp_model* m, float* norm, float* scale);
int cmp_train_metrics_wait_ex(cmp_model* m, int64_t ticket, float* loss, float* acc, float* norm, float* scale);
int cmp_loss_and_grads(cmp_model* m, const int32_t* x, const int32_t* y, int B, int T,
                       float* loss, float* acc);

int cmp_eval_step(cmp_model* m, const int32_t* x, const int32_t* y, int B, int T,
                  double* loss_sum, int64_t* correct, int64_t* count);

int cmp_forward_logits(cmp_model* m, const int32_t* x, int B, int T, float* logits_out);
int cmp_forward(cmp_model* m, const int32_t* x, int B, int T, int past_len, const float* const* past, int training,
                float* logits_out);
int cmp_forward_ex(cmp_model* m, const int32_t* x, int B, int T, int past_len, const float* const* past, int training,
                   const int32_t* position_ids, const int32_t* token_type_ids, const int32_t* attention_mask,
                   float* const* attention_weights_out, float* logits_out);
int cmp_present_get(cmp_model* m, int layer, int B, int T, float* host_out);
int cmp_forward_generation(cmp_model* m, int64_t* generation);
int cmp_present_get_at(cmp_model* m, int layer, int B, int T, int64_t generation, float* host_out);
int cmp_hidden_get_at(cmp_model* m, int index, int B, int T, int64_t generation, float* host_out);

int cmp_decode_begin(cmp_model* m, const int32_t* prompt, int P, int mode, float temperature, uint64_t seed);
int cmp_decode_steps(cmp_model* m, int n, int32_t* ids_out);
int cmp_decode_logits_get(cmp_model* m, float* host_out);
int cmp_decode_begin_slide(cmp_model* m, const int32_t* prompt, int P, int keep, float temperature, uint64_t seed);
int cmp_decode_slide_stats(cmp_model* m, int batched, int64_t* row_slides, int64_t* forward_calls);
int cmp_k_sample(void* stream, const float* logits, int V, float temperature, uint64_t seed, uint32_t counter0, int n,
                 int32_t* ids_out);

int cmp_k_sample_ex(void* stream, const float* logits, int V, float temperature, int top_k, float top_p, uint64_t seed,
                    uint32_t counter0, int n, int32_t* ids_out);
int cmp_decode_begin_ex(cmp_model* m, const int32_t* prompt, int P, int mode, int keep, float temperature, int top_k, float top_p,
                        uint64_t seed);

int cmp_decode_batch_begin(cmp_model* m, const int32_t* prompts, const int32_t* lens, int B, int ld, int mode,
                           float temperature, uint64_t seed);
int cmp_decode_batch_begin_slide(cmp_model* m, const int32_t* prompts, const int32_t* lens, int B, int ld, int keep,
                                 float temperature, uint64_t seed);
int cmp_decode_batch_steps(cmp_model* m, int n, int32_t* ids_out);
int cmp_decode_batch_logits_get(cmp_model* m, float* host_out);
int cmp_k_sample_rows(void* stream, const float* logits, int ldz, int B, int V, float temperature, uint64_t seed,
                      uint32_t counter, int32_t* ids_out);
int cmp_decode_batch_begin_ex(cmp_model* m, const int32_t* prompts, const int32_t* lens, int B, int ld, int mode, int keep,
                              const float* temperature, const int32_t* top_k, const float* top_p, uint64_t seed);
int cmp_k_sample_rows_ex(void* stream, const float* logits, int ldz, int B, int V, const float* temperature, const int32_t* top_k,
                         const float* top_p, uint64_t seed, uint32_t counter, int32_t* ids_out);

int cmp_prof_begin(int cls);
int cmp_prof_end(double* total_ms, int64_t* launches, double* work);
int cmp_prof_end2(double* total_ms, int64_t* launches, double* work, double* bytes);
int cmp_prof_pause(void);
int cmp_prof_resume(void);

int cmp_k_embed_fwd(void* stream, const int32_t* ids, const float* wte, const float* wpe, void* out,
                    int B, int T, int E, int pos0, int dtype, float p_drop, uint64_t seed, uint32_t rng_stream);
int cmp_k_embed_bwd(void* stream, const int32_t* ids, const void* dh, float* dwte, float* dwpe,
                    int B, int T, int E, int pos0, int dtype, float p_drop, uint64_t seed, uint32_t rng_stream);
int cmp_k_embed_bwd_v(void* stream, const int32_t* ids, const void* dh, float* dwte, float* dwpe,
                      int B, int T, int E, int pos0, int dtype, float p_drop, uint64_t seed, uint32_t rng_stream, int V);
int cmp_k_layernorm_fwd(void* stream, const void* x, const float* gamma, const float* beta, void* y,
                        float* mean, float* rstd, int rows, int E, float eps, int dtype);
int cmp_k_layernorm_bwd(void* stream, const void* dy, const void* x, const float* gamma, const float* mean,
                        const float* rstd, const void* resid, void* dx, float* dgamma, float* dbeta,
                        void* ws, int rows, int E, int dtype);
int64_t cmp_k_layernorm_bwd_ws(int rows, int E);
int cmp_k_layernorm_bwd_fused(void* stream, const void* dy, const void* x, const float* gamma, const float* mean,
                              const float* rstd, const void* resid, void* dx, float* dgamma, float* dbeta,
                              void* ws, int rows, int E, int dtype, void* dmask, float* colsum, float p_drop,
                              uint64_t seed, uint32_t rng_stream);
int cmp_k_gemm(void* stream, int dtype, int ta, int tb, int M, int N, int K,
               const void* A, int lda, const void* Bm, int ldb, void* C, int ldc,
               const float* bias, int act, void* aux, int ldaux, const void* resid, int ldr,
               int out_fp32, int splitk, float p_drop, uint64_t seed, uint32_t rng_stream, int flags);
#define CMP_GEMM_KPAD_ZERO 1
#define CMP_GEMM_GENERIC 2
#define CMP_GEMM_TILE128 4
#define CMP_GEMM_TILE256 8
#define CMP_GEMM_P4 16
#define CMP_GEMM_P4_128 32
int cmp_k_wgrad_group(void* stream, int nprob, const void* const* A, const int* lda, const void* const* B, const int* ldb,
                      float* const* C, const int* ldc, const int* M, const int* N, int K);
int cmp_k_embed_fwd_stats(void* stream, const int32_t* ids, const float* wte, const float* wpe, void* out, float* part,
                          int B, int T, int E, int pos0, float p_drop, uint64_t seed, uint32_t rng_stream);
int cmp_k_ln_fold_prep(void* stream, const float* W, const float* bias, const float* gamma, const float* beta, void* WT,
                       float* cs, float* bias_out, int E, int N);
int cmp_gemm_ln_next(const float* in_part, int np, float eps, const float* cs, const float* gamma, const float* beta,
                     float* out_part);
int cmp_gemm_ln_scale_next(const float* in_part, int np, float eps);
int cmp_k_ln_stats_merge(void* stream, const float* part, int np, float eps, float* mean, float* rstd, int rows);
int cmp_attn_bwd_ln_next(const float* rstd);
int cmp_k_layernorm_bwd_prescaled(void* stream, const void* dy_scaled, const void* x, const float* gamma, const float* mean,
                                  const float* rstd, const void* resid, void* dx, float* dgamma, float* dbeta, void* ws,
                                  int rows, int E, void* dmask, float* colsum, float p_drop, uint64_t seed, uint32_t rng_stream);
int cmp_k_wgrad_ln_fix(void* stream, float* G, int rows, int cols, const float* gamma, const float* beta, const float* colsum);
int cmp_k_layernorm_bwd_parts(void* stream, const void* dy, const void* x, const float* gamma, const float* beta,
                              const float* part, float eps, const void* resid, void* dx, void* yout, float* dgamma,
                              float* dbeta, void* ws, int rows, int E, void* dmask, float* colsum, float p_drop,
                              uint64_t seed, uint32_t rng_stream);
int cmp_model_path_info(cmp_model* m, int* fused, int64_t* wgrad_table_builds);
int cmp_gemm_set_workspace(void* ws_dev, int64_t bytes);
int cmp_gemm_colsum_next(float* out);
int cmp_gemm_set_stamps(void* dev_buf);
int cmp_k_colsum(void* stream, const void* X, int ldx, float* out, int rows, int cols, int dtype);
int cmp_k_attn_fwd(void* stream, const void* qkv, void* o, float* lse, int B, int T, int H, int D,
                   int scale, int dtype, float p_drop, uint64_t seed, uint32_t rng_stream);
int cmp_attn_bwd_bias_next(float* out);
int cmp_k_attn_bwd(void* stream, const void* qkv, const void* o, const void* d_o, const float* lse,
                   float* delta_ws, void* dqkv, int B, int T, int H, int D, int scale, int dtype,
                   float p_drop, uint64_t seed, uint32_t rng_stream);
int cmp_k_softmax_xent(void* stream, const float* logits, int ldz, const int32_t* y, void* dlogits,
                       float* row_loss, int32_t* row_correct, int rows, int V, float inv_n, int dtype);
int cmp_k_adam(void* stream, float* p, const float* g, float* m, float* v, void* shadow_bf16,
               int64_t n, float lr, float beta1, float beta2, float eps, int64_t step, float grad_scale);
int cmp_k_adam_dev(void* stream, float* p, const float* g, float* m, float* v, void* shadow_bf16,
                   int64_t n, float lr, float beta1, float beta2, float eps, int64_t step, const float* factor_dev);
int64_t cmp_k_grad_clip_ws(int64_t n);
int cmp_k_grad_clip(void* stream, const float* g, int64_t n, float gscale, float clip_norm, void* ws, void* out);

#ifdef __cplusplus
}
#endif
#endif
```

Measured before the change: 5.063 million tokens/s.

## Fuse LM-head GEMM with softmax cross-entropy and fuse transposed shadow write into Adam

Adds a loss_head kernel that computes the vocab logits GEMM (hidden × tied embedding, V≤512) and the softmax cross-entropy, argmax and bf16 dlogits in one pass. This avoids materialising fp32 logits and the separate softmax_xent read. The Adam step also gains a segmented kernel that writes a transposed bf16 shadow copy of the parameters alongside the update, so a later transpose pass can be skipped. The cost is a large register and LDS footprint, plus extra bookkeeping for shadow-state validity.

```diff
diff --git a/composer_amd/_lib.py b/composer_amd/_lib.py
--- a/composer_amd/_lib.py
+++ b/composer_amd/_lib.py
@@ -120,6 +120,9 @@
     "cmp_attn_bwd_bias_next": (_i, [_P]),
     "cmp_k_attn_bwd": (_i, [_P, _P, _P, _P, _P, _P, _P, _i, _i, _i, _i, _i, _i, _f, _u64, _u32]),
     "cmp_k_softmax_xent": (_i, [_P, _P, _i, _P, _P, _P, _P, _i, _i, _f, _i]),
+    "cmp_shadow_get": (_i, [_P, C.c_char_p, _i, _P, _i64, C.POINTER(_i)]),
+    "cmp_k_logits_xent_fused": (_i, [_i, _i, _i, _i, _i, _i]),
+    "cmp_k_logits_xent": (_i, [_P, _P, _i, _P, _i, _P, _P, _i, _P, _P, _i, _i, _i, _f, _i, _P]),
     "cmp_k_adam": (_i, [_P, _P, _P, _P, _P, _P, _i64, _f, _f, _f, _f, _i64, _f]),
     "cmp_k_adam_dev": (_i, [_P, _P, _P, _P, _P, _P, _i64, _f, _f, _f, _f, _i64, _P]),
     "cmp_k_grad_clip_ws": (_i64, [_i64]),
@@ -127,7 +130,8 @@
 }
 
 _ADDED_LATER = {"cmp_gemm_ln_scale_next", "cmp_attn_bwd_ln_next", "cmp_k_layernorm_bwd_prescaled", "cmp_k_wgrad_ln_fix", "cmp_k_ln_stats_merge", "cmp_dp_rccl_version", "cmp_dp_allreduce_pattern", "cmp_dp_init_exchange", "cmp_train_step_graph_probe", "cmp_train_step_launches", "cmp_k_embed_fwd_stats", "cmp_k_ln_fold_prep", "cmp_gemm_ln_next", "cmp_k_layernorm_bwd_parts", "cmp_model_path_info", "cmp_forward_ex", "cmp_hidden_get_at", "cmp_dp_stats", "cmp_prof_end2", "cmp_prof_pause", "cmp_prof_resume", "cmp_k_wgrad_group", "cmp_k_embed_bwd_v", "cmp_decode_batch_begin", "cmp_decode_batch_steps", "cmp_k_sample_rows", "cmp_decode_logits_get", "cmp_decode_batch_logits_get", "cmp_k_sample_ex", "cmp_k_sample_rows_ex", "cmp_decode_begin_ex", "cmp_decode_batch_begin_ex", "cmp_train_options",
-                "cmp_train_options_get", "cmp_train_grad_stats", "cmp_train_metrics_wait_ex", "cmp_k_adam_dev", "cmp_k_grad_clip_ws", "cmp_k_grad_clip"}
+                "cmp_train_options_get", "cmp_train_grad_stats", "cmp_train_metrics_wait_ex", "cmp_k_adam_dev", "cmp_k_grad_clip_ws", "cmp_k_grad_clip",
+                "cmp_k_logits_xent_fused", "cmp_k_logits_xent", "cmp_shadow_get"}
 
 _lib = None
 
diff --git a/composer_amd/build.py b/composer_amd/build.py
--- a/composer_amd/build.py
+++ b/composer_amd/build.py
@@ -11,7 +11,7 @@
 LIBDIR = os.path.join(HERE, "lib")
 LIB = os.path.join(LIBDIR, "libcomposer_hip.so")
 ROOT = os.path.dirname(HERE)
-SOURCES = ["elementwise.hip", "gemm.hip", "attention.hip", "model.hip", "decode.hip", "decode_batch.hip"]
+SOURCES = ["elementwise.hip", "gemm.hip", "attention.hip", "model.hip", "decode.hip", "decode_batch.hip", "loss_head.hip"]
 ARCH = "gfx950"
 FLAGS = ["--offload-arch=" + ARCH, "-O3", "-fPIC", "-std=c++17", "-Wno-unused-value", "-Wno-inline-asm", "-I" + os.path.join(ROOT, "include")]
 SOURCE_FLAGS = {"attention.hip": ["-fno-slp-vectorize"]}
diff --git a/composer_amd/csrc/elementwise.hip b/composer_amd/csrc/elementwise.hip
--- a/composer_amd/csrc/elementwise.hip
+++ b/composer_amd/csrc/elementwise.hip
@@ -808,6 +808,71 @@
     ADAM_LOOP()
 }
 #undef ADAM_LOOP
+
+template <bool DEV>
+__global__ __launch_bounds__(256) void adam_segs_kernel(float* __restrict__ p, const float* __restrict__ g, float* __restrict__ m,
+                                                        float* __restrict__ v, bf16_t* __restrict__ shadow,
+                                                        const AdamSeg* __restrict__ segs, float alpha, float beta1, float beta2, float eps,
+                                                        float gscale_arg, const float* __restrict__ factor_dev) {
+    __shared__ __attribute__((aligned(16))) bf16_t tile[64][72];
+    const float gscale = DEV ? *factor_dev : gscale_arg;
+    const AdamSeg d = segs[blockIdx.y];
+    const int tid = threadIdx.x;
+    auto update4 = [&](int64_t e) -> bf16x4 {
+        f32x4 pv = *reinterpret_cast<f32x4*>(p + e);
+        const f32x4 gv = *reinterpret_cast<const f32x4*>(g + e);
+        f32x4 mv = *reinterpret_cast<f32x4*>(m + e);
+        f32x4 vv = *reinterpret_cast<f32x4*>(v + e);
+#pragma unroll
+        for (int j = 0; j < 4; j++) {
+            float gg = gv[j] * gscale;
+            mv[j] = beta1 * mv[j] + (1.0f - beta1) * gg;
+            vv[j] = beta2 * vv[j] + (1.0f - beta2) * gg * gg;
+            pv[j] = pv[j] - alpha * mv[j] / (sqrtf(vv[j]) + eps);
+        }
+        *reinterpret_cast<f32x4*>(p + e) = pv;
+        *reinterpret_cast<f32x4*>(m + e) = mv;
+        *reinterpret_cast<f32x4*>(v + e) = vv;
+        bf16x4 sv;
+#pragma unroll
+        for (int j = 0; j < 4; j++) sv[j] = (bf16_t)pv[j];
+        *reinterpret_cast<bf16x4*>(shadow + e) = sv;
+        return sv;
+    };
+    if (d.rows == 0) {
+        const int n4 = d.cols >> 2;
+        for (int i = blockIdx.x * 256 + tid; i < n4; i += gridDim.x * 256) (void)update4(d.off + 4 * (int64_t)i);
+        return;
+    }
+    const int tiles_c = (d.cols + 63) >> 6, ntiles = ((d.rows + 63) >> 6) * tiles_c;
+    const int tx = tid & 15, ty = tid >> 4;
+    const bool vec = (d.rows & 7) == 0 && (d.dst_ld & 7) == 0;
+    for (int t = blockIdx.x; t < ntiles; t += gridDim.x) {
+        const int tr = (t / tiles_c) << 6, tc = (t % tiles_c) << 6;
+#pragma unroll
+        for (int j = 0; j < 4; j++) {
+            const int rl = ty + 16 * j, r = tr + rl, c = tc + 4 * tx;
+            bf16x4 sv = {(bf16_t)0.f, (bf16_t)0.f, (bf16_t)0.f, (bf16_t)0.f};
+            if (r < d.rows && c < d.cols) sv = update4(d.off + (int64_t)r * d.cols + c);
+#pragma unroll
+            for (int q = 0; q < 4; q++) tile[4 * tx + q][rl] = sv[q];
+        }
+        __syncthreads();
+#pragma unroll
+        for (int ps = 0; ps < 2; ps++) {
+            const int cl = (tid >> 3) + 32 * ps, c = tc + cl, r0 = tr + (tid & 7) * 8;
+            if (c < d.cols && r0 < d.rows) {
+                bf16_t* dst = d.dst + (int64_t)c * d.dst_ld + r0;
+                if (vec) {
+                    *reinterpret_cast<bf16x8*>(dst) = *reinterpret_cast<const bf16x8*>(&tile[cl][(tid & 7) * 8]);
+                } else {
+                    for (int q = 0; q < 8 && r0 + q < d.rows; q++) dst[q] = tile[cl][(tid & 7) * 8 + q];
+                }
+            }
+        }
+        __syncthreads();
+    }
+}
 
 #define CLIP_CHUNK 8192
 struct GradClipOut { double norm; float scale; float factor; };
@@ -1391,6 +1456,24 @@
     return CMP_OK;
 }
 
+int adam_segs_run(void* stream, float* p, const float* g, float* m, float* v, void* shadow_bf16, const AdamSeg* segs_dev, int nseg,
+                  int max_tiles, int64_t n, float lr, float beta1, float beta2, float eps, int64_t step, float grad_scale,
+                  const float* factor_dev) {
+    CMP_REQUIRE(shadow_bf16 && segs_dev && nseg > 0 && nseg <= 65535, "adam_segs: bad arguments (nseg=%d)", nseg);
+    hipStream_t s = (hipStream_t)stream;
+    double alpha = (double)lr * sqrt(1.0 - pow((double)beta2, (double)step)) / (1.0 - pow((double)beta1, (double)step));
+    const dim3 grid(std::max(1, std::min(max_tiles, 256)), nseg);
+    PROF_START(7, s);
+    if (factor_dev)
+        adam_segs_kernel<true><<<grid, 256, 0, s>>>(p, g, m, v, (bf16_t*)shadow_bf16, segs_dev, (float)alpha, beta1, beta2, eps, 1.0f, factor_dev);
+    else
+        adam_segs_kernel<false><<<grid, 256, 0, s>>>(p, g, m, v, (bf16_t*)shadow_bf16, segs_dev, (float)alpha, beta1, beta2, eps, grad_scale,
+                                                     nullptr);
+    PROF_STOP(7, s, (double)n * 32.0, (double)n * 32.0);
+    KERNEL_CHECK();
+    return CMP_OK;
+}
+
 int64_t grad_sumsq_slots(int64_t n) { return cdiv64(n, CLIP_CHUNK); }
 int grad_sumsq_run(void* stream, const float* g, int64_t n, double* slots) {
     CMP_REQUIRE(n % 4 == 0 && ((uintptr_t)g & 15) == 0, "grad_sumsq: n=%lld must be a multiple of 4 and the range 16-byte aligned", (long long)n);
diff --git a/composer_amd/csrc/loss_head.hip b/composer_amd/csrc/loss_head.hip
--- /dev/null
+++ b/composer_amd/csrc/loss_head.hip
@@ -0,0 +1,249 @@
+#include "common.h"
+#include "model.h"
+
+typedef __attribute__((address_space(3))) void lh_lds_void;
+
+#define LH_BM 128
+#define LH_BN 512
+#define LH_BK 64
+#define LH_AIMG (LH_BM * LH_BK * 2)
+#define LH_BIMG (LH_BN * LH_BK * 2)
+#define LH_STAGE (LH_AIMG + LH_BIMG)
+#define LH_SMEM (2 * LH_STAGE)
+#define LH_OT_LD 1040
+#define LH_RED_OFF (LH_BM * LH_OT_LD)
+static_assert(LH_RED_OFF + 2 * 4 * LH_BM * 8 <= LH_SMEM, "epilogue areas must fit the stages");
+
+__device__ __forceinline__ int lh_off(int r, int c) { return r * 128 + ((c ^ ((r >> 1) & 7)) << 4); }
+
+template <int NP>
+__device__ __forceinline__ void lh_glds(__amdgpu_buffer_rsrc_t rs, char* img, int ld_bytes, int k0, int p0, int lane) {
+#pragma unroll
+    for (int i = 0; i < NP; i++) {
+        const int p = p0 + i;
+        const int r = 8 * p + (lane >> 3);
+        const int c = (lane & 7) ^ ((r >> 1) & 7);
+        const int voff = r * ld_bytes + (k0 + c * 8) * 2;
+        __builtin_amdgcn_raw_ptr_buffer_load_lds(rs, (lh_lds_void*)(img + p * 1024), 16, voff, 0, 0, 0);
+    }
+}
+__device__ __forceinline__ bf16x8 lh_frag(const char* img, int t16, int ks, int lane) {
+    return *reinterpret_cast<const bf16x8*>(img + lh_off(t16 * 16 + (lane & 15), ks * 4 + (lane >> 4)));
+}
+
+__global__ __launch_bounds__(512, 2) void loss_head_kernel(const bf16_t* __restrict__ hf, int ldh, const bf16_t* __restrict__ wte, int ldw,
+                                                           const int32_t* __restrict__ y, bf16_t* __restrict__ dz, int ldz,
+                                                           float* __restrict__ row_loss, int32_t* __restrict__ row_correct, int M, int V,
+                                                           int E, float inv_n) {
+    extern __shared__ __attribute__((aligned(16))) char smem[];
+    const int tid = threadIdx.x, lane = tid & 63;
+    const int wave = __builtin_amdgcn_readfirstlane(tid >> 6);
+    const int wm = wave >> 2, wn = wave & 3;
+    const int m0 = blockIdx.x * LH_BM;
+    const int nk = E / LH_BK;
+    const int64_t abytes = (int64_t)(M - m0) * ldh * 2, bbytes = (int64_t)V * ldw * 2;
+    __amdgpu_buffer_rsrc_t ra = __builtin_amdgcn_make_buffer_rsrc((void*)(hf + (int64_t)m0 * ldh), 0,
+                                                                  (int)min(abytes, (int64_t)0x7FFFFFF0), 0x00020000);
+    __amdgpu_buffer_rsrc_t rb = __builtin_amdgcn_make_buffer_rsrc((void*)wte, 0, (int)min(bbytes, (int64_t)0x7FFFFFF0), 0x00020000);
+    lh_glds<2>(ra, smem, ldh * 2, 0, wave * 2, lane);
+    lh_glds<8>(rb, smem + LH_AIMG, ldw * 2, 0, wave * 8, lane);
+
+    f32x4 acc[4][8];
+#pragma unroll
+    for (int i = 0; i < 4; i++)
+#pragma unroll
+        for (int j = 0; j < 8; j++) acc[i][j] = (f32x4){0.f, 0.f, 0.f, 0.f};
+    __syncthreads();
+    for (int kt = 0; kt < nk; kt++) {
+        const char* ia = smem + (kt & 1) * LH_STAGE;
+        const char* ib = ia + LH_AIMG;
+        if (kt + 1 < nk) {
+            char* na = smem + ((kt & 1) ^ 1) * LH_STAGE;
+            lh_glds<2>(ra, na, ldh * 2, (kt + 1) * LH_BK, wave * 2, lane);
+            lh_glds<8>(rb, na + LH_AIMG, ldw * 2, (kt + 1) * LH_BK, wave * 8, lane);
+        }
+        {
+            bf16x8 fa0[4], fa1[4], fbA[4], fbB[4];
+            auto mfma16 = [&](const bf16x8 (&fa)[4], const bf16x8 (&fb)[4], const int jh) __attribute__((always_inline)) {
+#pragma unroll
+                for (int i = 0; i < 4; i++)
+#pragma unroll
+                    for (int j = 0; j < 4; j++)
+                        acc[i][jh * 4 + j] = __builtin_amdgcn_mfma_f32_16x16x32_bf16(fb[j], fa[i], acc[i][jh * 4 + j], 0, 0, 0);
+            };
+#pragma unroll
+            for (int j = 0; j < 4; j++) fbA[j] = lh_frag(ib, wn * 8 + j, 0, lane);
+#pragma unroll
+            for (int i = 0; i < 4; i++) fa0[i] = lh_frag(ia, wm * 4 + i, 0, lane);
+#pragma unroll
+            for (int j = 0; j < 4; j++) fbB[j] = lh_frag(ib, wn * 8 + 4 + j, 0, lane);
+            mfma16(fa0, fbA, 0);
+#pragma unroll
+            for (int i = 0; i < 4; i++) fa1[i] = lh_frag(ia, wm * 4 + i, 1, lane);
+#pragma unroll
+            for (int j = 0; j < 4; j++) fbA[j] = lh_frag(ib, wn * 8 + j, 1, lane);
+            mfma16(fa0, fbB, 1);
+#pragma unroll
+            for (int j = 0; j < 4; j++) fbB[j] = lh_frag(ib, wn * 8 + 4 + j, 1, lane);
+            mfma16(fa1, fbA, 0);
+            mfma16(fa1, fbB, 1);
+            __builtin_amdgcn_sched_group_barrier(0x100, 8, 0);
+            __builtin_amdgcn_sched_group_barrier(0x100, 4, 0);
+            __builtin_amdgcn_sched_group_barrier(0x008, 16, 0);
+            __builtin_amdgcn_sched_group_barrier(0x100, 8, 0);
+            __builtin_amdgcn_sched_group_barrier(0x008, 16, 0);
+            __builtin_amdgcn_sched_group_barrier(0x100, 4, 0);
+            __builtin_amdgcn_sched_group_barrier(0x008, 16, 0);
+            __builtin_amdgcn_sched_group_barrier(0x008, 16, 0);
+        }
+        __syncthreads();
+    }
+
+    const int lg = lane >> 4;
+    const int cb = wn * 128 + lg * 4;
+    const int rl0 = wm * 64 + (lane & 15);
+    f32x2* red = reinterpret_cast<f32x2*>(smem + LH_RED_OFF);
+    f32x2* sums = red + 4 * LH_BM;
+    int yy[4];
+#pragma unroll
+    for (int i = 0; i < 4; i++) {
+        const int row = m0 + rl0 + i * 16;
+        yy[i] = row < M ? y[row] : 0;
+    }
+#pragma unroll
+    for (int i = 0; i < 4; i++) {
+        float mx = -INFINITY;
+        int arg = 0x7fffff;
+#pragma unroll
+        for (int j = 0; j < 8; j++)
+#pragma unroll
+            for (int q = 0; q < 4; q++) {
+                const int c = cb + j * 16 + q;
+                float v = acc[i][j][q];
+                if (c >= V) v = -INFINITY;
+                acc[i][j][q] = v;
+                if (v > mx) {
+                    mx = v;
+                    arg = c;
+                }
+            }
+#pragma unroll
+        for (int o = 16; o <= 32; o <<= 1) {
+            const float om = __shfl_xor(mx, o);
+            const int oa = __shfl_xor(arg, o);
+            if (om > mx || (om == mx && oa < arg)) {
+                mx = om;
+                arg = oa;
+            }
+        }
+        if (lg == 0) red[wn * LH_BM + rl0 + i * 16] = (f32x2){mx, (float)arg};
+    }
+    __syncthreads();
+    float gmx[4], ssum[4], zy[4];
+    int garg[4];
+#pragma unroll
+    for (int i = 0; i < 4; i++) {
+        const int rl = rl0 + i * 16;
+        f32x2 p = red[rl];
+        gmx[i] = p[0];
+        garg[i] = (int)p[1];
+#pragma unroll
+        for (int w = 1; w < 4; w++) {
+            p = red[w * LH_BM + rl];
+            if (p[0] > gmx[i]) {
+                gmx[i] = p[0];
+                garg[i] = (int)p[1];
+            }
+        }
+        float s = 0.f, z = 0.f;
+#pragma unroll
+        for (int j = 0; j < 8; j++)
+#pragma unroll
+            for (int q = 0; q < 4; q++) {
+                const int c = cb + j * 16 + q;
+                const float v = acc[i][j][q];
+                if (c == yy[i]) z += v;
+                const float e = __builtin_amdgcn_exp2f((v - gmx[i]) * 1.4426950408889634f);
+                acc[i][j][q] = e;
+                s += e;
+            }
+        s += __shfl_xor(s, 16);
+        z += __shfl_xor(z, 16);
+        s += __shfl_xor(s, 32);
+        z += __shfl_xor(z, 32);
+        if (lg == 0) sums[wn * LH_BM + rl] = (f32x2){s, z};
+    }
+    __syncthreads();
+#pragma unroll
+    for (int i = 0; i < 4; i++) {
+        const int rl = rl0 + i * 16;
+        const f32x2 p0 = sums[rl], p1 = sums[LH_BM + rl], p2 = sums[2 * LH_BM + rl], p3 = sums[3 * LH_BM + rl];
+        ssum[i] = (p0[0] + p1[0]) + (p2[0] + p3[0]);
+        zy[i] = (p0[1] + p1[1]) + (p2[1] + p3[1]);
+        const int row = m0 + rl;
+        if (wn == 0 && lg == 0 && row < M) {
+            row_loss[row] = gmx[i] + logf(ssum[i]) - zy[i];
+            row_correct[row] = (garg[i] == yy[i]) ? 1 : 0;
+        }
+    }
+    if (!dz) return;
+#pragma unroll
+    for (int i = 0; i < 4; i++) {
+        const float inv = 1.0f / ssum[i];
+        char* orow = smem + (rl0 + i * 16) * LH_OT_LD;
+#pragma unroll
+        for (int j = 0; j < 8; j++) {
+            bf16x4 o;
+#pragma unroll
+            for (int q = 0; q < 4; q++) {
+                const int c = cb + j * 16 + q;
+                const float g = (c < V) ? (acc[i][j][q] * inv - (c == yy[i] ? 1.0f : 0.0f)) * inv_n : 0.f;
+                o[q] = (bf16_t)g;
+            }
+            *reinterpret_cast<bf16x4*>(orow + (cb + j * 16) * 2) = o;
+        }
+    }
+    __syncthreads();
+    const int nch = ldz >> 3;
+    for (int idx = tid; idx < LH_BM * nch; idx += 512) {
+        const int r = idx / nch, ch = idx - r * nch;
+        if (m0 + r < M)
+            *reinterpret_cast<bf16x8*>(dz + (int64_t)(m0 + r) * ldz + ch * 8) = *reinterpret_cast<const bf16x8*>(smem + r * LH_OT_LD + ch * 16);
+    }
+}
+
+extern "C" int cmp_k_logits_xent_fused(int dtype, int V, int E, int ldh, int ldw, int ldz) {
+    return dtype == CMP_BF16 && V > 0 && V <= LH_BN && ldz >= V && ldz <= LH_BN && ldz % 8 == 0 && E > 0 && E % LH_BK == 0 && ldh >= E &&
+           ldw >= E && ldh % 8 == 0 && ldw % 8 == 0 && (int64_t)LH_BN * ldw * 2 < 0x7FFFFFF0ll && (int64_t)LH_BM * ldh * 2 < 0x7FFFFFF0ll;
+}
+
+extern "C" int cmp_k_logits_xent(void* stream, const void* hf, int ldh, const void* wte, int ldw, const int32_t* y, void* dlogits, int ldz,
+                                 float* row_loss, int32_t* row_correct, int M, int V, int E, float inv_n, int dtype, float* logits_ws) {
+    CMP_REQUIRE(hf && wte && y && row_loss && row_correct, "logits_xent: null argument");
+    CMP_REQUIRE(M >= 0 && V > 0 && V <= ldz && E > 0 && ldh >= E && ldw >= E, "logits_xent: M=%d V=%d ldz=%d E=%d ldh=%d ldw=%d", M, V, ldz, E,
+                ldh, ldw);
+    if (M == 0) return CMP_OK;
+    hipStream_t s = (hipStream_t)stream;
+    if (!cmp_k_logits_xent_fused(dtype, V, E, ldh, ldw, ldz)) {
+        CMP_REQUIRE(logits_ws, "logits_xent: V=%d E=%d dtype=%d is outside the fused kernel's domain and no logits workspace was given", V, E,
+                    dtype);
+        GemmExtra ex;
+        ex.role = 0;
+        CHECK_RC(gemm_run(stream, dtype, 0, 1, M, V, E, hf, ldh, wte, ldw, logits_ws, ldz, nullptr, 0, nullptr, 0, nullptr, 0, 1, 1, 0.f, 0, 0,
+                          0, ex));
+        return cmp_k_softmax_xent(stream, logits_ws, ldz, y, dlogits, row_loss, row_correct, M, V, inv_n, dtype);
+    }
+    CMP_REQUIRE(((uintptr_t)hf & 15) == 0 && ((uintptr_t)wte & 15) == 0 && (!dlogits || ((uintptr_t)dlogits & 15) == 0),
+                "logits_xent: operands must be 16-byte aligned");
+    static const bool once = [] {
+        (void)hipFuncSetAttribute((const void*)loss_head_kernel, hipFuncAttributeMaxDynamicSharedMemorySize, LH_SMEM);
+        return true;
+    }();
+    (void)once;
+    PROF_START(0, s);
+    loss_head_kernel<<<cdiv(M, LH_BM), 512, LH_SMEM, s>>>((const bf16_t*)hf, ldh, (const bf16_t*)wte, ldw, y, (bf16_t*)dlogits, ldz, row_loss,
+                                                         row_correct, M, V, E, inv_n);
+    PROF_STOP(0, s, 2.0 * M * V * E, ((double)M * E + (double)V * E + (dlogits ? (double)M * ldz : 0.0)) * 2.0 + (double)M * 12.0);
+    KERNEL_CHECK();
+    return CMP_OK;
+}
diff --git a/composer_amd/csrc/model.h b/composer_amd/csrc/model.h
--- a/composer_amd/csrc/model.h
+++ b/composer_amd/csrc/model.h
@@ -69,6 +69,13 @@
 struct WDesc {
     int64_t off;
     int rows, cols;
+};
+
+struct AdamSeg {
+    int64_t off;
+    int rows, cols;
+    bf16_t* dst;
+    int dst_ld, pad;
 };
 
 struct FoldDesc {
@@ -104,6 +111,9 @@
     void* ln_sites = nullptr;
     float* lnfold = nullptr;
     int64_t fold_stride = 0;
+    std::vector<AdamSeg> adam_segs_h;
+    void* adam_segs = nullptr;
+    bool st_sync = false;
     int st_state = 0;
     int64_t st_version = -1;
     bool fused_last = false;
@@ -112,6 +122,7 @@
     float* lnf_fold = nullptr;
     int lnf_npad = 0;
     float* lnf_part = nullptr;
+    bool head_pending = false;
     bool hf_valid = false;
     int64_t iterations = 0;
     int64_t param_version = 0;
@@ -222,13 +233,16 @@
 int lnf_fold_prep_run(void* stream, const float* wte, const float* gamma, const float* beta, void* out, float* cs, float* bias, int V, int E,
                       int npad);
 int colsum_run(void* stream, const void* X, int ldx, float* out, int rows, int cols, int dtype, float* det_ws, size_t det_ws_bytes);
+int adam_segs_run(void* stream, float* p, const float* g, float* m, float* v, void* shadow_bf16, const AdamSeg* segs_dev, int nseg,
+                  int max_tiles, int64_t n, float lr, float beta1, float beta2, float eps, int64_t step, float grad_scale,
+                  const float* factor_dev);
 int launch_metrics_reduce(hipStream_t s, const float* row_loss, const int32_t* row_correct, int rows, void* metrics);
 int launch_cast_bf16(hipStream_t s, const float* in, void* out, int64_t n);
 int64_t grad_sumsq_slots(int64_t n);
 int grad_sumsq_run(void* stream, const float* g, int64_t n, double* slots);
 int grad_clip_finish_run(void* stream, const double* slots, int nslots, float gscale, float clip_norm, void* out);
 int ensure_workspace(cmp_model* m, int B, int T);
-int model_forward(cmp_model* m, const int32_t* x_dev, int B, int T, bool training, int64_t step, int past_len = 0);
+int model_forward(cmp_model* m, const int32_t* x_dev, int B, int T, bool training, int64_t step, int past_len = 0, bool for_loss = false);
 void decode_state_free(DecodeState* d);
 void decode_batch_state_free(DecodeBatchState* d);
 int decode_batch_slide_stats(DecodeBatchState* d, int64_t* row_slides, int64_t* forward_calls);
diff --git a/composer_amd/csrc/model.hip b/composer_amd/csrc/model.hip
--- a/composer_amd/csrc/model.hip
+++ b/composer_amd/csrc/model.hip
@@ -327,6 +327,32 @@
         }
         CHECK_RC(dev_alloc(m, &m->wdesc, wd.size() * sizeof(WDesc)));
         HIP_CHECK(hipMemcpyAsync(m->wdesc, wd.data(), wd.size() * sizeof(WDesc), hipMemcpyHostToDevice, ctx->stream));
+        {
+            bool ok = true;
+            for (const WDesc& d : wd) ok = ok && d.cols % 4 == 0 && d.off % 4 == 0;
+            int64_t at = 0;
+            for (size_t i = 0; ok && i <= wd.size(); i++) {
+                const int64_t upto = i < wd.size() ? wd[i].off : m->total;
+                while (at < upto) {
+                    int64_t stop = upto;
+                    for (int b = 0; b < m->L; b++) if (m->lo[b].begin > at && m->lo[b].begin < stop) stop = m->lo[b].begin;
+                    if (m->off_lnf_g > at && m->off_lnf_g < stop) stop = m->off_lnf_g;
+                    ok = ok && (stop - at) % 4 == 0 && stop - at < (1ll << 31);
+                    m->adam_segs_h.push_back({at, 0, (int)(stop - at), nullptr, 0, 0});
+                    at = stop;
+                }
+                if (i < wd.size()) {
+                    m->adam_segs_h.push_back({wd[i].off, wd[i].rows, wd[i].cols, m->ST + wd[i].off, wd[i].rows, 0});
+                    at = wd[i].off + (int64_t)wd[i].rows * wd[i].cols;
+                }
+            }
+            if (!ok) m->adam_segs_h.clear();
+            if (!m->adam_segs_h.empty()) {
+                CHECK_RC(dev_alloc(m, &m->adam_segs, m->adam_segs_h.size() * sizeof(AdamSeg)));
+                HIP_CHECK(hipMemcpyAsync(m->adam_segs, m->adam_segs_h.data(), m->adam_segs_h.size() * sizeof(AdamSeg), hipMemcpyHostToDevice,
+                                         ctx->stream));
+            }
+        }
         std::vector<WDesc> wp;
         std::vector<FoldDesc> fd;
         m->fold_stride = 2 * (int64_t)(3 * m->Ea + 4 * m->E);
@@ -455,6 +481,21 @@
     }
     HIP_CHECK(hipMemcpyAsync(host, b + p.offset, (size_t)numel * 4, hipMemcpyDeviceToHost, m->ctx->stream));
     HIP_CHECK(hipStreamSynchronize(m->ctx->stream));
+    return CMP_OK;
+}
+extern "C" int cmp_shadow_get(cmp_model* m, const char* name, int transposed, void* host_u16, int64_t numel, int* current) {
+    CMP_REQUIRE(m && name && host_u16, "shadow_get: null");
+    CMP_REQUIRE(m->S && (!transposed || m->ST), "shadow_get: the model keeps no bf16 shadow (fp32 mode)");
+    auto it = m->index.find(name);
+    CMP_REQUIRE(it != m->index.end(), "shadow_get: unknown parameter '%s'", name);
+    const ParamInfo& p = m->params[it->second];
+    CMP_REQUIRE(numel == p.store, "shadow_get: '%s' stores %lld elements, caller passed %lld", name, (long long)p.store, (long long)numel);
+    HIP_CHECK(hipSetDevice(m->ctx->device));
+    HIP_CHECK(hipStreamSynchronize(m->ctx->stream));
+    HIP_CHECK(hipStreamSynchronize(m->ctx->comm_stream));
+    HIP_CHECK(hipMemcpyAsync(host_u16, (transposed ? m->ST : m->S) + p.offset, (size_t)numel * 2, hipMemcpyDeviceToHost, m->ctx->stream));
+    HIP_CHECK(hipStreamSynchronize(m->ctx->stream));
+    if (current) *current = transposed ? (m->st_state == 1 && m->st_version == m->param_version ? 1 : 0) : 1;
     return CMP_OK;
 }
 extern "C" int cmp_param_set(cmp_model* m, const char* name, int kind, const float* host, int64_t numel) {
@@ -720,8 +761,14 @@
 
 static float attn_scale(const cmp_model* m) { return m->cfg.scale_attention ? 1.0f / sqrtf((float)m->Dl) : 1.0f; }
 
-int model_forward(cmp_model* m, const int32_t* x_dev, int B, int T, bool training, int64_t step, int past_len) {
+static bool loss_head_ok(const cmp_model* m) {
+    static const bool on = [] { const char* e = getenv("COMPOSER_LOSS_HEAD"); return !(e && e[0] == '0'); }();
+    return on && cmp_k_logits_xent_fused(m->dtype, m->V, m->E, m->E, m->E, m->ldz) != 0;
+}
+
+int model_forward(cmp_model* m, const int32_t* x_dev, int B, int T, bool training, int64_t step, int past_len, bool for_loss) {
     Range range_("composer.forward");
+    m->head_pending = false;
     hipStream_t s = m->ctx->stream;
     struct RoleGuard {
         cmp_model* m;
@@ -815,6 +862,10 @@
     CHECK_RC(cmp_k_layernorm_fwd(s, m->xs[m->L], m->P + m->off_lnf_g, m->P + m->off_lnf_b, m->hf, m->lnf_mean, m->lnf_rstd, M,
                                  E, m->cfg.ln_eps, dt));
     m->hf_valid = true;
+    if (for_loss && loss_head_ok(m)) {
+        m->head_pending = true;
+        return CMP_OK;
+    }
     CHECK_RC(gemm(m, 0, 1, M, m->V, E, m->hf, E, m->w(m->off_wte), E, m->logits, m->ldz, nullptr, 0, nullptr, 0, nullptr, 0, 1,
                   1, 0.f, 0));
     return CMP_OK;
@@ -823,6 +874,11 @@
 static int loss(cmp_model* m, const int32_t* y_dev, int M, bool want_grad) {
     Range range_("composer.loss");
     hipStream_t s = m->ctx->stream;
+    if (m->head_pending) {
+        m->head_pending = false;
+        CHECK_RC(cmp_k_logits_xent(s, m->hf, m->E, m->w(m->off_wte), m->E, y_dev, want_grad ? m->dlogits : nullptr, m->ldz, m->row_loss,
+                                   m->row_correct, M, m->V, m->E, 1.0f / (float)M, m->dtype, nullptr));
+    } else
     CHECK_RC(cmp_k_softmax_xent(s, m->logits, m->ldz, y_dev, want_grad ? m->dlogits : nullptr, m->row_loss, m->row_correct, M,
                                 m->V, 1.0f / (float)M, m->dtype));
     CHECK_RC(launch_metrics_reduce(s, m->row_loss, m->row_correct, M, m->metrics));
@@ -837,9 +893,33 @@
     return std::min(s, std::max(1, K / 256));
 }
 
+static bool adam_seg_run_of(const cmp_model* m, int64_t begin, int64_t end, int* first, int* count, int* max_tiles) {
+    const std::vector<AdamSeg>& t = m->adam_segs_h;
+    int i0 = -1, i1 = -1, mt = 1;
+    for (int i = 0; i < (int)t.size(); i++) {
+        const int64_t e = t[i].off + (t[i].rows ? (int64_t)t[i].rows * t[i].cols : (int64_t)t[i].cols);
+        if (t[i].off == begin) i0 = i;
+        if (i0 >= 0 && i1 < 0) mt = std::max(mt, t[i].rows ? cdiv(t[i].rows, 64) * cdiv(t[i].cols, 64) : cdiv(t[i].cols, 1024));
+        if (e == end && i0 >= 0 && i1 < 0) i1 = i + 1;
+    }
+    if (i0 < 0 || i1 <= i0) return false;
+    *first = i0; *count = i1 - i0; *max_tiles = mt;
+    return true;
+}
+static int adam_span(cmp_model* m, hipStream_t s, int64_t begin, int64_t end, float lr, int64_t step, float gscale, const float* factor_dev) {
+    int first = 0, count = 0, mt = 1;
+    if (m->adam_segs && adam_seg_run_of(m, begin, end, &first, &count, &mt))
+        return adam_segs_run(s, m->P, m->G, m->Am, m->Av, m->S, (const AdamSeg*)m->adam_segs + first, count, mt, end - begin, lr, 0.9f, 0.999f,
+                             1e-7f, step, gscale, factor_dev);
+    m->st_sync = false;
+    void* sh = m->S ? (void*)(m->S + begin) : nullptr;
+    if (factor_dev)
+        return cmp_k_adam_dev(s, m->P + begin, m->G + begin, m->Am + begin, m->Av + begin, sh, end - begin, lr, 0.9f, 0.999f, 1e-7f, step,
+                              factor_dev);
+    return cmp_k_adam(s, m->P + begin, m->G + begin, m->Am + begin, m->Av + begin, sh, end - begin, lr, 0.9f, 0.999f, 1e-7f, step, gscale);
+}
 static int adam_range(cmp_model* m, hipStream_t s, int64_t begin, int64_t end, float lr, int64_t step, float gscale) {
-    return cmp_k_adam(s, m->P + begin, m->G + begin, m->Am + begin, m->Av + begin, m->S ? (void*)(m->S + begin) : nullptr, end - begin, lr,
-                      0.9f, 0.999f, 1e-7f, step, gscale);
+    return adam_span(m, s, begin, end, lr, step, gscale, nullptr);
 }
 
 static int bucket_ready(cmp_model* m, int ev, int64_t begin, int64_t end, float lr, bool update) {
@@ -1048,8 +1128,7 @@
 
 static int adam_clipped(cmp_model* m, hipStream_t s, int nslots, float lr, int64_t step, float gscale) {
     CHECK_RC(grad_clip_finish_run(s, m->clip_slots, nslots, gscale, m->clip_norm, m->clip_out));
-    return cmp_k_adam_dev(s, m->P, m->G, m->Am, m->Av, m->S ? (void*)m->S : nullptr, m->total, lr, 0.9f, 0.999f, 1e-7f, step,
-                          &m->clip_out->factor);
+    return adam_span(m, s, 0, m->total, lr, step, gscale, &m->clip_out->factor);
 }
 
 static int adam(cmp_model* m, float lr) {
@@ -1232,12 +1311,17 @@
     m->last_has_norm = false;
     m->dp_buckets_updated = 0;
     m->clip_slots_used = 0;
-    int rc = model_forward(m, x_dev, B, T, true, step);
+    m->st_sync = true;
+    int rc = model_forward(m, x_dev, B, T, true, step, 0, true);
     if (rc == CMP_OK) rc = loss(m, y_dev, B * T, true);
     if (rc == CMP_OK) rc = dp_metrics_begin(m);
     if (rc == CMP_OK) rc = backward(m, x_dev, B, T, step, final_, lr, final_, j == 0);
     m->ctx->seed_mix = seed_mix;
     if (rc == CMP_OK) rc = final_ ? adam(m, lr) : dp_metrics_end(m);
+    if (rc == CMP_OK && final_ && m->adam_segs && m->st_sync && (!m->ctx->dp_on() || m->dp_buckets_updated == m->L + 2)) {
+        m->st_state = 1;
+        m->st_version = m->param_version;
+    }
     if (rc == CMP_OK) {
         m->accum_pending = final_ ? 0 : j + 1;
         m->accumB = B; m->accumT = T;
@@ -1457,7 +1541,7 @@
     CHECK_RC(upload_xy(m, x, y, B, T));
     const int64_t step = m->iterations;
     m->accum_pending = 0;
-    CHECK_RC(model_forward(m, m->x_dev, B, T, true, step));
+    CHECK_RC(model_forward(m, m->x_dev, B, T, true, step, 0, true));
     CHECK_RC(loss(m, m->y_dev, B * T, true));
     CHECK_RC(backward(m, m->x_dev, B, T, step, false));
     CHECK_RC(fetch_metrics(m));
@@ -1470,7 +1554,7 @@
     CMP_REQUIRE(m && x && y, "eval_step: null argument");
     HIP_CHECK(hipSetDevice(m->ctx->device));
     CHECK_RC(upload_xy(m, x, y, B, T));
-    CHECK_RC(model_forward(m, m->x_dev, B, T, false, 0));
+    CHECK_RC(model_forward(m, m->x_dev, B, T, false, 0, 0, true));
     CHECK_RC(loss(m, m->y_dev, B * T, false));
     CHECK_RC(fetch_metrics(m));
     HIP_CHECK(hipStreamSynchronize(m->ctx->stream));
diff --git a/include/composer_hip.h b/include/composer_hip.h
--- a/include/composer_hip.h
+++ b/include/composer_hip.h
@@ -74,6 +74,7 @@
 int cmp_param_info(cmp_model* m, int i, const char** name, int* rank, int64_t shape[4], int64_t* numel);
 int cmp_param_get(cmp_model* m, const char* name, int kind, float* host, int64_t numel);
 int cmp_param_set(cmp_model* m, const char* name, int kind, const float* host, int64_t numel);
+int cmp_shadow_get(cmp_model* m, const char* name, int transposed, void* host_u16, int64_t numel, int* current);
 int cmp_adam_iter_get(cmp_model* m, int64_t* iterations);
 int cmp_adam_iter_set(cmp_model* m, int64_t iterations);
 
@@ -197,6 +198,9 @@
                    float p_drop, uint64_t seed, uint32_t rng_stream);
 int cmp_k_softmax_xent(void* stream, const float* logits, int ldz, const int32_t* y, void* dlogits,
                        float* row_loss, int32_t* row_correct, int rows, int V, float inv_n, int dtype);
+int cmp_k_logits_xent_fused(int dtype, int V, int E, int ldh, int ldw, int ldz);
+int cmp_k_logits_xent(void* stream, const void* hf, int ldh, const void* wte, int ldw, const int32_t* y, void* dlogits, int ldz,
+                      float* row_loss, int32_t* row_correct, int M, int V, int E, float inv_n, int dtype, float* logits_ws);
 int cmp_k_adam(void* stream, float* p, const float* g, float* m, float* v, void* shadow_bf16,
                int64_t n, float lr, float beta1, float beta2, float eps, int64_t step, float grad_scale);
 int cmp_k_adam_dev(void* stream, float* p, const float* g, float* m, float* v, void* shadow_bf16,
```

After: 5.079 million tokens/s (median of 6 runs). Within noise of the previous version (+0.3%).
